# sc15i2gp/daily-ray-trace

Measured on AMD Instinct MI355X. Metric: Mpaths/s (pixels*spp/s) Cornell 1024^2 depth 8; achieved HBM GB/s % of peak, higher is better.
Workload: dtype f64

## Files before the change

daily-ray-trace_amd/csrc/drt_kernels.h:

```cpp
#pragma once

#include "drt_device.h"
#include "drt_build_rule.h"
#include "drt_stash_rule.h"
#include <type_traits>
#include "../../include/drt_hip.h"


enum
{
    SF_PX = 0, SF_PY, SF_PZ, SF_RADIUS,
    SF_NX, SF_NY, SF_NZ,
    SF_UNX, SF_UNY, SF_UNZ,
    SF_VNX, SF_VNY, SF_VNZ,
    SF_ULEN, SF_VLEN,
    SF_COUNT
};
enum
{
    LF_PX = 0, LF_PY, LF_PZ, LF_RADIUS,
    LF_UX, LF_UY, LF_UZ,
    LF_VX, LF_VY, LF_VZ,
    LF_PDF,
    LF_COUNT
// ... 1696 lines not shown
{
    const DevRayTable no_table = {nullptr, nullptr, nullptr, 0u, 0u, 0u, 0u};
    trace_paths_form<SCENE_IN_LDS, TAIL, LIST, false, SCENE_IN_LDS>(k_sc, k_cam, k_tp, records, headers, k_hits, k_counters, k_work_counter, no_table);
}

template <bool SCENE_IN_LDS, bool TAIL = false, bool LIST = false>
__global__ __launch_bounds__(TRACE_BLOCK, DRT_TRACE_WAVES_PER_SIMD) void drt_trace_direct_kernel(DevScene k_sc, DevCamera k_cam, TraceParams k_tp,
                                                                 uint64_t *__restrict__ records, uint64_t *__restrict__ headers,
                                                                 int32_t *__restrict__ k_hits, unsigned long long *__restrict__ k_counters,
                                                                 unsigned long long *__restrict__ k_work_counter)
{
    const DevRayTable no_table = {nullptr, nullptr, nullptr, 0u, 0u, 0u, 0u};
    trace_paths<SCENE_IN_LDS, TAIL, LIST, false>(k_sc, k_cam, k_tp, records, headers, k_hits, k_counters, k_work_counter, no_table);
}

template <bool SCENE_IN_LDS, bool TAIL = false, bool LIST = false>
__global__ __launch_bounds__(TRACE_BLOCK, DRT_TRACE_WAVES_PER_SIMD) void drt_trace_rays_kernel(DevScene k_sc, DevCamera k_cam, TraceParams k_tp,
                                                                 uint64_t *__restrict__ records, uint64_t *__restrict__ headers,
                                                                 int32_t *__restrict__ k_hits, unsigned long long *__restrict__ k_counters,
                                                                 unsigned long long *__restrict__ k_work_counter, DevRayTable k_rt)
{
    trace_paths<SCENE_IN_LDS, TAIL, LIST, true>(k_sc, k_cam, k_tp, records, headers, k_hits, k_counters, k_work_counter, k_rt);
}


#define SHADE_BLOCK 256
#ifndef DRT_SHADE_WAVES_PER_SIMD
#define DRT_SHADE_WAVES_PER_SIMD 4
#endif
#define SHADE_WAVES (SHADE_BLOCK / 64)
#ifndef DRT_SHADE_WAVES_MULTISET
#define DRT_SHADE_WAVES_MULTISET(n) ((n) == 2 ? 3 : 2)
#endif
#define SHADE_WAVES_PER_SIMD_FOR(n) ((n) == 1 ? DRT_SHADE_WAVES_PER_SIMD : DRT_SHADE_WAVES_MULTISET(n))
#ifndef DRT_SHADE_WAVES_SIMPLE
#define DRT_SHADE_WAVES_SIMPLE 5
#endif
#define SHADE_MAX_SETS 4

struct ShadeParams
{
    uint64_t n_pix;
    uint32_t n_samples, first_sample, vertex_words, block_words;
    uint32_t n_lights, batch;
    const uint32_t *overflow;
    uint32_t vertex_shift, mode;
    uint32_t tail_first, tail_count;
    uint32_t chunk, sub_pixels;
    uint32_t light0_em_spd, tail_staged;
    double  *tail_stage;
    const double *tail_resume;
    uint32_t cmf_rw, cmf_x, cmf_y, cmf_z;
    uint32_t tail_period_mains, no_fixed_lists;
    uint32_t items_per_group, n_items;
    const uint32_t *pixel_list;
    const uint32_t *sample_base;
};

struct ShadeConst
{
    DevScene    sc;
    ShadeParams sp;
    const uint64_t     *records, *headers;
    double             *film_pixels, *film_avgs, *film_vars;
    unsigned long long *work_counter;
};
static_assert(sizeof(DevScene) % 8 == 0 && sizeof(ShadeParams) % 8 == 0, "ShadeConst mirrors the kernarg segment only while every argument ends on an 8-byte boundary");
__device__ __forceinline__ const ShadeConst &shade_const()
{
    uint32_t off = 0;
    asm volatile("" : "+s"(off));
    return *(const ShadeConst *)((const char *)__builtin_amdgcn_kernarg_segment_ptr() + off);
}

__device__ __forceinline__ double word_as_double(uint64_t w) { return __longlong_as_double((long long)w); }

__device__ __forceinline__ uint64_t readlane64(uint64_t v, uint32_t l)
{
    uint32_t lo = (uint32_t)__builtin_amdgcn_readlane((int)(uint32_t)v, (int)l);
    uint32_t hi = (uint32_t)__builtin_amdgcn_readlane((int)(uint32_t)(v >> 32), (int)l);
    return (uint64_t)lo | ((uint64_t)hi << 32);
}

__device__ __forceinline__ const uint64_t *path_vertex(const uint64_t *__restrict__ pool, uint32_t block_words, uint32_t vw, uint64_t h2, uint64_t h3, uint32_t v)
{
    const uint32_t b = v >> REC_BLOCK_SHIFT;
    uint32_t id;
    if (b == 0) id = (uint32_t)h2;
    else if (b == 1) id = (uint32_t)(h2 >> 32);
    else if (b == 2) id = (uint32_t)h3;
    else id = ((const uint32_t *)(pool + (uint64_t)(uint32_t)(h3 >> 32) * block_words))[b - REC_HEADER_BLOCKS];
    return pool + (uint64_t)id * block_words + (uint64_t)(v & (REC_BLOCK_VERTICES - 1u)) * vw;
}

template <typename SpdPtr>
__device__ __forceinline__ double spd_at(SpdPtr spds, uint32_t S, uint32_t idx, uint32_t lam)
{
    return spds[idx * S + lam];
}

#define DRT_LIST_MIRROR ((uint64_t)DRT_BDSF_mirror_bdsf)
#define DRT_LIST_GLASS ((uint64_t)DRT_BDSF_fs_dielectric_reflectance_bdsf | ((uint64_t)DRT_BDSF_fs_dielectric_transmittance_bdsf << 4))
#define DRT_LIST_CONDUCTOR ((uint64_t)DRT_BDSF_fs_conductor_bdsf)
#define DRT_LIST_GGX ((uint64_t)DRT_BDSF_ct_conductor_bdsf)
#define DRT_LIST_PLASTIC ((uint64_t)DRT_BDSF_bp_diffuse_bdsf | ((uint64_t)DRT_BDSF_bp_glossy_bdsf << 4))
template <bool SIMPLE = false, uint32_t FIXED_N = 0, uint64_t FIXED_LIST = 0>
__device__ __forceinline__ double bdsf_at_wavelength(uint64_t list_arg, uint32_t num_bdsfs_arg, double diffuse_pi, double glossy, double mirror,
                                                     double ir, double tr, double te, double on_dot, double a_in, double spec,
                                                     double mn_dot, double ct_coef, uint32_t flags, bool paired)
{
    const uint64_t list = FIXED_N != 0u ? FIXED_LIST : list_arg;
    const uint32_t num_bdsfs = FIXED_N != 0u ? FIXED_N : num_bdsfs_arg;
    double bdsf_result = 0.0;
    double reflectance = 0.0;
#define DRT_PIN_HERE(x) asm volatile("" : "+v"(x))
    for (uint32_t i = 0; i < num_bdsfs; i += 1)
    {
        switch ((uint32_t)(list >> (4 * i)) & 15u)
        {
            case DRT_BDSF_bp_diffuse_bdsf:
                bdsf_result = diffuse_pi * a_in;
                break;
            case DRT_BDSF_bp_glossy_bdsf:
                bdsf_result = (glossy * spec) * a_in;
                break;
            case DRT_BDSF_mirror_bdsf:
                bdsf_result = (flags & FLAG_EQR) ? mirror : 0.0;
                break;
            case DRT_BDSF_fs_conductor_bdsf:
                if (SIMPLE) break;
                if (flags & FLAG_EQR)
                {
                    DRT_PIN_HERE(ir);
                    double c2 = on_dot * on_dot;
                    bdsf_result = conductor_reflectance_sel(paired, ir, tr, te, on_dot, c2, 1.0 - c2);
                }
                break;
            case DRT_BDSF_fs_dielectric_reflectance_bdsf:
                if (SIMPLE) break;
                if (flags & FLAG_EQR)
                {
                    DRT_PIN_HERE(ir);
                    bdsf_result = dielectric_reflectance_sel(paired, ir, tr, te, on_dot, 1.0 - on_dot * on_dot);
                }
                break;
            case DRT_BDSF_fs_dielectric_transmittance_bdsf:
                if (SIMPLE) break;
                if (flags & FLAG_EQT)
                {
                    DRT_PIN_HERE(ir);
                    bdsf_result = 1.0 - dielectric_reflectance_sel(paired, ir, tr, te, on_dot, 1.0 - on_dot * on_dot);
                }
                break;
            case DRT_BDSF_ct_conductor_bdsf:
            {
                if (SIMPLE) break;
                DRT_PIN_HERE(ir);
                double c2 = mn_dot * mn_dot;
                bdsf_result = conductor_reflectance_sel(paired, ir, tr, te, mn_dot, c2, 1.0 - c2) * ct_coef;
                break;
            }
            default: break;
        }
        reflectance = bdsf_result + reflectance;
    }
#undef DRT_PIN_HERE
    return reflectance;
}

#ifndef SHADE_PREFETCH_REGS
#define SHADE_PREFETCH_REGS 2
#endif
#define SHADE_PREFETCH_DEPTH 1
#define SHADE_PIXEL_CHUNK 16
#define TAIL_WINDOW_ENTRIES 112u
#define TAIL_WINDOW_WORDS (3u * TAIL_WINDOW_ENTRIES + TAIL_WINDOW_ENTRIES / 4u)
#define SHADE_WAVE_LDS_WORDS ((2u * 64u * SHADE_PREFETCH_REGS) > TAIL_WINDOW_WORDS ? (2u * 64u * SHADE_PREFETCH_REGS) : TAIL_WINDOW_WORDS)

#define XYZ_FILM_WORDS 8

template <bool SPDS_IN_LDS, bool XYZ, bool SIMPLE, bool LIST = false>
__device__ __forceinline__ void shade_tail_group(const DevScene &sc, const ShadeParams &sp, const double *lds, uint64_t *wave_lds, const uint64_t *__restrict__ records,
                                                 const uint64_t *__restrict__ headers, double *__restrict__ film_pixels,
                                                 double *__restrict__ film_avgs, double *__restrict__ film_vars, uint64_t chunk_base,
                                                 uint64_t chunk_end, uint32_t lane, const bool closed)
{
    const uint32_t S = sc.S;
    const uint32_t vw = sp.vertex_words;
    const uint32_t R = sp.tail_count;
    const uint32_t g = lane / R, j = lane - g * R;
    const bool act = g < (uint32_t)(chunk_end - chunk_base) && g < 64u / R;
    const uint32_t lam = sp.tail_first + j;
    const double *table = SPDS_IN_LDS ? (const double *)lds : sc.spds;
    const uint32_t n_groups = 64u / R;
    const uint32_t win = TAIL_WINDOW_ENTRIES / n_groups;
    uint16_t *task_list = (uint16_t *)(wave_lds + 3u * TAIL_WINDOW_ENTRIES);
    const uint32_t leader = g * R;
    const bool in_group = g < n_groups;
    uint32_t v = 0, n_shaded = 0;
    uint64_t ph0 = 0;
    double vignette = 0.0, throughput = 1.0, dst = 0.0;
    uint64_t ph2 = 0;
    uint64_t slot = 0;
    const uint64_t *vcur = records;
    const bool one_light = sp.n_lights == 1u;
    const double em0 = spd_at(table, S, one_light ? sp.light0_em_spd : 0u, lam);
    auto deep_blocks = [&](uint32_t vertex) -> uint64_t { return vertex >= 2u * REC_BLOCK_VERTICES ? headers[slot * REC_HEADER_WORDS + 3] : 0ull; };
    for (uint32_t s0 = sp.tail_staged ? sp.n_samples : 0u; s0 < sp.n_samples; s0 += win)
    {
        const uint32_t s_end = s0 + win < sp.n_samples ? s0 + win : sp.n_samples;
        const uint32_t n_win = s_end - s0, n_px = (uint32_t)(chunk_end - chunk_base);
        uint32_t n_tasks = 0;
        for (uint32_t e0 = 0; e0 < n_px * n_win; e0 += 64u)
        {
            const uint32_t e = e0 + lane;
            const bool valid = e < n_px * n_win;
            const uint32_t ge = valid ? e / n_win : 0u, off = valid ? e - ge * n_win : 0u;
            const uint64_t eslot = (chunk_base + ge) * (uint64_t)sp.batch + s0 + off;
            uint64_t h0 = 0, h1 = 0, h2 = 0;
            if (valid)
            {
                const uint64_t *h = headers + eslot * REC_HEADER_WORDS;
                h0 = h[0];
                h1 = h[1];
                h2 = h[2];
            }
            const bool staged = ((uint32_t)(h0 >> 16) & HDR_TERM_TAIL_STAGED) != 0u;
            const bool has_path = valid && !staged && (h0 & 0xFFFFu) != 0u;
            if (valid && !staged && !has_path)
            {
                const bool emissive = ((uint32_t)(h0 >> 16) & HDR_TERM_MASK) == 1u;
                const uint32_t row = (uint32_t)(h0 >> 32) & 0xFFFFu;
                for (uint32_t t = 0; t < R; t += 1)
                {
                    double d = 0.0;
                    if (emissive) d = d + 1.0 * spd_at(table, S, row, sp.tail_first + t);
                    sp.tail_stage[eslot * R + t] = d * word_as_double(h1);
                }
            }
            const unsigned long long m = __ballot(has_path);
            if (has_path)
            {
                const uint32_t k = n_tasks + (uint32_t)__popcll(m & ((1ull << lane) - 1ull));
                task_list[k] = (uint16_t)e;
                uint64_t *w = wave_lds + e * 3u;
                w[0] = h0;
                w[1] = h1;
                w[2] = h2;
            }
            n_tasks += (uint32_t)__popcll(m);
        }
        __builtin_amdgcn_wave_barrier();
        uint32_t next_task = 0;
        bool busy = false;
        for (;;)
        {
            const unsigned long long want = __ballot(!busy && in_group && lane == leader);
            if (want != 0ull)
            {
                const uint32_t mine = next_task + (uint32_t)__popcll(want & ((1ull << leader) - 1ull));
                if (!busy && in_group && mine < n_tasks)
                {
                    const uint32_t e = task_list[mine];
                    const uint64_t *w = wave_lds + e * 3u;
                    const uint32_t ge = e / n_win, off = e - ge * n_win;
                    slot = (chunk_base + ge) * (uint64_t)sp.batch + s0 + off;
                    ph0 = w[0];
                    vignette = word_as_double(w[1]);
                    ph2 = w[2];
                    n_shaded = (uint32_t)(ph0 & 0xFFFFu);
                    const uint32_t k = ((uint32_t)(ph0 >> 16) >> HDR_TERM_RESUME_SHIFT) & HDR_TERM_RESUME_MASK;
                    v = k;
                    throughput = 1.0;
                    dst = 0.0;
                    if (k != 0u)
                    {
                        const double *at = sp.tail_stage + (slot * R + j);
                        dst = at[0];
                        throughput = at[shade_const().sp.tail_resume - sp.tail_stage];
// ... 121 lines not shown
                        });
                    else if (closed)
                        lane_vertex([&](uint32_t flags, const uint64_t *a) {
                            return bdsf_at_wavelength<SIMPLE, 2, DRT_LIST_PLASTIC>(0, 0, diffuse_pi, glossy, 0.0, 0.0, 0.0, 0.0, 0.0, word_as_double(a[0]), word_as_double(a[1]), 0.0, 0.0, flags, false);
                        });
                    else
                        lane_vertex([&](uint32_t flags, const uint64_t *a) {
                            return bdsf_at_wavelength<SIMPLE>(list, num_bdsfs, diffuse_pi, glossy, mirror, ir, tr, te, on_dot, word_as_double(a[0]), word_as_double(a[1]),
                                                              word_as_double(a[2]), word_as_double(a[3]), flags, paired);
                        });
                    v += 1;
                    if (v < n_shaded) vcur = (v & (REC_BLOCK_VERTICES - 1u)) != 0u ? vcur + vw : path_vertex(records, sp.block_words, vw, ph2, deep_blocks(v), v);
                }
            }
            if (busy && v >= n_shaded)
            {
                if (((uint32_t)(ph0 >> 16) & HDR_TERM_MASK) == 1u) dst = dst + throughput * spd_at(table, S, (uint32_t)(ph0 >> 32) & 0xFFFFu, lam);
                sp.tail_stage[slot * R + j] = dst * vignette;
                busy = false;
            }
        }
        __builtin_amdgcn_wave_barrier();
    }
    uint32_t j_b = j;
    asm volatile("" : "+v"(j_b));
    const uint32_t lam_b = sp.tail_first + j_b;
    uint32_t g_b = g;
    asm volatile("" : "+v"(g_b));
    const uint64_t pix_b = chunk_base + g_b;
    const uint64_t pix_f = LIST ? (act ? (uint64_t)sp.pixel_list[pix_b] : 0u) : pix_b;
    double *px = film_pixels + pix_f * (uint64_t)(XYZ ? XYZ_FILM_WORDS : S + 1);
    double *pa = XYZ ? nullptr : film_avgs + pix_f * (uint64_t)S;
    double *pv = XYZ ? nullptr : film_vars + pix_f * (uint64_t)S;
    const double *stage = sp.tail_stage + (pix_b * (uint64_t)sp.batch) * R + j_b;
    const uint32_t first = LIST ? sp.first_sample + (act ? sp.sample_base[pix_f] : 0u) : sp.first_sample;
    double f_sum = (act && !XYZ) ? px[lam_b] : 0.0, f_avg = (act && !XYZ) ? pa[lam_b] : 0.0, f_var = (act && !XYZ) ? pv[lam_b] : 0.0;
#pragma unroll 4
    for (uint32_t k = 0; k < sp.n_samples; k += 1)
    {
        const double contribution = act ? stage[(uint64_t)k * R] : 0.0;
        const double denom = (double)(first + k + 1);
        f_sum = f_sum + contribution;
        if (!XYZ)
        {
            double t0 = contribution - f_avg;
            double t1 = t0;
            t0 = t0 / denom;
            f_avg = f_avg + t0;
            t0 = contribution - f_avg;
            t0 = t1 * t0;
            f_var = f_var + t0;
        }
    }
    if (XYZ)
    {
        const double rw = spd_at(table, S, sp.cmf_rw, lam_b);
        const double x = act ? (spd_at(table, S, sp.cmf_x, lam_b) * f_sum * rw) : 0.0;
        const double y = act ? (spd_at(table, S, sp.cmf_y, lam_b) * f_sum * rw) : 0.0;
        const double z = act ? (spd_at(table, S, sp.cmf_z, lam_b) * f_sum * rw) : 0.0;
        double X = 0.0, Y = 0.0, Z = 0.0;
        for (uint32_t t = 0; t < R; t += 1)
        {
            const int src = (int)((lane - j_b + t) & 63u);
            X += __shfl(x, src);
            Y += __shfl(y, src);
            Z += __shfl(z, src);
        }
        if (act && j_b == 0)
        {
            px[4] += X;
            px[5] += Y;
            px[6] += Z;
        }
    }
    else if (act)
    {
        px[lam_b] = f_sum;
        pa[lam_b] = f_avg;
        pv[lam_b] = f_var;
    }
}


template <int NSETS, bool SPDS_IN_LDS, bool XYZ, bool DARK, bool SIMPLE, bool LIST, bool CLOSED>
__device__ __forceinline__ void shade_pixels(const DevScene &sc, const ShadeParams &sp, const uint64_t *__restrict__ records,
                                             const uint64_t *__restrict__ headers, double *__restrict__ film_pixels,
                                             double *__restrict__ film_avgs, double *__restrict__ film_vars,
                                             unsigned long long *__restrict__ work_counter)
{
    static_assert(!CLOSED || (NSETS == 1 && SPDS_IN_LDS && !XYZ && !SIMPLE && !LIST), "the closed form exists for one wavelength set, tables in LDS, spectral film, dense launches");
    extern __shared__ double lds[];
    const uint32_t S = sc.S;
    if (*sp.overflow) return;
    if (SPDS_IN_LDS)
    {
        const uint32_t spd_words = sc.n_spd * S;
        for (uint32_t k = threadIdx.x; k < spd_words; k += SHADE_BLOCK) lds[k] = sc.spds[k];
        __syncthreads();
    }
    const uint32_t lane = threadIdx.x & 63u;
    uint64_t *rec_lds = (uint64_t *)(lds + (SPDS_IN_LDS ? (size_t)sc.n_spd * S : 0)) + (size_t)(threadIdx.x >> 6) * SHADE_WAVE_LDS_WORDS;
    const uint32_t vw = sp.vertex_words;
    const uint32_t vpr = vw <= 64 ? 64u / vw : 0u;
    const uint32_t n_fast_regs = vpr * SHADE_PREFETCH_REGS;
    const uint32_t n_fast = n_fast_regs < 2u * REC_BLOCK_VERTICES ? n_fast_regs : 2u * REC_BLOCK_VERTICES;

    uint32_t lam_c[NSETS];
#pragma unroll
    for (int k = 0; k < NSETS; k += 1)
    {
        const uint32_t lam = 64u * k + lane;
        lam_c[k] = lam < S ? lam : 0;
    }

    const uint32_t S_main = sp.tail_count ? sp.tail_first : S;
    for (;;)
    {
        const ShadeParams &qc = shade_const().sp;
        uint32_t item = 0;
        if (lane == 0) item = (uint32_t)atomicAdd(work_counter, 1ull);
        item = (uint32_t)__builtin_amdgcn_readfirstlane((int)item);
        if (item >= qc.n_items) break;
        const bool split = qc.items_per_group > 1;
        const bool inline_tail = qc.tail_count != 0;
        const uint32_t mains_per_group = qc.items_per_group - (inline_tail ? 1u : 0u);
        bool tail_item = inline_tail;
        uint32_t group = item, sub = 0;
        if (split)
        {
            uint32_t m = item;
            if (inline_tail)
            {
                const uint32_t n_groups = qc.n_items / qc.items_per_group;
                const uint32_t q = qc.tail_period_mains, mixed = n_groups * (q + 1u);
                if (item < mixed)
                {
                    const uint32_t period = item / (q + 1u), r = item - period * (q + 1u);
                    tail_item = r == 0u;
                    group = period;
                    m = period * q + (r - 1u);
                }
                else
                {
                    tail_item = false;
                    m = n_groups * q + (item - mixed);
                }
            }
            if (!tail_item)
            {
                group = m / mains_per_group;
                sub = m - group * mains_per_group;
            }
        }
        const uint64_t chunk_base = (uint64_t)group * qc.chunk;
        const uint64_t chunk_end = (chunk_base + qc.chunk < qc.n_pix) ? chunk_base + qc.chunk : qc.n_pix;
        uint64_t main_base = chunk_base, main_end = chunk_end;
        if (split)
        {
            main_base = chunk_base + (uint64_t)sub * qc.sub_pixels;
            main_end = (main_base + qc.sub_pixels < chunk_end) ? main_base + qc.sub_pixels : chunk_end;
            if (tail_item || main_base > chunk_end) main_base = main_end = chunk_end;
        }

      if (qc.mode == 2u) main_base = main_end;
      for (uint64_t pix = main_base; pix < main_end; pix += 1)
      {

        const uint64_t pix_f = LIST ? (uint64_t)sp.pixel_list[pix] : pix;
        double *px = film_pixels + pix_f * (uint64_t)(XYZ ? XYZ_FILM_WORDS : S + 1);
        double *pa = XYZ ? nullptr : film_avgs + pix_f * (uint64_t)S;
        double *pv = XYZ ? nullptr : film_vars + pix_f * (uint64_t)S;
        const uint32_t first = LIST ? sp.first_sample + sp.sample_base[pix_f] : sp.first_sample;
        double f_sum[NSETS], f_avg[NSETS], f_var[NSETS];
#pragma unroll
        for (int k = 0; k < NSETS; k += 1)
        {
            const uint32_t lam = 64u * k + lane;
            const bool active = lam < S_main;
            f_sum[k] = (active && !XYZ) ? px[lam] : 0.0;
            f_avg[k] = (active && !XYZ) ? pa[lam] : 0.0;
            f_var[k] = (active && !XYZ) ? pv[lam] : 0.0;
        }
        bool dark = false;
        if (DARK)
        {
            bool some = false;
#pragma unroll
            for (int k = 0; k < NSETS; k += 1)
                some = some || ((uint64_t)__double_as_longlong(f_sum[k]) | (uint64_t)__double_as_longlong(f_avg[k]) | (uint64_t)__double_as_longlong(f_var[k])) != 0ull;
            dark = !__any(some);
        }
      for (uint32_t s0 = 0; s0 < sp.n_samples; s0 += 64u)
      {
        const uint32_t n_win = (uint32_t)__builtin_amdgcn_readfirstlane((int)((sp.n_samples - s0 < 64u) ? sp.n_samples - s0 : 64u));
        __builtin_assume(n_win >= 1u);
        uint64_t h0 = 0, h1 = 0, h2 = 0, h3 = 0;
        if (lane < n_win)
        {
            const uint64_t *h = headers + (pix * sp.batch + s0 + lane) * REC_HEADER_WORDS;
            h0 = h[0];
            h1 = h[1];
            h2 = h[2];
            h3 = h[3];
        }
        const unsigned long long worthless = !DARK ? 0ull : __ballot(lane < n_win && (h0 & 0xFFFFu) == 0ull && ((uint32_t)(h0 >> 16) & HDR_TERM_MASK) != 1u &&
                                                                      __builtin_isfinite(word_as_double(h1)));
        if (DARK && dark && (uint32_t)__popcll(worthless) == n_win) continue;
        auto prefetch = [&](uint32_t sa, uint32_t nw, uint64_t *dst) {
            if (nw == 0u) return;
            const uint64_t b2 = readlane64(h2, sa);
#pragma unroll
            for (int k = 0; k < SHADE_PREFETCH_REGS; k += 1)
            {
                const uint32_t b = (64u * k) >> (sp.vertex_shift + REC_BLOCK_SHIFT);
                const uint32_t id = b == 0 ? (uint32_t)b2 : (uint32_t)(b2 >> 32);
                const uint64_t *base = records + (uint64_t)id * sp.block_words + (64u * k - (b << (sp.vertex_shift + REC_BLOCK_SHIFT)));
                dst[k] = (64u * k + lane < nw) ? base[lane] : 0;
            }
        };
        uint64_t ring[SHADE_PREFETCH_DEPTH + 1][SHADE_PREFETCH_REGS];
#pragma unroll
        for (int d = 0; d < SHADE_PREFETCH_DEPTH; d += 1)
        {
            const uint32_t nw = ((uint32_t)d < n_win) ? (uint32_t)(readlane64(h0, d) & 0xFFFFu) * vw : 0u;
            prefetch((uint32_t)d < n_win ? (uint32_t)d : 0u, nw, ring[d + 1]);
        }
        for (uint32_t s = 0; s < n_win; s += 1)
        {
            const uint64_t hs = readlane64(h0, s);
            const double vignette = word_as_double(readlane64(h1, s));
            const uint32_t n_shaded = (uint32_t)(hs & 0xFFFFu);
            const uint32_t term = (uint32_t)(hs >> 16) & HDR_TERM_MASK;
            const uint32_t term_spd = (uint32_t)(hs >> 32) & 0xFFFFu;
            const uint32_t plastic_mask = (uint32_t)(hs >> 48);
            const uint32_t vis0_mask = (uint32_t)(hs >> 24) & 0xFFu;
#pragma unroll
            for (int d = 0; d < SHADE_PREFETCH_DEPTH; d += 1)
#pragma unroll
                for (int k = 0; k < SHADE_PREFETCH_REGS; k += 1) ring[d][k] = ring[d + 1][k];
            {
                const uint32_t sa = s + SHADE_PREFETCH_DEPTH;
                const uint32_t nw = (sa < n_win) ? (uint32_t)(readlane64(h0, sa) & 0xFFFFu) * vw : 0u;
                prefetch(sa < n_win ? sa : 0u, nw, ring[SHADE_PREFETCH_DEPTH]);
            }
            const uint64_t *cur = ring[0];
            if (n_shaded != 0u)
            {
                uint64_t *slot_now = rec_lds + (s & 1u) * (64u * SHADE_PREFETCH_REGS);
#pragma unroll
                for (int k = 0; k < SHADE_PREFETCH_REGS; k += 1) slot_now[64u * k + lane] = ring[0][k];
            }
            const uint64_t *rec_words = rec_lds + (s & 1u) * (64u * SHADE_PREFETCH_REGS);
            if (DARK && dark && ((worthless >> s) & 1ull) != 0ull) continue;

            double throughput[NSETS], dst[NSETS];
#pragma unroll
            for (int k = 0; k < NSETS; k += 1)
            {
                throughput[k] = 1.0;
                dst[k] = 0.0;
            }
            uint32_t v_first = 0;
            if (NSETS == 1 && sp.n_lights == 1u && vpr != 0u)
            {
                uint32_t run = (uint32_t)__builtin_ctz(~plastic_mask | 0x10000u);
                run = run < n_shaded ? run : n_shaded;
                run = run < n_fast ? run : n_fast;
                run = run < 8u ? run : 8u;
                if (run != 0u)
                {
                const double *table1 = SPDS_IN_LDS ? (const double *)lds : sc.spds;
                const double em0 = spd_at(table1, S, sp.light0_em_spd, lam_c[0]);
                auto run_vertex = [&](uint64_t w1, const uint64_t *vwords, bool visible) {
                    const double diffuse_pi = spd_at(table1, S, (uint32_t)(w1 >> 16) & 0xFFFFu, lam_c[0]);
                    const double glossy = spd_at(table1, S, (uint32_t)(w1 >> 32) & 0xFFFFu, lam_c[0]);
                    const double dir_pdf = word_as_double(vwords[4]), s_a_in = word_as_double(vwords[5]), s_spec = word_as_double(vwords[6]);
                    const double c = word_as_double(vwords[REC_VERTEX_WORDS + 1]), a_in = word_as_double(vwords[REC_VERTEX_WORDS + 2]);
                    const double spec = word_as_double(vwords[REC_VERTEX_WORDS + 3]);
                    double contribution = 0.0;
                    if (visible)
                    {
                        double reflectance = diffuse_pi * a_in + 0.0;
                        reflectance = (glossy * spec) * a_in + reflectance;
                        contribution = contribution + reflectance;
                        contribution = contribution * em0;
                        contribution = contribution * c;
                    }
                    dst[0] = dst[0] + throughput[0] * contribution;
                    double reflectance = diffuse_pi * s_a_in + 0.0;
                    reflectance = (glossy * s_spec) * s_a_in + reflectance;
                    reflectance = reflectance * dir_pdf;
                    throughput[0] = throughput[0] * reflectance;
                };
                const uint32_t run0 = run < vpr ? run : vpr;
                for (uint32_t v = 0; v < run0; v += 1)
                    run_vertex(readlane64(cur[0], v * vw + 1u), rec_words + v * vw, ((vis0_mask >> v) & 1u) != 0u);
                for (uint32_t v = run0; v < run; v += 1)
                    run_vertex(readlane64(cur[SHADE_PREFETCH_REGS > 1 ? 1 : 0], (v - vpr) * vw + 1u), rec_words + v * vw, ((vis0_mask >> v) & 1u) != 0u);
                v_first = run;
                if (run == n_fast && n_shaded > run && vw * REC_BLOCK_VERTICES == 64u)
                {
                    const uint64_t h3s = readlane64(h3, s);
                    for (uint32_t b = n_fast / REC_BLOCK_VERTICES; b * REC_BLOCK_VERTICES < n_shaded && b < 4u; b += 1)
                    {
                        uint32_t id = (uint32_t)h3s;
                        if (b == 1u) id = (uint32_t)(readlane64(h2, s) >> 32);
                        if (b >= REC_HEADER_BLOCKS) id = ((const uint32_t *)(records + (uint64_t)(uint32_t)(h3s >> 32) * sp.block_words))[b - REC_HEADER_BLOCKS];
                        const uint64_t blockw = records[(uint64_t)id * sp.block_words + lane];
                        uint64_t *slot = rec_lds + (s & 1u) * (64u * SHADE_PREFETCH_REGS);
                        slot[lane] = blockw;
                        const uint32_t v_lo = b * REC_BLOCK_VERTICES;
                        const uint32_t v_hi = n_shaded < v_lo + REC_BLOCK_VERTICES ? n_shaded : v_lo + REC_BLOCK_VERTICES;
                        uint32_t v = v_lo;
                        for (; v < v_hi && ((plastic_mask >> v) & 1u); v += 1)
                        {
                            const uint32_t w0 = (v - v_lo) * vw;
                            const uint64_t lw0 = readlane64(blockw, w0 + REC_VERTEX_WORDS);
                            run_vertex(readlane64(blockw, w0 + 1u), slot + w0, ((uint32_t)(lw0 >> 16) & FLAG_VISIBLE) != 0u);
                        }
                        v_first = v;
                        if (v < v_hi) break;
                    }
                }
                }
            }
            for (uint32_t v = v_first; v < n_shaded; v += 1)
            {
                uint64_t src;
                uint32_t lane0;
                if (v < n_fast)
                {
                    const uint32_t sel = v / vpr;
                    lane0 = (v - sel * vpr) * vw;
                    src = cur[0];
                    if (SHADE_PREFETCH_REGS > 1 && sel != 0) src = cur[SHADE_PREFETCH_REGS > 1 ? 1 : 0];
                }
                else
                {
                    lane0 = 0;
                    src = (lane < vw) ? path_vertex(records, sp.block_words, vw, readlane64(h2, s), readlane64(h3, s), v)[lane] : 0;
                }
                const double *table = SPDS_IN_LDS ? (const double *)lds : sc.spds;
                double contribution[NSETS];
#pragma unroll
                for (int k = 0; k < NSETS; k += 1) contribution[k] = 0.0;
                auto plastic_vertex = [&](uint64_t w1, double dir_pdf, double s_a_in, double s_spec) {
                    const uint32_t i_diffuse = (uint32_t)(w1 >> 16) & 0xFFFFu, i_glossy = (uint32_t)(w1 >> 32) & 0xFFFFu;
                        double diffuse_pi[NSETS], glossy[NSETS];
#pragma unroll
                        for (int k = 0; k < NSETS; k += 1)
                        {
                            diffuse_pi[k] = spd_at(table, S, i_diffuse, lam_c[k]);
                            glossy[k] = spd_at(table, S, i_glossy, lam_c[k]);
                        }
                        if (sp.n_lights == 1u && v < 8u && v < n_fast)
                        {
                            if ((vis0_mask >> v) & 1u)
                            {
                                const uint32_t off = REC_VERTEX_WORDS;
                                const uint64_t *lw = rec_words + v * vw + off;
                                const double c = word_as_double(lw[1]), a_in = word_as_double(lw[2]), spec = word_as_double(lw[3]);
#pragma unroll
                                for (int k = 0; k < NSETS; k += 1)
                                {
                                    double reflectance = diffuse_pi[k] * a_in + 0.0;
                                    reflectance = (glossy[k] * spec) * a_in + reflectance;
                                    contribution[k] = contribution[k] + reflectance;
                                    contribution[k] = contribution[k] * spd_at(table, S, sp.light0_em_spd, lam_c[k]);
                                    contribution[k] = contribution[k] * c;
                                }
                            }
                        }
                        else
                        for (uint32_t l = 0; l < sp.n_lights; l += 1)
                        {
                            if (l == 0 && v < 8u && !((vis0_mask >> v) & 1u)) continue;
                            const uint32_t off = REC_VERTEX_WORDS + l * REC_LIGHT_WORDS;
                            uint64_t lw[4];
                            if (off + REC_LIGHT_WORDS <= 64 || v < n_fast)
                            {
#pragma unroll
                                for (int k = 0; k < 4; k += 1) lw[k] = readlane64(src, lane0 + off + k);
                            }
                            else
                            {
                                const uint64_t *lp = path_vertex(records, sp.block_words, vw, readlane64(h2, s), readlane64(h3, s), v) + off;
#pragma unroll
                                for (int k = 0; k < 4; k += 1) lw[k] = readlane64(lp[k], 0);
                            }
                            if (!((uint32_t)(lw[0] >> 16) & FLAG_VISIBLE)) continue;
                            const uint32_t i_em = (uint32_t)(lw[0] & 0xFFFFu);
                            const double c = word_as_double(lw[1]), a_in = word_as_double(lw[2]), spec = word_as_double(lw[3]);
#pragma unroll
                            for (int k = 0; k < NSETS; k += 1)
                            {
                                double reflectance = diffuse_pi[k] * a_in + 0.0;
                                reflectance = (glossy[k] * spec) * a_in + reflectance;
                                contribution[k] = contribution[k] + reflectance;
                                contribution[k] = contribution[k] * spd_at(table, S, i_em, lam_c[k]);
                                contribution[k] = contribution[k] * c;
                            }
                        }
#pragma unroll
                        for (int k = 0; k < NSETS; k += 1)
                        {
                            dst[k] = dst[k] + throughput[k] * contribution[k];
                            double reflectance = diffuse_pi[k] * s_a_in + 0.0;
                            reflectance = (glossy[k] * s_spec) * s_a_in + reflectance;
                            reflectance = reflectance * dir_pdf;
                            throughput[k] = throughput[k] * reflectance;
                        }
                };
                if (v < 16u && ((plastic_mask >> v) & 1u))
                {
                    const uint64_t w1p = readlane64(src, lane0 + 1);
                    if (v < n_fast)
                    {
                        const uint64_t *vwords = rec_words + v * vw;
                        plastic_vertex(w1p, word_as_double(vwords[4]), word_as_double(vwords[5]), word_as_double(vwords[6]));
                        continue;
                    }
                    const double dir_pdf_p = word_as_double(readlane64(src, lane0 + 4));
                    const double s_a_in_p = word_as_double(readlane64(src, lane0 + 5)), s_spec_p = word_as_double(readlane64(src, lane0 + 6));
                    plastic_vertex(w1p, dir_pdf_p, s_a_in_p, s_spec_p);
                    continue;
                }
                const uint64_t list = readlane64(src, lane0 + 0);
                const uint64_t w1 = readlane64(src, lane0 + 1);
                const uint32_t num_bdsfs = (uint32_t)(w1 & 0xFFu);
                const uint32_t sflags = (uint32_t)(w1 >> 8) & 0xFFu;
                auto fixed_vertex = [&](uint32_t kind) {
                    const bool fresnel = !SIMPLE && kind != 0u;
                    constexpr bool GGX_BODY = CLOSED;
                    const bool rough = GGX_BODY && kind == 3u;
                    const bool in_lds = v < n_fast;
                    const uint64_t *vwords = rec_words + v * vw;
                    uint32_t i_r0 = (uint32_t)(w1 >> 48) & 0xFFFFu, i_r1 = 0, i_r2 = 0;
                    bool paired = false;
                    double on_dot = 0.0;
                    double ct = 0.0;
                    double r0[NSETS], r1[NSETS], r2[NSETS];
#pragma unroll
                    for (int k = 0; k < NSETS; k += 1) r1[k] = r2[k] = 0.0;
                    if (fresnel)
                    {
                        fresnel_rows(readlane64(src, lane0 + 2), i_r0, i_r1, i_r2, paired);
                        if (!rough) on_dot = in_lds ? word_as_double(vwords[3]) : word_as_double(readlane64(src, lane0 + 3));
#pragma unroll
                        for (int k = 0; k < NSETS; k += 1)
                        {
                            r1[k] = spd_at(table, S, i_r1, lam_c[k]);
                            r2[k] = spd_at(table, S, i_r2, lam_c[k]);
                        }
                    }
#pragma unroll
                    for (int k = 0; k < NSETS; k += 1) r0[k] = spd_at(table, S, i_r0, lam_c[k]);
                    auto eval = [&](int k, uint32_t flags) -> double {
                        if (SIMPLE || kind == 0u)
                            return bdsf_at_wavelength<SIMPLE, 1u, DRT_LIST_MIRROR>(0ull, 0u, 0.0, 0.0, r0[k], 0.0, 0.0, 0.0, 0.0, 0.0, 0.0, 0.0, 0.0, flags, false);
                        if (kind == 1u)
                            return bdsf_at_wavelength<SIMPLE, 2u, DRT_LIST_GLASS>(0ull, 0u, 0.0, 0.0, 0.0, r0[k], r1[k], r2[k], on_dot, 0.0, 0.0, 0.0, 0.0, flags, paired);
                        if (kind == 2u || !GGX_BODY)
                            return bdsf_at_wavelength<SIMPLE, 1u, DRT_LIST_CONDUCTOR>(0ull, 0u, 0.0, 0.0, 0.0, r0[k], r1[k], r2[k], on_dot, 0.0, 0.0, 0.0, 0.0, flags, paired);
                        return bdsf_at_wavelength<SIMPLE, 1u, DRT_LIST_GGX>(0ull, 0u, 0.0, 0.0, 0.0, r0[k], r1[k], r2[k], 0.0, 0.0, 0.0, on_dot, ct, flags, paired);
                    };
                    for (uint32_t l = 0; l < sp.n_lights; l += 1)
                    {
                        if (l == 0 && v < 8u && !((vis0_mask >> v) & 1u)) continue;
                        const uint32_t off = REC_VERTEX_WORDS + l * REC_LIGHT_WORDS;
                        uint64_t lw0;
                        double c;
                        if (off + REC_LIGHT_WORDS <= 64 || v < n_fast)
                        {
                            lw0 = readlane64(src, lane0 + off);
                            c = in_lds ? word_as_double(vwords[off + 1u]) : word_as_double(readlane64(src, lane0 + off + 1u));
                            if (rough)
                            {
                                on_dot = in_lds ? word_as_double(vwords[off + 4u]) : word_as_double(readlane64(src, lane0 + off + 4u));
                                ct = in_lds ? word_as_double(vwords[off + 5u]) : word_as_double(readlane64(src, lane0 + off + 5u));
                            }
                        }
                        else
                        {
                            const uint64_t *lp = path_vertex(records, sp.block_words, vw, readlane64(h2, s), readlane64(h3, s), v) + off;
                            lw0 = readlane64(lp[0], 0);
                            c = word_as_double(lp[1]);
                            if (rough)
                            {
                                on_dot = word_as_double(lp[4]);
                                ct = word_as_double(lp[5]);
                            }
                        }
                        const uint32_t lflags = (uint32_t)(lw0 >> 16) & 0xFFu;
                        if (!(lflags & FLAG_VISIBLE)) continue;
                        const uint32_t i_em = (uint32_t)(lw0 & 0xFFFFu);
#pragma unroll
                        for (int k = 0; k < NSETS; k += 1)
                        {
                            double reflectance = eval(k, lflags);
                            contribution[k] = contribution[k] + reflectance;
                            contribution[k] = contribution[k] * spd_at(table, S, i_em, lam_c[k]);
                            contribution[k] = contribution[k] * c;
                        }
                    }
                    if (rough)
                    {
                        on_dot = in_lds ? word_as_double(vwords[7]) : word_as_double(readlane64(src, lane0 + 7));
                        ct = in_lds ? word_as_double(vwords[8]) : word_as_double(readlane64(src, lane0 + 8));
                    }
#pragma unroll
                    for (int k = 0; k < NSETS; k += 1)
                    {
                        dst[k] = dst[k] + throughput[k] * contribution[k];
                        double reflectance = eval(k, sflags);
                        const double dir_pdf = in_lds ? word_as_double(vwords[4]) : word_as_double(readlane64(src, lane0 + 4));
                        reflectance = reflectance * dir_pdf;
                        throughput[k] = throughput[k] * reflectance;
                    }
                };
                if (CLOSED)
                {
                    if (sflags & FLAG_PLASTIC)
                        plastic_vertex(w1, word_as_double(readlane64(src, lane0 + 4)), word_as_double(readlane64(src, lane0 + 5)), word_as_double(readlane64(src, lane0 + 6)));
                    else
                        fixed_vertex(list == DRT_LIST_MIRROR ? 0u : list == DRT_LIST_GLASS ? 1u : list == DRT_LIST_CONDUCTOR ? 2u : 3u);
                    continue;
                }
                if (!shade_const().sp.no_fixed_lists)
                {
                    uint32_t kind = 4u;
                    if (num_bdsfs == 1u && list == DRT_LIST_MIRROR) kind = 0u;
                    if (!SIMPLE && num_bdsfs == 2u && list == DRT_LIST_GLASS) kind = 1u;
                    if (!SIMPLE && num_bdsfs == 1u && list == DRT_LIST_CONDUCTOR) kind = 2u;
                    if (kind != 4u)
                    {
                        fixed_vertex(kind);
                        continue;
                    }
                }
                const uint64_t w2 = readlane64(src, lane0 + 2);
                const double on_dot = word_as_double(readlane64(src, lane0 + 3));
                const double dir_pdf = word_as_double(readlane64(src, lane0 + 4));
                const uint32_t i_diffuse = (uint32_t)(w1 >> 16) & 0xFFFFu, i_glossy = (uint32_t)(w1 >> 32) & 0xFFFFu;
                const uint32_t i_mirror = (uint32_t)(w1 >> 48) & 0xFFFFu;
                uint32_t i_ir, i_tr, i_te;
                bool paired;
                fresnel_rows(w2, i_ir, i_tr, i_te, paired);
                const double s_a_in = word_as_double(readlane64(src, lane0 + 5)), s_spec = word_as_double(readlane64(src, lane0 + 6));

                if (sflags & FLAG_PLASTIC)
                {
                    plastic_vertex(w1, dir_pdf, s_a_in, s_spec);
                    continue;
                }

                double diffuse[NSETS], glossy[NSETS], mirror[NSETS], ir[NSETS], tr[NSETS], te[NSETS];
#pragma unroll
                for (int k = 0; k < NSETS; k += 1)
                {
                    diffuse[k] = spd_at(table, S, i_diffuse, lam_c[k]); glossy[k] = spd_at(table, S, i_glossy, lam_c[k]);
                    mirror[k] = spd_at(table, S, i_mirror, lam_c[k]);   ir[k] = SIMPLE ? 0.0 : spd_at(table, S, i_ir, lam_c[k]);
                    tr[k] = SIMPLE ? 0.0 : spd_at(table, S, i_tr, lam_c[k]); te[k] = SIMPLE ? 0.0 : spd_at(table, S, i_te, lam_c[k]);
                }
                for (uint32_t l = 0; l < sp.n_lights; l += 1)
                {
                    if (l == 0 && v < 8u && !((vis0_mask >> v) & 1u)) continue;
                    const uint32_t off = REC_VERTEX_WORDS + l * REC_LIGHT_WORDS;
                    uint64_t lw[REC_LIGHT_WORDS];
                    if (off + REC_LIGHT_WORDS <= 64 || v < n_fast)
                    {
#pragma unroll
                        for (int k = 0; k < REC_LIGHT_WORDS; k += 1) lw[k] = readlane64(src, lane0 + off + k);
                    }
                    else
                    {
                        const uint64_t *lp = path_vertex(records, sp.block_words, vw, readlane64(h2, s), readlane64(h3, s), v) + off;
#pragma unroll
                        for (int k = 0; k < REC_LIGHT_WORDS; k += 1) lw[k] = readlane64(lp[k], 0);
                    }
                    const uint32_t lflags = (uint32_t)(lw[0] >> 16) & 0xFFu;
                    if (!(lflags & FLAG_VISIBLE)) continue;
                    const uint32_t i_em = (uint32_t)(lw[0] & 0xFFFFu);
                    const double c = word_as_double(lw[1]);
#pragma unroll
                    for (int k = 0; k < NSETS; k += 1)
                    {
                        double reflectance = bdsf_at_wavelength<SIMPLE>(list, num_bdsfs, diffuse[k], glossy[k], mirror[k], ir[k], tr[k], te[k], on_dot,
                                                                word_as_double(lw[2]), word_as_double(lw[3]), word_as_double(lw[4]),
                                                                word_as_double(lw[5]), lflags, paired);
                        contribution[k] = contribution[k] + reflectance;
                        contribution[k] = contribution[k] * spd_at(table, S, i_em, lam_c[k]);
                        contribution[k] = contribution[k] * c;
                    }
                }
                const double s_mn = word_as_double(readlane64(src, lane0 + 7)), s_ct = word_as_double(readlane64(src, lane0 + 8));
#pragma unroll
                for (int k = 0; k < NSETS; k += 1)
                {
                    dst[k] = dst[k] + throughput[k] * contribution[k];
                    double reflectance = bdsf_at_wavelength<SIMPLE>(list, num_bdsfs, diffuse[k], glossy[k], mirror[k], ir[k], tr[k], te[k], on_dot,
                                                            s_a_in, s_spec, s_mn, s_ct, sflags, paired);
                    reflectance = reflectance * dir_pdf;
                    throughput[k] = throughput[k] * reflectance;
                }
            }
            const double denom = (double)(first + s0 + s + 1);
            if (DARK) dark = false;
#pragma unroll
            for (int k = 0; k < NSETS; k += 1)
            {
                if (term == 1)
                {
                    const double em = SPDS_IN_LDS ? spd_at((const double *)lds, S, term_spd, lam_c[k]) : spd_at(sc.spds, S, term_spd, lam_c[k]);
                    dst[k] = dst[k] + throughput[k] * em;
                }
                const double contribution = dst[k] * vignette;
                f_sum[k] = f_sum[k] + contribution;
                if (!XYZ)
                {
                    double t0 = contribution - f_avg[k];
                    double t1 = t0;
                    t0 = t0 / denom;
                    f_avg[k] = f_avg[k] + t0;
                    t0 = contribution - f_avg[k];
                    t0 = t1 * t0;
                    f_var[k] = f_var[k] + t0;
                }
            }
        }
      }
        if (XYZ)
        {
            const double *table = SPDS_IN_LDS ? (const double *)lds : sc.spds;
            double X = 0.0, Y = 0.0, Z = 0.0;
#pragma unroll
            for (int k = 0; k < NSETS; k += 1)
            {
                const uint32_t lam = 64u * k + lane;
                if (lam < S_main)
                {
                    const double rw = spd_at(table, S, sp.cmf_rw, lam);
                    X += (spd_at(table, S, sp.cmf_x, lam) * f_sum[k] * rw);
                    Y += (spd_at(table, S, sp.cmf_y, lam) * f_sum[k] * rw);
                    Z += (spd_at(table, S, sp.cmf_z, lam) * f_sum[k] * rw);
                }
            }
            for (int off = 32; off > 0; off >>= 1)
            {
                X += __shfl_xor(X, off);
                Y += __shfl_xor(Y, off);
                Z += __shfl_xor(Z, off);
            }
            if (lane == 0)
            {
                px[0] += X;
                px[1] += Y;
                px[2] += Z;
                px[3] += (double)sp.n_samples * 1.0;
            }
        }
        else
        {
#pragma unroll
            for (int k = 0; k < NSETS; k += 1)
            {
                const uint32_t lam = 64u * k + lane;
                if (lam < S_main)
                {
                    px[lam] = f_sum[k];
                    pa[lam] = f_avg[k];
                    pv[lam] = f_var[k];
                }
            }
            if (lane == 0) px[S] += (double)sp.n_samples * 1.0;
        }
      }

        if (tail_item && sp.mode != 1u) shade_tail_group<SPDS_IN_LDS, XYZ, SIMPLE, LIST>(sc, sp, (const double *)lds, rec_lds, records, headers, film_pixels, film_avgs, film_vars, chunk_base, chunk_end, lane, CLOSED);
    }
}

template <int NSETS, bool SPDS_IN_LDS, bool XYZ, bool DARK, bool SIMPLE = false, bool LIST = false>
__global__ __launch_bounds__(SHADE_BLOCK, (SIMPLE && NSETS == 1) ? DRT_SHADE_WAVES_SIMPLE : SHADE_WAVES_PER_SIMD_FOR(NSETS)) void drt_shade_kernel(DevScene sc, ShadeParams sp, const uint64_t *__restrict__ records,
                                                                 const uint64_t *__restrict__ headers, double *__restrict__ film_pixels,
                                                                 double *__restrict__ film_avgs, double *__restrict__ film_vars,
                                                                 unsigned long long *__restrict__ work_counter)
{
    shade_pixels<NSETS, SPDS_IN_LDS, XYZ, DARK, SIMPLE, LIST, false>(sc, sp, records, headers, film_pixels, film_avgs, film_vars, work_counter);
}

#ifndef DRT_SHADE_WAVES_CLOSED
#define DRT_SHADE_WAVES_CLOSED 4
#endif
template <bool DARK>
__global__ __launch_bounds__(SHADE_BLOCK, DRT_SHADE_WAVES_CLOSED) void drt_shade_kernel_closed(DevScene sc, ShadeParams sp, const uint64_t *__restrict__ records,
                                                                 const uint64_t *__restrict__ headers, double *__restrict__ film_pixels,
                                                                 double *__restrict__ film_avgs, double *__restrict__ film_vars,
                                                                 unsigned long long *__restrict__ work_counter)
{
    shade_pixels<1, true, false, DARK, false, false, true>(sc, sp, records, headers, film_pixels, film_avgs, film_vars, work_counter);
}

__global__ void drt_film_xyz_kernel(DevScene sc, uint32_t cmf_rw, uint32_t cmf_x, uint32_t cmf_y, uint32_t cmf_z, double interval,
                                    uint64_t n_pix, const double *__restrict__ film_pixels, double *__restrict__ xyz)
{
    uint64_t p = (uint64_t)blockIdx.x * blockDim.x + threadIdx.x;
    if (p >= n_pix) return;
    const uint32_t S = sc.S;
    const double *rw = sc.spds + (size_t)cmf_rw * S, *cx = sc.spds + (size_t)cmf_x * S;
    const double *cy = sc.spds + (size_t)cmf_y * S, *cz = sc.spds + (size_t)cmf_z * S;
    const double *px = film_pixels + p * (uint64_t)(S + 1);
    double f = px[S];
    double n = 0.0;
    for (uint32_t i = 0; i < S; i += 1) n += (cy[i] * rw[i]);
    n *= interval;
    double X = 0.0, Y = 0.0, Z = 0.0;
    for (uint32_t i = 0; i < S; i += 1)
    {
        double v = px[i] / f;
        X += (cx[i] * v * rw[i]);
        Y += (cy[i] * v * rw[i]);
        Z += (cz[i] * v * rw[i]);
    }
    xyz[3 * p + 0] = X * (interval / n);
    xyz[3 * p + 1] = Y * (interval / n);
    xyz[3 * p + 2] = Z * (interval / n);
}

__global__ void drt_film_bgra_kernel(DevScene sc, uint32_t cmf_rw, uint32_t cmf_x, uint32_t cmf_y, uint32_t cmf_z, double interval,
                                     uint64_t n_pix, const double *__restrict__ film, int which, uint8_t *__restrict__ bgra)
{
    uint64_t p = (uint64_t)blockIdx.x * blockDim.x + threadIdx.x;
    if (p >= n_pix) return;
    const uint32_t S = sc.S;
    const double *rw = sc.spds + (size_t)cmf_rw * S, *cx = sc.spds + (size_t)cmf_x * S;
    const double *cy = sc.spds + (size_t)cmf_y * S, *cz = sc.spds + (size_t)cmf_z * S;
    const double *px = film + p * (uint64_t)(which == 0 ? S + 1 : S);
    double div = 1.0;
    bool divide = false;
    if (which == 0) { div = px[S]; divide = true; }
    if (which == 2)
    {
        double highest = 0.0;
        for (uint32_t i = 0; i < S; i += 1) if (px[i] > highest) highest = px[i];
        div = highest;
        divide = true;
    }
    double n = 0.0;
    for (uint32_t i = 0; i < S; i += 1) n += (cy[i] * rw[i]);
    n *= interval;
    double X = 0.0, Y = 0.0, Z = 0.0;
    for (uint32_t i = 0; i < S; i += 1)
    {
        double v = divide ? px[i] / div : px[i];
        X += (cx[i] * v * rw[i]);
        Y += (cy[i] * v * rw[i]);
        Z += (cz[i] * v * rw[i]);
    }
    X *= (interval / n);
    Y *= (interval / n);
    Z *= (interval / n);
    double rgb[3];
    rgb[0] = (2.3706743 * X) - (0.9000405 * Y) - (0.4706338 * Z);
    rgb[1] = (-0.5138850 * X) + (1.4253036 * Y) + (0.0885814 * Z);
    rgb[2] = (0.0052982 * X) - (0.0146949 * Y) + (1.0093968 * Z);
    uint8_t out[3];
    for (int c = 0; c < 3; c += 1)
    {
        double f = rgb[c];
        f = (f < 0.0) ? 0.0 : f;
        f = (f > 1.0) ? 1.0 : f;
        out[c] = (f == f) ? (uint8_t)(f * 255.0) : (uint8_t)0;
    }
    uchar4 o;
    o.x = out[2]; o.y = out[1]; o.z = out[0]; o.w = 255;
    ((uchar4 *)bgra)[p] = o;
}

__global__ void drt_xyz_finish_kernel(DevScene sc, uint32_t cmf_rw, uint32_t cmf_y, double interval, uint64_t n_pix,
                                      const double *__restrict__ film, double *__restrict__ xyz)
{
    uint64_t p = (uint64_t)blockIdx.x * blockDim.x + threadIdx.x;
    if (p >= n_pix) return;
    const uint32_t S = sc.S;
// ... 311 lines not shown
```

daily-ray-trace_amd/csrc/drt_launcher.hip:

```cpp
#include "drt_kernels.h"
#include "drt_bvh_kernels.h"
#include "drt_adaptive_kernels.h"
#include "drt_sample_map_kernels.h"
#include "drt_denoise_kernels.h"
#include "drt_feature_kernels.h"
#include "drt_matte_kernels.h"
#include "drt_ray_kernels.h"
#include "drt_update_kernels.h"
#include "drt_build_kernels.h"
#include "drt_material_kernels.h"
#include "drt_depth_kernels.h"
#include "drt_sensor_kernels.h"
#include "drt_bucket_kernels.h"
#include "drt_lobe_kernels.h"
#include "drt_window_kernels.h"
#include "drt_window_rule.h"
#include "drt_pair_rule.h"
#include "drt_owned.h"

#include <algorithm>
#include <cmath>
#include <cstdarg>
#include <cstdio>
#include <cstdlib>
#include <cstring>
#include <map>
#include <string>
#include <chrono>
#include <vector>

static thread_local std::string g_last_error;

#define RAY_STAGING_RAYS (1u << 20)
#define DRT_DEFAULT_MAX_BATCH 256

#define DRT_PAIR_COUNTERS (DRT_NUM_COUNTERS + 8)
#define DRT_COUNTER_WORDS (DRT_PAIR_COUNTERS + DRT_NUM_COUNTERS)

static int fail(int code, const char *fmt, ...)
{
    char buf[512];
    va_list ap;
    va_start(ap, fmt);
    vsnprintf(buf, sizeof(buf), fmt, ap);
    va_end(ap);
    g_last_error = buf;
    return code;
}

#define HIP_TRY(expr)                                                                                      \
    do                                                                                                     \
    {                                                                                                      \
        hipError_t e_ = (expr);                                                                            \
        if (e_ != hipSuccess) return fail(-100 - (int)e_, "%s: %s", #expr, hipGetErrorString(e_));         \
    } while (0)

struct DeviceMem
{
    static std::atomic<uint64_t> &live() { static std::atomic<uint64_t> n{0}; return n; }
    static hipError_t alloc(void **p, size_t bytes)
    {
        const hipError_t e = hipMalloc(p, bytes);
        if (e == hipSuccess) live() += 1;
        return e;
    }
    static void free(void *p) { (void)hipFree(p); live() -= 1; }
};
struct PinnedMem
{
    static std::atomic<uint64_t> &live() { static std::atomic<uint64_t> n{0}; return n; }
    static hipError_t alloc(void **p, size_t bytes)
    {
        const hipError_t e = hipHostMalloc(p, bytes, hipHostMallocDefault);
        if (e == hipSuccess) live() += 1;
        return e;
    }
    static void free(void *p) { (void)hipHostFree(p); live() -= 1; }
};
template <typename T> using DevBuf = Owned<T, DeviceMem>;
template <typename T> using PinnedBuf = Owned<T, PinnedMem>;

struct drt_context
{
    int         device = 0;
    hipStream_t stream = nullptr;
    Stream      own_stream;
    drt_params  params{};
    DevScene    dsc{};
    DevCamera   dcam{};
    uint32_t    cmf_rw = 0, cmf_x = 0, cmf_y = 0, cmf_z = 0;
    double      interval = 0.0;

    std::vector<DevBuf<unsigned char>> allocations;
    std::vector<DevMaterial> host_mats;
    DevMaterial *d_mat_variants = nullptr;
    double *d_pixels = nullptr, *d_avgs = nullptr, *d_vars = nullptr;
    DevBuf<double> own_pixels, own_avgs, own_vars;
    bool    xyz_mode = false;
    bool    own_film = false;
    DevBuf<uint64_t> d_records, d_headers;
    uint32_t  light0_em_spd = 0;
    DevBuf<double> d_tail_stage;
    DevBuf<double> d_tail_resume;
    uint32_t  batch_spp = 1;
    uint32_t  vertex_words = 0, vertex_shift = 0, block_words = 0;
    uint64_t  pool_blocks = 0;
    uint32_t  worst_blocks_per_path = 0;
    double    est_blocks_per_path = 0.0;
    struct Batch { PairSpan span; uint64_t seq; };
    std::vector<Batch> inflight;
    uint64_t  next_seq = 1;
    uint64_t  redone_batches = 0, pool_peak = 0;
    DevBuf<int32_t> d_hits;
    uint64_t  hits_capacity = 0;
    uint32_t  hits_samples = 0;
    DevBuf<unsigned long long> d_counters;
    DevBuf<PrimaryHit> d_primary;
    DevBuf<uint64_t> d_queue;
    bool        bvh_pipeline = false;
    int         primary_grid_cap = 0, bounce_grid_cap = 0;
    DevBuf<double> d_xyz;
    DevBuf<uint8_t> d_bgra;
    bool      trace_tail = false;
    bool      tail_all_staged = false;
    bool      tail_resume = false;
    bool      dark_skip = true;
    bool      dark_skip_win = true;
    bool      no_fixed_lists = false;
    bool      simple_bdsfs = false;
    bool      no_closed_shade = false;
    bool      closed_lists = false;
    const double *d_spd_tail = nullptr;

    bool   scene_in_lds = true, spds_in_lds = true, use_bvh = false;
    size_t trace_lds = 0, shade_lds = 0;
    bool trace_stash = false;
    int    trace_grid_cap = 0, shade_grid_cap = 0;
    uint32_t trace_chunk_override = 0;
    ShadeOverrides shade_overrides;
    uint32_t debug_shade_mode = 0;
    bool     debug_tail_phase_a_off = false;
    uint32_t shade_sets = 1, tail_first = 0, tail_count = 0;
    uint64_t n_pix = 0;

    std::vector<Event> ev;
    std::vector<double> ev_paths;
    size_t ev_used = 0;
    double trace_ms = 0.0, shade_ms = 0.0;
    uint64_t timed_pairs = 0;
    double min_sample_ms = 0.0, max_sample_ms = 0.0, avg_sample_ms = 0.0;

    bool film_used = false, adaptive_done = false;
    DevBuf<uint32_t> d_counts;
    DevBuf<uint32_t> d_alist[2];
    DevBuf<unsigned long long> d_keep;
    DevBuf<uint32_t> d_bkeep;
    DevBuf<uint32_t> d_ainfo;
    PinnedBuf<uint32_t> h_active;
    uint64_t film_gen = 0;
    uint64_t dn_gen = 0;
    bool     dn_valid = false;
    DevBuf<double> d_dn_mean, d_dn_var, d_dn_guide, d_dn_weights, d_dn_wsum;
    DevBuf<uint32_t> d_dn_unusable;
    uint32_t dn_window_cap = 0;
    std::vector<drt_material> ft_mats;
    std::vector<double> ft_spds;
    uint32_t ft_n_spd = 0, ft_S = 0;
    DevBuf<double> d_ft_mean, d_ft_m2, d_ft_colour;
    DevBuf<int32_t> d_ft_ids;
    DevBuf<uint32_t> d_ft_counts, d_ft_report;
    DevBuf<unsigned long long> d_ft_info;
    Event    ft_ev[2];
    bool     ft_valid = false, ft_from_film = false;
    uint64_t ft_gen = 0;
    DevBuf<int32_t> d_mt_ids, d_mt_list;
    DevBuf<uint32_t> d_mt_counts, d_mt_tail;
    DevBuf<double> d_mt_cover;
    DevBuf<unsigned long long> d_mt_info;
    Event    mt_ev[2];
    bool     mt_valid = false, mt_from_film = false;
    uint64_t mt_gen = 0;
    uint64_t ray_chunk = RAY_STAGING_RAYS;
    int      ray_grid_cap = 1;
    DevBuf<double> d_ray_a, d_ray_b;
    DevBuf<drt_ray_hit> d_ray_hits;
    DevBuf<uint8_t> d_ray_visible;
    DevBuf<uint32_t> d_ray_xy, d_ray_samples;
    bool        rays_bound = false;
    DevRayTable rt{};
    DevBuf<double> d_rt_origins, d_rt_dirs, d_rt_weights;
    std::vector<drt_surface> h_surfaces;
    bool      h_stale = false;
    std::vector<BvhNode>  h_nodes;
    std::vector<uint32_t> h_order;
    double    cam_reach = 0.0, extent = 0.0;
    bool      extent_known = true;
    bool      upd_ready = false;
    DevBuf<drt_surface> d_raw; PinnedBuf<drt_surface> h_stage;
    DevBuf<int32_t> d_light_slot;
    DevBuf<double> d_boxes;
    DevBuf<uint32_t> d_leaf_parent;
    DevBuf<uint2> d_levels;
    std::vector<uint32_t> level_first;
    DevBuf<unsigned long long> d_upd_status;
    Event     upd_ev[3];
    bool      upd_timed = false, stage_busy = false;
    bool      upd_check = false, upd_violation = false;
    uint32_t  updates = 0, refits = 0;
    double    upd_ms = 0.0;
    bool      boxes_valid = false;
    bool      hb_ready = false, hb_timed = false;
    bool      hb_mirror_pending = false;
    DevBuf<uint32_t> d_hb_tree_surf, d_hb_pos[2], d_hb_table, d_hb_order;
    DevBuf<uint64_t> d_hb_keys[2];
    DevBuf<uint4> d_hb_items[2];
    DevBuf<unsigned char> d_hb_status; PinnedBuf<unsigned char> hb_mirror;
    Event     hb_ev[3];
    uint32_t  hb_builds = 0, hb_built_by = 0, hb_depth = 0;
// ... 518 lines not shown
    d.bvh_leaf = nullptr;
    if (ctx->use_bvh)
    {
        BvhBuilder bb;
        bb.build(scene, reach);
        if (bb.max_depth > BVH_STACK) return fail(-2, "BVH of %zu surfaces is %d levels deep, the traversal stack holds %d", bb.prims.size(), bb.max_depth, BVH_STACK);
        if (!(bb.extent < 134217728.0)) return fail(-2, "scene or camera coordinates reach %g: the hierarchy's f32 box test holds up to 2^27", bb.extent);
        std::vector<BvhLeafPrim> leaf(std::max<size_t>(bb.order.size(), 1));
        memset(leaf.data(), 0, leaf.size() * sizeof(BvhLeafPrim));
        for (size_t k = 0; k < bb.order.size(); k += 1)
        {
            const uint32_t i = bb.order[k];
            leaf[k].index = i;
            leaf[k].type = stype[i];
            for (int f = 0; f < 4; f += 1) leaf[k].f[f] = surf[(size_t)f * n_surf + i];
            leaf[k].reach32 = INFINITY;
            if (stype[i] == DRT_GEO_SPHERE)
            {
                for (int f = 0; f < 3; f += 1) leaf[k].c32[f] = (float)leaf[k].f[f];
                leaf[k].reach32 = bvh_sphere_reach32(leaf[k].f[3], bb.extent);
            }
        }
        if ((rc = upload(ctx, bb.nodes, &d.bvh_nodes))) return rc;
        if ((rc = upload(ctx, leaf, &d.bvh_leaf))) return rc;
        ctx->h_nodes = bb.nodes;
        ctx->h_order = bb.order;
        ctx->hb_depth = (uint32_t)bb.max_depth;
        ctx->extent = bb.extent;
    }
    if (!ctx->scene_in_lds) ctx->trace_lds = 0;
    ctx->spds_in_lds = (size_t)d.n_spd * S * 8 <= 64 * 1024;
    {
        uint32_t sets = 0, tf = 0, tc = 0;
        shade_sets(S, &sets, &tf, &tc);
        const size_t extra = (size_t)d.n_spd * tc * 8 + (size_t)(TRACE_BLOCK / 64) * (2 * tc + 1) * 64 * 8;
        ctx->simple_bdsfs = !getenv("DRT_NO_SIMPLE_SHADE");
        ctx->no_fixed_lists = getenv("DRT_NO_FIXED_LISTS") != nullptr;
        for (uint32_t i = 0; i < scene->num_materials; i += 1)
            for (uint32_t j = 0; j < mats[i].num_bdsfs; j += 1)
            {
                const uint32_t b = mats[i].bdsfs[j];
                if (b != DRT_BDSF_bp_diffuse_bdsf && b != DRT_BDSF_bp_glossy_bdsf && b != DRT_BDSF_mirror_bdsf) ctx->simple_bdsfs = false;
            }
        ctx->no_closed_shade = getenv("DRT_NO_CLOSED_SHADE") != nullptr;
        ctx->closed_lists = closed_lists(mats.data(), scene->num_materials, smat.data(), n_surf);
        bool all_simple = true;
        for (uint32_t i = 0; i < n_surf; i += 1)
        {
            const DevMaterial &m = mats[smat[i]];
            const bool mirror_only = m.num_bdsfs == 1u && m.bdsfs[0] == DRT_BDSF_mirror_bdsf;
            if (!(m.is_black_body || (m.vertex_flags & FLAG_PLASTIC) || mirror_only)) all_simple = false;
        }
        const char *e = getenv("DRT_TRACE_TAIL");
        const size_t lane_rows = (size_t)(TRACE_BLOCK / 64) * (TRACE_LANE_ROWS + 1) * 64 * 8;
        ctx->trace_tail = ctx->scene_in_lds && sets == 1 && tc > 0 && tc <= 8 && n_lights == 1 && ctx->trace_lds + extra - lane_rows <= 48 * 1024 && !(e && *e == '0') &&
                          (all_simple || !(e && *e == '2'));
        ctx->tail_all_staged = ctx->trace_tail && all_simple;
        const char *er = getenv("DRT_TAIL_RESUME");
        ctx->tail_resume = ctx->trace_tail && !ctx->tail_all_staged && !(er && *er == '0');
        if (ctx->trace_tail)
        {
            std::vector<double> cols((size_t)d.n_spd * tc);
            for (uint32_t r = 0; r < d.n_spd; r += 1)
                for (uint32_t j = 0; j < tc; j += 1) cols[(size_t)r * tc + j] = spds[(size_t)r * S + tf + j];
            if ((rc = upload(ctx, cols, &ctx->d_spd_tail))) return rc;
            ctx->trace_lds += extra;
        }
    }
    return 0;
}

static bool shade_simple(const drt_context *ctx) { return ctx->simple_bdsfs && ctx->spds_in_lds && ctx->shade_sets == 1; }

static bool shade_dark(const drt_context *ctx, const ShadeParams &sp)
{
    return (ctx->win_open && !sp.pixel_list) ? ctx->dark_skip_win : ctx->dark_skip;
}

static bool shade_closed(const drt_context *ctx)
{
    return ctx->closed_lists && !ctx->no_closed_shade && !ctx->no_fixed_lists && !shade_simple(ctx) && ctx->spds_in_lds && ctx->shade_sets == 1 && !ctx->xyz_mode;
}

template <int NSETS, bool XYZ, bool LIST>
static int launch_shade_mode(drt_context *ctx, uint32_t grid, const ShadeParams &sp, double *const film[3])
{
    if (NSETS == 1 && !XYZ && !LIST && shade_closed(ctx))
    {
#define DRT_LAUNCH_CLOSED(DARK)                                                                                                                    \
    hipLaunchKernelGGL((drt_shade_kernel_closed<DARK>), dim3(grid), dim3(SHADE_BLOCK), ctx->shade_lds, ctx->stream, ctx->dsc, sp, ctx->d_records, \
                       ctx->d_headers, film[0], film[1], film[2], ctx->d_counters + DRT_NUM_COUNTERS + 1)
        if (shade_dark(ctx, sp)) DRT_LAUNCH_CLOSED(true);
        else DRT_LAUNCH_CLOSED(false);
#undef DRT_LAUNCH_CLOSED
        return 0;
    }
#define DRT_LAUNCH_SHADE(LDS, DARK, SIMPLE)                                                                                                       \
    hipLaunchKernelGGL((drt_shade_kernel<NSETS, LDS, XYZ, DARK, SIMPLE, LIST>), dim3(grid), dim3(SHADE_BLOCK), ctx->shade_lds, ctx->stream, ctx->dsc, sp, \
                       ctx->d_records, ctx->d_headers, film[0], film[1], film[2], ctx->d_counters + DRT_NUM_COUNTERS + 1)
    if (NSETS == 1 && shade_simple(ctx))
    {
        if (shade_dark(ctx, sp)) DRT_LAUNCH_SHADE(true, true, (NSETS == 1));
        else DRT_LAUNCH_SHADE(true, false, (NSETS == 1));
    }
    else if (ctx->spds_in_lds && shade_dark(ctx, sp)) DRT_LAUNCH_SHADE(true, true, false);
    else if (ctx->spds_in_lds) DRT_LAUNCH_SHADE(true, false, false);
    else if (shade_dark(ctx, sp)) DRT_LAUNCH_SHADE(false, true, false);
    else DRT_LAUNCH_SHADE(false, false, false);
#undef DRT_LAUNCH_SHADE
    return 0;
}

template <int NSETS>
static int launch_shade_sets(drt_context *ctx, uint32_t grid, const ShadeParams &sp, double *const film[3])
{
    if (sp.pixel_list) return launch_shade_mode<NSETS, false, true>(ctx, grid, sp, film);
    return ctx->xyz_mode ? launch_shade_mode<NSETS, true, false>(ctx, grid, sp, film) : launch_shade_mode<NSETS, false, false>(ctx, grid, sp, film);
}

static void shade_sets(uint32_t S, uint32_t *n_sets, uint32_t *tail_first, uint32_t *tail_count)
{
    uint32_t full = S / 64, rem = S % 64;
    *tail_first = 0;
    *tail_count = 0;
    if (S <= 64 || rem == 0) *n_sets = (S + 63) / 64;
    else if (rem <= 16 && !getenv("DRT_NO_TAIL_PASS"))
    {
        *n_sets = full;
        *tail_first = 64 * full;
        *tail_count = rem;
    }
    else *n_sets = full + 1;
}

static int launch_shade(drt_context *ctx, uint32_t grid, const ShadeParams &sp, double *const film[3])
{
    switch (ctx->shade_sets)
    {
        case 1: return launch_shade_sets<1>(ctx, grid, sp, film);
        case 2: return launch_shade_sets<2>(ctx, grid, sp, film);
        case 3: return launch_shade_sets<3>(ctx, grid, sp, film);
        default: return launch_shade_sets<4>(ctx, grid, sp, film);
    }
}

template <int NCUTS>
static const void *depth_kernel(bool lds) { return lds ? (const void *)drt_depth_cut_kernel<NCUTS, true> : (const void *)drt_depth_cut_kernel<NCUTS, false>; }
static const void *depth_kernel(uint32_t n_cuts, bool lds)
{
    switch (n_cuts)
    {
        case 1: return depth_kernel<1>(lds);
        case 2: return depth_kernel<2>(lds);
        case 3: return depth_kernel<3>(lds);
        case 4: return depth_kernel<4>(lds);
        case 5: return depth_kernel<5>(lds);
        case 6: return depth_kernel<6>(lds);
        case 7: return depth_kernel<7>(lds);
        default: return depth_kernel<8>(lds);
    }
}
static size_t depth_lds_bytes(const drt_context *ctx) { return ctx->spds_in_lds ? (size_t)ctx->dsc.n_spd * ctx->dsc.S * 8 : 0; }

static int launch_depth_cuts(drt_context *ctx, const ShadeParams &sp, uint64_t pix0)
{
    const size_t S = ctx->dsc.S;
    DepthCutParams dp{};
    dp.n_pix = sp.n_pix;
    dp.n_samples = sp.n_samples;
    dp.first_sample = sp.first_sample;
    dp.vertex_words = sp.vertex_words;
    dp.block_words = sp.block_words;
    dp.n_lights = sp.n_lights;
    dp.batch = sp.batch;
    dp.overflow = sp.overflow;
    dp.n_sets = (uint32_t)((S + 63) / 64);
// ... 74 lines not shown
        case 2: return lobe_kernel<2>(lds);
        case 3: return lobe_kernel<3>(lds);
        case 4: return lobe_kernel<4>(lds);
        case 5: return lobe_kernel<5>(lds);
        case 6: return lobe_kernel<6>(lds);
        case 7: return lobe_kernel<7>(lds);
        default: return lobe_kernel<8>(lds);
    }
}

static uint64_t lobe_row(const uint8_t *row)
{
    uint64_t w = 0;
    for (uint32_t f = 0; f < (uint32_t)DRT_NUM_BDSFS; f += 1) w |= (uint64_t)row[f] << (8 * f);
    return w;
}

static int launch_lobes(drt_context *ctx, const ShadeParams &sp, uint64_t pix0)
{
    const size_t S = ctx->dsc.S;
    LobeParams lp{};
    lp.n_pix = sp.n_pix;
    lp.n_samples = sp.n_samples;
    lp.first_sample = sp.first_sample;
    lp.vertex_words = sp.vertex_words;
    lp.block_words = sp.block_words;
    lp.n_lights = sp.n_lights;
    lp.batch = sp.batch;
    lp.overflow = sp.overflow;
    lp.n_sets = (uint32_t)((S + 63) / 64);
    lp.max_depth = ctx->params.max_depth;
    lp.emission = ctx->lobe_map.emission;
    lp.direct = lobe_row(ctx->lobe_map.direct);
    lp.indirect = lobe_row(ctx->lobe_map.indirect);
    if (sp.n_pix * lp.n_sets >= 0xFFFFFFFFull) return fail(-1, "tile too large for the lobe work queue");
    lp.n_items = (uint32_t)(sp.n_pix * lp.n_sets);
    for (uint32_t c = 0; c < ctx->n_lobes; c += 1)
    {
        lp.pixels[c] = ctx->lobes.pixels[c] + pix0 * (S + 1);
        lp.avgs[c] = ctx->lobes.avgs[c] + pix0 * S;
        lp.vars[c] = ctx->lobes.vars[c] + pix0 * S;
    }
    const uint64_t *records = ctx->d_records, *headers = ctx->d_headers;
    unsigned long long *queue = ctx->d_counters + DRT_NUM_COUNTERS + 3;
    const uint32_t grid = (uint32_t)std::min<uint64_t>(((uint64_t)lp.n_items + LOBE_WAVES - 1) / LOBE_WAVES, (uint64_t)ctx->lobes.grid_cap);
    void *args[] = {&ctx->dsc, &lp, &records, &headers, &queue};
    HIP_TRY(hipLaunchKernel(lobe_kernel(ctx->n_lobes, ctx->spds_in_lds), dim3(grid), dim3(LOBE_BLOCK), args, depth_lds_bytes(ctx), ctx->stream));
    return 0;
}

static int launch_sensor(drt_context *ctx, const ShadeParams &sp, uint64_t pix0)
{
    const size_t S = ctx->dsc.S, n = ctx->n_sensor;
    SensorParams np{};
    np.n_pix = sp.n_pix;
    np.n_samples = sp.n_samples;
    np.first_sample = sp.first_sample;
    np.vertex_words = sp.vertex_words;
    np.block_words = sp.block_words;
    np.n_lights = sp.n_lights;
    np.batch = sp.batch;
    np.overflow = sp.overflow;
    np.n_sets = (uint32_t)((S + 63) / 64);
    np.max_depth = ctx->params.max_depth;
    np.n_channels = ctx->n_sensor;
    if (sp.n_pix >= 0xFFFFFFFFull) return fail(-1, "tile too large for the sensor work queue");
    np.n_items = (uint32_t)sp.n_pix;
    np.curves = ctx->sensor.curves;
    np.pixels = ctx->sensor.pixels + pix0 * (n + 1);
    np.avgs = ctx->sensor.avgs + pix0 * n;
    np.vars = ctx->sensor.vars + pix0 * n;
    const uint64_t *records = ctx->d_records, *headers = ctx->d_headers;
    unsigned long long *queue = ctx->d_counters + DRT_NUM_COUNTERS + 3;
    const uint32_t grid = (uint32_t)std::min<uint64_t>((sp.n_pix + SENSOR_WAVES - 1) / SENSOR_WAVES, (uint64_t)ctx->sensor.grid_cap);
    void *args[] = {&ctx->dsc, &np, &records, &headers, &queue};
    HIP_TRY(hipLaunchKernel(sensor_kernel(ctx->sensor.spds_in_lds), dim3(grid), dim3(SENSOR_BLOCK), args,
                            sensor_lds_bytes(ctx, ctx->n_sensor, ctx->sensor.spds_in_lds), ctx->stream));
    return 0;
}

template <int NSETS, bool XYZ>
static int shade_occupancy_mode(drt_context *ctx, int *per_cu)
{
    if (NSETS == 1 && !XYZ && shade_closed(ctx))
        HIP_TRY(hipOccupancyMaxActiveBlocksPerMultiprocessor(per_cu, drt_shade_kernel_closed<true>, SHADE_BLOCK, ctx->shade_lds));
    else if (NSETS == 1 && shade_simple(ctx))
        HIP_TRY(hipOccupancyMaxActiveBlocksPerMultiprocessor(per_cu, drt_shade_kernel<NSETS, true, XYZ, true, (NSETS == 1)>, SHADE_BLOCK, ctx->shade_lds));
    else if (ctx->spds_in_lds)
        HIP_TRY(hipOccupancyMaxActiveBlocksPerMultiprocessor(per_cu, drt_shade_kernel<NSETS, true, XYZ, true>, SHADE_BLOCK, ctx->shade_lds));
    else
        HIP_TRY(hipOccupancyMaxActiveBlocksPerMultiprocessor(per_cu, drt_shade_kernel<NSETS, false, XYZ, true>, SHADE_BLOCK, ctx->shade_lds));
    return 0;
}

template <int NSETS>
static int shade_occupancy(drt_context *ctx, int *per_cu)
{
    return ctx->xyz_mode ? shade_occupancy_mode<NSETS, true>(ctx, per_cu) : shade_occupancy_mode<NSETS, false>(ctx, per_cu);
}

extern "C" const char *drt_last_error(void) { return g_last_error.c_str(); }

extern "C" int drt_bvh_stats(const drt_scene *scene, uint32_t *nodes, uint32_t *leaf_surfaces, uint32_t *depth, uint32_t *stack_entries)
{
    g_last_error.clear();
    if (!scene) return fail(-1, "null argument");
    BvhBuilder bb;
    bb.build(scene, 0.0);
    if (nodes) *nodes = (uint32_t)bb.nodes.size();
    if (leaf_surfaces) *leaf_surfaces = (uint32_t)bb.order.size();
    if (depth) *depth = (uint32_t)bb.max_depth;
    if (stack_entries) *stack_entries = BVH_STACK;
    return 0;
}

extern "C" int drt_device_count(void)
{
    int n = 0;
    hipError_t e = hipGetDeviceCount(&n);
    if (e != hipSuccess) return fail(-1, "hipGetDeviceCount: %s", hipGetErrorString(e));
    return n;
}

static size_t pixels_bytes(const drt_context *ctx)
{
    return (size_t)ctx->n_pix * (ctx->xyz_mode ? (size_t)XYZ_FILM_WORDS : (size_t)ctx->dsc.S + 1) * 8;
}

static int enqueue_trace(drt_context *ctx, const TraceTile &tile, const PairSpan &span);

static uint64_t trace_waves(const drt_context *ctx, uint64_t n_paths)
{
    const uint64_t cap = (uint64_t)(ctx->bvh_pipeline ? ctx->bounce_grid_cap : ctx->trace_grid_cap);
    return std::min<uint64_t>(cap, (n_paths + TRACE_BLOCK - 1) / TRACE_BLOCK) * (TRACE_BLOCK / 64);
}
static uint64_t blocks_worst_case(const drt_context *ctx, uint64_t n_paths)
{
    return (uint64_t)((double)n_paths * ctx->worst_blocks_per_path * (1.0 + 64.0 / POOL_CHUNK)) + trace_waves(ctx, n_paths) * (POOL_CHUNK + 2 * 64) + 1;
}

static double camera_reach(const drt_camera *camera)
{
    double reach = 0.0;
    for (int k = 0; k < 3; k += 1)
    {
        const double a = camera->aperture_position[k], f = camera->film_bottom_left[k];
        reach = std::max(reach, std::fabs(a) + 2.0 * std::fabs(f - a) + std::fabs(camera->aperture_radius));
    }
    return reach;
}

static void set_device_camera(drt_context *ctx, const drt_camera *camera)
{
    DevCamera &c = ctx->dcam;
    c.forward = hv(camera->forward); c.right = hv(camera->right); c.up = hv(camera->up);
    c.aperture_position = hv(camera->aperture_position); c.film_bottom_left = hv(camera->film_bottom_left);
    c.aperture_radius = camera->aperture_radius; c.focal_depth = camera->focal_depth;
    c.pixel_width = camera->pixel_width; c.pixel_height = camera->pixel_height;
    ctx->h_camera = *camera;
    ctx->win_dirty = true;
}

static LiveWindow live_window_of(const drt_surface *surfaces, size_t n_surf, const drt_material &escape, const drt_camera &camera, const drt_params &params)
{
    double lo[3] = {HUGE_VAL, HUGE_VAL, HUGE_VAL}, hi[3] = {-HUGE_VAL, -HUGE_VAL, -HUGE_VAL};
    bool any = false;
// ... 62 lines not shown
    ctx->cam_reach = reach;
    ctx->h_surfaces.assign(scene->surfaces, scene->surfaces + scene->num_surfaces);
    ctx->ft_mats.assign(scene->materials, scene->materials + scene->num_materials);
    ctx->ft_n_spd = scene->num_spds;
    ctx->ft_S = scene->num_wavelengths;
    ctx->ft_spds.assign(scene->spds, scene->spds + (size_t)scene->num_spds * scene->num_wavelengths);
    if (const char *e = getenv("DRT_NO_LIVE_WINDOW")) ctx->win_allowed = atoi(e) == 0;
    if (ctx->xyz_mode)
    {
        const uint32_t rows[4] = {scene->cmf_rw, scene->cmf_x, scene->cmf_y, scene->cmf_z};
        for (int k = 0; k < 4; k += 1)
            for (uint32_t i = 0; i < scene->num_wavelengths; i += 1)
                if (!std::isfinite(scene->spds[(size_t)rows[k] * scene->num_wavelengths + i])) ctx->win_allowed = false;
    }

    set_device_camera(ctx, camera);

    const uint32_t S = scene->num_wavelengths;
    ctx->n_pix = (uint64_t)params->tile_w * params->tile_h;
    ctx->vertex_words = 16;
    while (ctx->vertex_words < REC_VERTEX_WORDS + REC_LIGHT_WORDS * ctx->dsc.n_lights) ctx->vertex_words *= 2;
    ctx->vertex_shift = 0;
    while ((1u << ctx->vertex_shift) < ctx->vertex_words) ctx->vertex_shift += 1;
    ctx->block_words = REC_BLOCK_VERTICES * ctx->vertex_words;
    const uint32_t deepest = (params->max_depth + REC_BLOCK_VERTICES - 1) / REC_BLOCK_VERTICES;
    ctx->worst_blocks_per_path = deepest + (deepest > REC_HEADER_BLOCKS ? 1u : 0u);
    if (deepest > REC_HEADER_BLOCKS + 2 * ctx->block_words)
        return fail(-2, "max_depth %u: a path's table block holds %u blocks beyond the header's %d", params->max_depth, 2 * ctx->block_words, REC_HEADER_BLOCKS);
    if (ctx->dsc.n_spd >= 0xFFFFu) return fail(-2, "too many SPDs for the 16-bit record indices");
    if (S > 64 * SHADE_MAX_SETS) return fail(-2, "more than %d wavelengths", 64 * SHADE_MAX_SETS);
    {
        uint32_t sets = 0, tf = 0, tc = 0;
        shade_sets(S, &sets, &tf, &tc);
        ctx->tail_count = tc;
    }
    ctx->bvh_pipeline = !ctx->scene_in_lds;

    HIP_TRY(ctx->own_pixels.need(pixels_bytes(ctx) / 8));
    if (!ctx->xyz_mode)
    {
        HIP_TRY(ctx->own_avgs.need((size_t)ctx->n_pix * S));
        HIP_TRY(ctx->own_vars.need((size_t)ctx->n_pix * S));
    }
    ctx->d_pixels = ctx->own_pixels;
    ctx->d_avgs = ctx->own_avgs;
    ctx->d_vars = ctx->own_vars;
    ctx->own_film = true;
    HIP_TRY(hipMemsetAsync(ctx->d_pixels, 0, pixels_bytes(ctx), ctx->stream));
    if (ctx->d_avgs) HIP_TRY(hipMemsetAsync(ctx->d_avgs, 0, (size_t)ctx->n_pix * S * 8, ctx->stream));
    if (ctx->d_vars) HIP_TRY(hipMemsetAsync(ctx->d_vars, 0, (size_t)ctx->n_pix * S * 8, ctx->stream));
    HIP_TRY(ctx->d_counters.need(DRT_COUNTER_WORDS));
    HIP_TRY(hipMemsetAsync(ctx->d_counters, 0, DRT_COUNTER_WORDS * sizeof(unsigned long long), ctx->stream));

    hipDeviceProp_t prop;
    HIP_TRY(hipGetDeviceProperties(&prop, ctx->device));
    int per_cu = 0;
    if (ctx->scene_in_lds && ctx->trace_tail)
        HIP_TRY(hipOccupancyMaxActiveBlocksPerMultiprocessor(&per_cu, drt_trace_direct_kernel<true, true>, TRACE_BLOCK, ctx->trace_lds));
    else if (ctx->scene_in_lds)
        HIP_TRY(hipOccupancyMaxActiveBlocksPerMultiprocessor(&per_cu, drt_trace_direct_kernel<true, false>, TRACE_BLOCK, ctx->trace_lds));
    ctx->trace_stash = false;
    if (ctx->scene_in_lds && !(getenv("DRT_NO_RAY_STASH") && atoi(getenv("DRT_NO_RAY_STASH")) != 0) && ctx->trace_lds + TRACE_STASH_BYTES <= 64 * 1024)
    {
        int with = 0;
        if (ctx->trace_tail) HIP_TRY(hipOccupancyMaxActiveBlocksPerMultiprocessor(&with, drt_trace_kernel<true, true>, TRACE_BLOCK, ctx->trace_lds + TRACE_STASH_BYTES));
        else HIP_TRY(hipOccupancyMaxActiveBlocksPerMultiprocessor(&with, drt_trace_kernel<true, false>, TRACE_BLOCK, ctx->trace_lds + TRACE_STASH_BYTES));
        ctx->trace_stash = with >= 1 && with >= per_cu;
    }
    if (per_cu < 1) per_cu = 1;
    if (const char *e = getenv("DRT_TRACE_BLOCKS_PER_CU")) per_cu = std::max(1, atoi(e));
    ctx->trace_grid_cap = prop.multiProcessorCount * per_cu;
    ctx->ray_grid_cap = prop.multiProcessorCount * 4;
    if (const char *e = getenv("DRT_RAY_CHUNK"))
        ctx->ray_chunk = std::max<uint64_t>(1, std::min<uint64_t>(RAY_STAGING_RAYS, strtoull(e, nullptr, 0)));
    if (ctx->bvh_pipeline)
    {
        int p_cu = 0, b_cu = 0;
        HIP_TRY(hipOccupancyMaxActiveBlocksPerMultiprocessor(&p_cu, drt_primary_kernel<false>, PRIMARY_BLOCK, 0));
        HIP_TRY(hipOccupancyMaxActiveBlocksPerMultiprocessor(&b_cu, drt_bounce_kernel<false>, BOUNCE_BLOCK, 0));
        if (const char *e = getenv("DRT_TRACE_BLOCKS_PER_CU")) b_cu = std::max(1, atoi(e));
        ctx->primary_grid_cap = prop.multiProcessorCount * std::max(1, p_cu);
        ctx->bounce_grid_cap = prop.multiProcessorCount * std::max(1, b_cu);
    }
    ctx->shade_lds = ctx->spds_in_lds ? (size_t)ctx->dsc.n_spd * S * 8 : 0;
    ctx->shade_lds += (size_t)SHADE_WAVES * SHADE_WAVE_LDS_WORDS * 8;
    int s_per_cu = 0;
    shade_sets(S, &ctx->shade_sets, &ctx->tail_first, &ctx->tail_count);
    switch (ctx->shade_sets)
    {
        case 1: rc = shade_occupancy<1>(ctx, &s_per_cu); break;
        case 2: rc = shade_occupancy<2>(ctx, &s_per_cu); break;
        case 3: rc = shade_occupancy<3>(ctx, &s_per_cu); break;
        default: rc = shade_occupancy<4>(ctx, &s_per_cu); break;
    }
    if (rc) return rc;
    if (s_per_cu < 1) s_per_cu = 1;
    if (const char *e = getenv("DRT_SHADE_BLOCKS_PER_CU")) s_per_cu = std::max(1, atoi(e));
    ctx->shade_grid_cap = prop.multiProcessorCount * s_per_cu;
    if (const char *e = getenv("DRT_RESERVE_BLOCKS"))
    {
        int n = std::max(0, atoi(e));
        ctx->trace_grid_cap = std::max(1, ctx->trace_grid_cap - n);
        ctx->shade_grid_cap = std::max(1, ctx->shade_grid_cap - n);
    }
    if (const char *e = getenv("DRT_TRACE_CHUNK")) ctx->trace_chunk_override = (uint32_t)std::min(1 << 20, std::max(64, atoi(e) / 64 * 64));
    if (const char *e = getenv("DRT_TAIL_PERIOD")) ctx->shade_overrides.tail_period = (uint32_t)std::max(0, atoi(e));
    if (const char *e = getenv("DRT_SHADE_SUBS")) ctx->shade_overrides.subs = (uint32_t)std::max(0, atoi(e));
    if (const char *e = getenv("DRT_SHADE_CHUNK")) ctx->shade_overrides.chunk = (uint32_t)atoi(e);
    if (const char *e = getenv("DRT_DEBUG_SHADE_MODE")) ctx->debug_shade_mode = (uint32_t)atoi(e);
    if (const char *e = getenv("DRT_DEBUG_TAIL_PHASE_A_OFF")) ctx->debug_tail_phase_a_off = atoi(e) != 0;
    const size_t block_bytes = (size_t)ctx->block_words * 8;
    const uint64_t npx = std::max<uint64_t>(ctx->n_pix, 1);
    const size_t per_path_fixed = REC_HEADER_WORDS * 8 + (size_t)ctx->tail_count * 8 * (ctx->tail_resume ? 2 : 1) +
                                  (ctx->bvh_pipeline ? sizeof(PrimaryHit) + sizeof(uint64_t) : 0);
    size_t free_b = 0, total_b = 0;
    HIP_TRY(hipMemGetInfo(&free_b, &total_b));
    ctx->est_blocks_per_path = (double)ctx->worst_blocks_per_path;
    if (npx * (uint64_t)ctx->worst_blocks_per_path * block_bytes > (256ull << 20) && !getenv("DRT_POOL_WORST_CASE"))
    {
        const bool win = window_in_use(ctx);
        const PairWindow pw = {win, ctx->wx0, ctx->wx1, ctx->wy0, ctx->wy1};
        const uint64_t live_px = win ? (uint64_t)(ctx->wx1 - ctx->wx0) * (ctx->wy1 - ctx->wy0) : npx;
        const TraceTile sample = pool_sample_tile(ctx->params, pw, pool_sample_step(live_px));
        const uint64_t n_sample = sample.n_pix;
        ctx->pool_blocks = blocks_worst_case(ctx, n_sample);
        HIP_TRY(ctx->d_records.need(ctx->pool_blocks * ctx->block_words));
        HIP_TRY(ctx->d_headers.need(n_sample * REC_HEADER_WORDS));
        if (ctx->bvh_pipeline)
        {
            HIP_TRY(ctx->d_primary.need(n_sample));
            HIP_TRY(ctx->d_queue.need(n_sample));
        }
        if ((rc = enqueue_trace(ctx, sample, PairSpan::whole_tile(ctx->params.first_sample, 1, 0)))) return rc;
        unsigned long long used = 0;
        HIP_TRY(hipMemcpyAsync(&used, ctx->d_counters + DRT_PAIR_COUNTERS + 5, sizeof(used), hipMemcpyDeviceToHost, ctx->stream));
        HIP_TRY(hipStreamSynchronize(ctx->stream));
        ctx->est_blocks_per_path = (double)used / (double)n_sample * ((double)live_px / (double)npx);
        {
            unsigned long long cnt[3] = {0, 0, 0};
            HIP_TRY(hipMemcpy(cnt, ctx->d_counters + DRT_PAIR_COUNTERS, sizeof(cnt), hipMemcpyDeviceToHost));
            if (cnt[0] > 0)
            {
                const double per_path = (double)cnt[2] / (double)cnt[0];
                ctx->dark_skip_win = per_path < 3.0;
                ctx->dark_skip = per_path * ((double)live_px / (double)npx) < 3.0;
            }
        }
        ctx->d_records.reset();
        ctx->d_headers.reset();
        ctx->d_primary.reset();
        ctx->d_queue.reset();
        HIP_TRY(hipMemsetAsync(ctx->d_counters, 0, DRT_COUNTER_WORDS * sizeof(unsigned long long), ctx->stream));
        ctx->ev_used = 0;
        ctx->ev_paths.clear();
    }
    auto blocks_for = [&](uint64_t n_paths) -> uint64_t {
        const double want = 1.2 * ctx->est_blocks_per_path * (double)n_paths + 16.0 * std::sqrt((double)n_paths) + 4096.0;
        const uint64_t expect = (uint64_t)(want * (1.0 + 64.0 / POOL_CHUNK)) + trace_waves(ctx, n_paths) * (POOL_CHUNK + 2 * 64) + 1;
        return std::max<uint64_t>(std::min<uint64_t>(expect, blocks_worst_case(ctx, n_paths)), blocks_worst_case(ctx, npx));
    };
    uint32_t batch = params->batch_spp;
    if (batch == DRT_BATCH_RESIDENT)
    {
        const uint64_t resident_paths = getenv("DRT_RESIDENT_PATHS_M") ? (uint64_t)std::max(1, atoi(getenv("DRT_RESIDENT_PATHS_M"))) << 20 : (256ull << 20);
        const uint64_t by_paths = std::max<uint64_t>(1, std::min<uint64_t>(DRT_DEFAULT_MAX_BATCH, resident_paths / npx));
        batch = (uint32_t)std::max<uint64_t>(by_paths, 16);
        if (params->spp) batch = std::min(batch, params->spp);
    }
    else if (batch == 0)
    {
        const double path_bytes = 1.2 * (1.0 + 64.0 / POOL_CHUNK) * ctx->est_blocks_per_path * (double)block_bytes + (double)per_path_fixed;
        uint64_t by_job = (std::max<uint32_t>(params->spp, 1) + 31) / 32;
        uint64_t by_floor = (uint64_t)((double)(16ull << 30) / (path_bytes * (double)npx));
        uint64_t cap = std::max<uint64_t>(1, std::min<uint64_t>(DRT_DEFAULT_MAX_BATCH, (64ull << 20) / npx));
        batch = (uint32_t)std::max<uint64_t>(1, std::min(std::max(by_job, by_floor), cap));
        if (params->spp) batch = std::min(batch, params->spp);
    }
    batch = std::min<uint32_t>(batch, 4096);
    const size_t film_bytes = ctx->xyz_mode ? (size_t)ctx->n_pix * XYZ_FILM_WORDS * 8 : (size_t)ctx->n_pix * (3 * (size_t)S + 1) * 8;
    (void)film_bytes;
    auto bytes_for = [&](uint32_t b) -> size_t { return blocks_for(npx * b) * block_bytes + (size_t)npx * b * per_path_fixed; };
    while (batch > 1 && bytes_for(batch) > free_b / 2) batch /= 2;
    if (bytes_for(batch) > free_b) return fail(-3, "not enough device memory: need %zu bytes", bytes_for(batch));
    ctx->batch_spp = batch;
    ctx->pool_blocks = blocks_for(npx * batch);
    if (const char *e = getenv("DRT_POOL_BLOCKS"))
    {
        const bool win = window_in_use(ctx);
        const uint64_t live = (uint64_t)(ctx->wx1 - ctx->wx0) * (ctx->wy1 - ctx->wy0);
        const uint64_t floor_px = win ? std::min<uint64_t>(npx, std::max<uint64_t>(live, params->tile_w)) : npx;
        ctx->pool_blocks = std::max<uint64_t>(blocks_worst_case(ctx, floor_px), std::min<uint64_t>(ctx->pool_blocks, strtoull(e, nullptr, 0)));
    }
    if (ctx->pool_blocks >= 0xFFFFFFF0ull) return fail(-3, "record pool of %llu blocks: block numbers are 32 bits", (unsigned long long)ctx->pool_blocks);
    HIP_TRY(ctx->d_records.need(ctx->pool_blocks * ctx->block_words));
    HIP_TRY(ctx->d_headers.need((size_t)npx * batch * REC_HEADER_WORDS));
    if (ctx->bvh_pipeline)
    {
        HIP_TRY(ctx->d_primary.need((size_t)npx * batch));
        HIP_TRY(ctx->d_queue.need((size_t)npx * batch));
    }
    if (ctx->tail_count) HIP_TRY(ctx->d_tail_stage.need((size_t)npx * batch * ctx->tail_count));
    if (ctx->tail_count && ctx->tail_resume) HIP_TRY(ctx->d_tail_resume.need((size_t)npx * batch * ctx->tail_count));
    if (const char *e = getenv("DRT_DARK_SKIP")) ctx->dark_skip = ctx->dark_skip_win = atoi(e) != 0;
    if (getenv("DRT_VERBOSE"))
        fprintf(stderr, "drt: %d CUs, trace %d blocks/CU (lds %zu), shade %d blocks/CU (lds %zu), batch %u, %.3f blocks/path measured (worst %u), pool %.2f GB\n",
                prop.multiProcessorCount, per_cu, ctx->trace_lds, s_per_cu, ctx->shade_lds, ctx->batch_spp, ctx->est_blocks_per_path,
                ctx->worst_blocks_per_path, (double)(ctx->pool_blocks * block_bytes) / 1e9);
    HIP_TRY(hipStreamSynchronize(ctx->stream));
    return 0;
}

extern "C" drt_context *drt_create(const drt_scene *scene, const drt_camera *camera, const drt_params *params)
{
    g_last_error.clear();
    drt_context *ctx = new drt_context();
    int rc = create_impl(ctx, scene, camera, params);
    if (rc != 0)
    {
        std::string keep = g_last_error;
        drt_destroy(ctx);
        (void)hipGetLastError();
        g_last_error = keep;
        return nullptr;
    }
    return ctx;
}

extern "C" void drt_destroy(drt_context *ctx)
{
    if (!ctx) return;
    (void)hipSetDevice(ctx->device);
    if (ctx->stream) (void)hipStreamSynchronize(ctx->stream);
    delete ctx;
}

extern "C" int drt_bind_film(drt_context *ctx, void *d_pixels, void *d_avgs, void *d_vars)
{
    if (!ctx || !d_pixels || (!ctx->xyz_mode && (!d_avgs || !d_vars))) return fail(-1, "null argument");
    HIP_TRY(hipSetDevice(ctx->device));
    HIP_TRY(hipStreamSynchronize(ctx->stream));
    ctx->own_pixels.reset();
    ctx->own_avgs.reset();
    ctx->own_vars.reset();
    ctx->own_film = false;
    ctx->film_gen += 1;
    ctx->d_pixels = (double *)d_pixels;
    ctx->d_avgs = (double *)d_avgs;
    ctx->d_vars = (double *)d_vars;
    return 0;
}

extern "C" int drt_set_stream(drt_context *ctx, void *hip_stream)
{
    if (!ctx) return fail(-1, "null context");
    HIP_TRY(hipSetDevice(ctx->device));
    HIP_TRY(hipStreamSynchronize(ctx->stream));
    ctx->stream = hip_stream ? (hipStream_t)hip_stream : ctx->own_stream;
    return 0;
}

extern "C" int drt_synchronize(drt_context *ctx);

static int next_events(drt_context *ctx, hipEvent_t out[3])
{
    if (ctx->ev.size() < ctx->ev_used + 3) ctx->ev.resize(ctx->ev_used + 3);
    for (int k = 0; k < 3; k += 1) HIP_TRY(ctx->ev[ctx->ev_used + k].need());
    for (int k = 0; k < 3; k += 1) out[k] = ctx->ev[ctx->ev_used + k];
    ctx->ev_used += 3;
    return 0;
}

static int collect_timings(drt_context *ctx)
{
    for (size_t k = 0; k + 3 <= ctx->ev_used; k += 3)
    {
        float a = 0.f, b = 0.f;
        HIP_TRY(hipEventElapsedTime(&a, ctx->ev[k], ctx->ev[k + 1]));
        HIP_TRY(hipEventElapsedTime(&b, ctx->ev[k + 1], ctx->ev[k + 2]));
        ctx->trace_ms += a;
        ctx->shade_ms += b;
        const double paths = k / 3 < ctx->ev_paths.size() ? ctx->ev_paths[k / 3] : 0.0;
        if (paths > 0.0)
        {
            const double t = ((double)a + (double)b) * (double)ctx->n_pix / paths;
            if (ctx->timed_pairs == 0 || t < ctx->min_sample_ms) ctx->min_sample_ms = t;
            if (ctx->timed_pairs == 0 || t > ctx->max_sample_ms) ctx->max_sample_ms = t;
            ctx->timed_pairs += 1;
            ctx->avg_sample_ms += (t - ctx->avg_sample_ms) / (double)ctx->timed_pairs;
        }
// ... 527 lines not shown
    return 0;
}

extern "C" int drt_read_bgra(drt_context *ctx, int which, uint8_t *bgra)
{
    if (!ctx || !bgra) return fail(-1, "null argument");
    int rc = film_to_bgra(ctx, which);
    if (rc) return rc;
    HIP_TRY(hipMemcpy(bgra, ctx->d_bgra, (size_t)ctx->n_pix * 4, hipMemcpyDeviceToHost));
    return 0;
}

extern "C" int drt_read_hit_indices(drt_context *ctx, int32_t *dst, uint64_t capacity_paths)
{
    if (!ctx || !dst) return fail(-1, "null argument");
    if (!(ctx->params.flags & DRT_FLAG_RECORD_HITS) || !ctx->d_hits) return fail(-4, "hit recording is off (DRT_FLAG_RECORD_HITS)");
    int rc = drt_synchronize(ctx);
    if (rc) return rc;
    uint64_t n = std::min<uint64_t>(capacity_paths, ctx->n_pix * (uint64_t)ctx->hits_samples);
    HIP_TRY(hipMemcpy(dst, ctx->d_hits, n * ctx->params.max_depth * sizeof(int32_t), hipMemcpyDeviceToHost));
    return 0;
}

extern "C" int drt_get_stats(drt_context *ctx, drt_stats *out)
{
    if (!ctx || !out) return fail(-1, "null argument");
    int rc = drt_synchronize(ctx);
    if (rc) return rc;
    unsigned long long c[DRT_NUM_COUNTERS];
    HIP_TRY(hipMemcpy(c, ctx->d_counters, sizeof(c), hipMemcpyDeviceToHost));
    memset(out, 0, sizeof(*out));
    out->paths = c[0];
    out->closest_hit_scans = c[1];
    out->shaded_vertices = c[2];
    out->shadow_scans = c[3];
    out->rng_draws = c[4];
    out->trace_ms = ctx->trace_ms;
    out->shade_ms = ctx->shade_ms;
    out->total_ms = ctx->trace_ms + ctx->shade_ms;
    out->record_pool_blocks = ctx->pool_blocks;
    out->record_pool_peak = ctx->pool_peak;
    out->record_block_bytes = ctx->block_words * 8;
    out->redone_launches = (uint32_t)ctx->redone_batches;
    out->launches = (uint32_t)std::min<uint64_t>(ctx->timed_pairs, 0xFFFFFFFFull);
    out->path_flags = (ctx->bvh_pipeline ? DRT_PATH_BVH : 0u) | ((ctx->trace_tail && ctx->d_tail_stage) ? DRT_PATH_TRACE_TAIL : 0u) |
                      (ctx->rays_bound ? DRT_PATH_RAYS : 0u) | ((ctx->trace_stash && !ctx->bvh_pipeline) ? DRT_PATH_RAY_STASH : 0u);
    out->min_sample_ms = ctx->min_sample_ms;
    out->max_sample_ms = ctx->max_sample_ms;
    out->avg_sample_ms = ctx->avg_sample_ms;
    return 0;
}

extern "C" uint32_t drt_batch_spp(drt_context *ctx) { return ctx ? ctx->batch_spp : 0; }

static void window_out(const LiveWindow &w, uint32_t out[4]) { out[0] = w.x_lo; out[1] = w.x_hi; out[2] = w.y_lo; out[3] = w.y_hi; }

extern "C" int drt_live_window_of(const drt_scene *scene, const drt_camera *camera, const drt_params *params, uint32_t out[4])
{
    g_last_error.clear();
    if (!scene || !camera || !params || !out) return fail(-1, "drt_live_window_of: null argument");
    if (scene->escape_material >= scene->num_materials) return fail(-2, "base/escape material index out of range");
    if ((uint64_t)params->x0 + params->tile_w > params->width ||
        (params->tile_h && (uint64_t)params->y0 + (uint64_t)(params->tile_h - 1) * (params->row_stride ? params->row_stride : 1) >= params->height))
        return fail(-1, "tile does not fit the %ux%u image", params->width, params->height);
    drt_params p = *params;
    if (p.row_stride == 0) p.row_stride = 1;
    window_out(live_window_of(scene->surfaces, scene->num_surfaces, scene->materials[scene->escape_material], *camera, p), out);
    return 0;
}

extern "C" int drt_live_window(drt_context *ctx, uint32_t out[4])
{
    if (!ctx || !out) return fail(-1, "drt_live_window: null argument");
    window_refresh(ctx);
    window_out(ctx->win, out);
    return 0;
}

extern "C" int drt_shade_instantiation(const drt_context *ctx)
{
    if (!ctx) return -1;
    if (shade_closed(ctx)) return DRT_SHADE_CLOSED;
    return shade_simple(ctx) ? DRT_SHADE_SIMPLE : DRT_SHADE_GENERAL;
}

static int adaptive_check(drt_context *ctx, const drt_adaptive *a, bool held = false)
{
    if (!ctx || !a) return fail(-1, "null argument");
    if (ctx->n_cuts) return fail(-4, "adaptive sampling with depth cuts bound is not supported: drt_bind_depth_cuts(ctx, NULL, 0) first");
    if (ctx->n_sensor) return fail(-4, "adaptive sampling with a sensor bound is not supported: drt_bind_sensor(ctx, NULL, 0) first");
    if (ctx->n_buckets) return fail(-4, "adaptive sampling with buckets bound is not supported: drt_bind_buckets(ctx, 0) first");
    if (ctx->n_lobes) return fail(-4, "adaptive sampling with lobes bound is not supported: drt_bind_lobes(ctx, 0, NULL) first");
    if (ctx->xyz_mode) return fail(-4, "adaptive sampling needs the spectral film (DRT_MODE_XYZ keeps no variance)");
    if (ctx->params.flags & DRT_FLAG_RECORD_HITS) return fail(-4, "adaptive sampling does not record hit indices (DRT_FLAG_RECORD_HITS)");
    if (!held && ctx->adaptive_done) return fail(-7, "the film holds an adaptive render: drt_reset_film first");
    if (!held && ctx->film_used) return fail(-7, "adaptive sampling needs a film without samples: drt_reset_film first");
    if (held && !ctx->adaptive_done && !ctx->film_used) return fail(-7, "the film holds no samples to continue from: drt_render_adaptive renders from the start");
    if (a->min_spp < 2) return fail(-1, "min_spp %u: at least 2 (the variance needs two samples)", a->min_spp);
    if (a->max_spp < a->min_spp) return fail(-1, "max_spp %u is below min_spp %u", a->max_spp, a->min_spp);
    if (a->step < 1) return fail(-1, "step must be at least 1");
    if (a->flags != 0) return fail(-1, "flags %u: none are defined", a->flags);
    if (!std::isfinite(a->rel_error) || !(a->rel_error > 0.0)) return fail(-1, "rel_error %g: a finite number above 0", a->rel_error);
    if (!std::isfinite(a->floor) || !(a->floor >= 0.0)) return fail(-1, "floor %g: a finite number, 0 or more", a->floor);
    if (ctx->n_pix > 0xFFFFFFFFull) return fail(-1, "adaptive sampling lists pixels in 32 bits: the tile has %llu", (unsigned long long)ctx->n_pix);
    return 0;
}

static int enqueue_converge(drt_context *ctx)
{
    drt_context::Adaptive &ad = ctx->ad;
    const uint32_t n_blocks = (uint32_t)(((uint64_t)ad.n_in + CONVERGE_BLOCK - 1) / CONVERGE_BLOCK);
    ConvergeParams cp{};
    cp.list_in = ad.first ? nullptr : ctx->d_alist[ad.cur];
    cp.n_in = ad.n_in;
    cp.max_spp = ad.a.max_spp;
    cp.cmf_rw = ctx->cmf_rw;
    cp.cmf_y = ctx->cmf_y;
    cp.interval = ctx->interval;
    cp.rel_error = ad.a.rel_error;
    cp.floor = ad.a.floor;
    cp.counts = ctx->d_counts;
    cp.keep_mask = ctx->d_keep;
    cp.block_keep = ctx->d_bkeep;
    cp.active = ctx->d_bkeep + n_blocks;
    cp.list_out = ctx->d_alist[ad.cur ^ 1];
    cp.overflow = (const uint32_t *)(ctx->d_counters + DRT_NUM_COUNTERS + 5);
    cp.pixels = ctx->d_pixels;
    cp.at_max = ctx->d_ainfo;
    hipLaunchKernelGGL(drt_converge_kernel, dim3(n_blocks), dim3(CONVERGE_BLOCK), 0, ctx->stream, ctx->dsc, cp, ctx->d_avgs, ctx->d_vars);
    HIP_TRY(hipGetLastError());
    hipLaunchKernelGGL(drt_converge_scan, dim3(1), dim3(CONVERGE_SCAN_BLOCK), 0, ctx->stream, cp, n_blocks);
    HIP_TRY(hipGetLastError());
    hipLaunchKernelGGL(drt_converge_scatter, dim3(n_blocks), dim3(CONVERGE_BLOCK), 0, ctx->stream, cp);
    HIP_TRY(hipGetLastError());
    HIP_TRY(hipMemcpyAsync(ctx->h_active, cp.active, sizeof(uint32_t), hipMemcpyDeviceToHost, ctx->stream));
    HIP_TRY(hipMemcpyAsync(ctx->h_active + 1, ctx->d_ainfo, sizeof(uint32_t), hipMemcpyDeviceToHost, ctx->stream));
    return 0;
}

static int adaptive_alloc(drt_context *ctx)
{
    const uint64_t n_pix = ctx->n_pix;
    HIP_TRY(ctx->d_counts.need(n_pix));
    HIP_TRY(ctx->d_alist[0].need(n_pix));
    HIP_TRY(ctx->d_alist[1].need(n_pix));
    HIP_TRY(ctx->d_keep.need((n_pix + 63) / 64));
    HIP_TRY(ctx->d_bkeep.need((n_pix + CONVERGE_BLOCK - 1) / CONVERGE_BLOCK + 1));
    HIP_TRY(ctx->d_ainfo.need(1 + ADOPT_WORDS));
    HIP_TRY(ctx->h_active.need(2 + ADOPT_WORDS));
    return 0;
}

static int adaptive_buffers(drt_context *ctx)
{
    if (!ctx->h_active)
    {
        const int rc = adaptive_alloc(ctx);
        if (rc)
        {
            for (DevBuf<uint32_t> *b : {&ctx->d_counts, &ctx->d_alist[0], &ctx->d_alist[1], &ctx->d_bkeep, &ctx->d_ainfo}) b->reset();
            ctx->d_keep.reset();
            return rc;
        }
    }
    HIP_TRY(hipMemsetAsync(ctx->d_ainfo, 0, sizeof(uint32_t), ctx->stream));
    HIP_TRY(hipMemsetAsync(ctx->d_ainfo + 1 + ADOPT_BAD, 0xFF, sizeof(uint32_t), ctx->stream));
// ... 4042 lines not shown
```

daily-ray-trace_amd/pydrt.py:

```python
import ctypes as C
import os
import sys

import numpy as np

HERE = os.path.dirname(os.path.abspath(__file__))
REPO = os.path.dirname(HERE)

DRT_MAX_BDSFS = 16
GEO_POINT, GEO_SPHERE, GEO_PLANE = 1, 2, 3
FILM_SAMPLE_CENTER, FILM_SAMPLE_RANDOM = 1, 2
MODE_SPECTRAL, MODE_XYZ = 0, 1
FLAG_RECORD_HITS = 1
BATCH_RESIDENT = 0xFFFFFFFF
FLAG_FILM_ZERO = 2
PATH_BVH, PATH_TRACE_TAIL, PATH_RAYS, PATH_RAY_STASH = 1, 2, 4, 8

BDSF_NAMES = ["bp_diffuse_bdsf", "bp_glossy_bdsf", "mirror_bdsf", "fs_conductor_bdsf",
              "fs_dielectric_reflectance_bdsf", "fs_dielectric_transmittance_bdsf", "ct_conductor_bdsf"]
DIRF_NAMES = ["cos_weighted_sample_hemisphere", "uniform_sample_hemisphere", "sample_specular_direction",
              "sample_transmit_direction", "sample_reflect_or_transmit_direction", "sample_ct_direction"]
BDSF = {n: i for i, n in enumerate(BDSF_NAMES)}
DIRF = {n: i for i, n in enumerate(DIRF_NAMES)}

# ... 560 lines not shown
    global _hip
    if _hip is None:
        path = os.environ.get("DRT_HIP_LIB") or os.path.join(HERE, "libdrt_hip.so")
        if not os.path.exists(path):
            raise RuntimeError("libdrt_hip.so is not built (no fallback exists): run __graft_entry__.build()")
        _share_torch_hip_runtime()
        L = C.CDLL(path)
        L.drt_last_error.restype = C.c_char_p
        L.drt_device_count.restype = C.c_int
        L.drt_create.restype = C.c_void_p
        L.drt_create.argtypes = [C.POINTER(Scene), C.POINTER(Camera), C.POINTER(Params)]
        L.drt_destroy.argtypes = [C.c_void_p]
        L.drt_bind_film.argtypes = [C.c_void_p, C.c_void_p, C.c_void_p, C.c_void_p]
        L.drt_set_stream.argtypes = [C.c_void_p, C.c_void_p]
        L.drt_render.argtypes = [C.c_void_p, C.c_uint32, C.c_uint32]
        L.drt_synchronize.argtypes = [C.c_void_p]
        L.drt_reset_film.argtypes = [C.c_void_p]
        L.drt_film_device_ptrs.argtypes = [C.c_void_p, C.POINTER(C.c_void_p), C.POINTER(C.c_void_p), C.POINTER(C.c_void_p)]
        L.drt_read_film.argtypes = [C.c_void_p, C.POINTER(C.c_double), C.POINTER(C.c_double), C.POINTER(C.c_double)]
        L.drt_read_xyz.argtypes = [C.c_void_p, C.POINTER(C.c_double)]
        L.drt_read_bgra.argtypes = [C.c_void_p, C.c_int, C.POINTER(C.c_uint8)]
        L.drt_group_read_bgra.argtypes = [C.c_void_p, C.c_int, C.POINTER(C.c_uint8)]
        f64p, i32p = C.POINTER(C.c_double), C.POINTER(C.c_int32)
        L.drt_group_create.restype = C.c_void_p
        L.drt_group_create.argtypes = [C.POINTER(Scene), C.POINTER(Camera), C.POINTER(Params), i32p, C.c_uint32]
        L.drt_group_destroy.argtypes = [C.c_void_p]
        L.drt_group_destroy.restype = None
        L.drt_group_size.argtypes = [C.c_void_p]
        L.drt_group_size.restype = C.c_uint32
        L.drt_group_render.argtypes = [C.c_void_p, C.c_uint32, C.c_uint32]
        L.drt_group_synchronize.argtypes = [C.c_void_p]
        L.drt_group_read_film.argtypes = [C.c_void_p, f64p, f64p, f64p]
        L.drt_group_write_film.argtypes = [C.c_void_p, f64p, f64p, f64p]
        L.drt_group_get_stats.argtypes = [C.c_void_p, C.POINTER(Stats)]
        L.drt_render_tile_multi.argtypes = [C.POINTER(Scene), C.POINTER(Camera), C.POINTER(Params), i32p, C.c_uint32, f64p, f64p, f64p,
                                            C.POINTER(Stats)]
        L.drt_write_film.argtypes = [C.c_void_p, C.POINTER(C.c_double), C.POINTER(C.c_double), C.POINTER(C.c_double)]
        L.drt_read_hit_indices.argtypes = [C.c_void_p, C.POINTER(C.c_int32), C.c_uint64]
        L.drt_get_stats.argtypes = [C.c_void_p, C.POINTER(Stats)]
        L.drt_render_adaptive.argtypes = [C.c_void_p, C.POINTER(Adaptive)]
        L.drt_read_sample_counts.argtypes = [C.c_void_p, C.POINTER(C.c_uint32)]
        L.drt_read_active_list.argtypes = [C.c_void_p, C.POINTER(C.c_uint32), C.c_uint32, C.POINTER(C.c_uint32)]
        L.drt_group_render_adaptive.argtypes = [C.c_void_p, C.POINTER(Adaptive)]
        L.drt_group_read_sample_counts.argtypes = [C.c_void_p, C.POINTER(C.c_uint32)]
        L.drt_render_adaptive_continue.argtypes = [C.c_void_p, C.POINTER(Adaptive), C.c_uint32, C.POINTER(C.c_uint32)]
        L.drt_group_render_adaptive_continue.argtypes = [C.c_void_p, C.POINTER(Adaptive), C.c_uint32, C.POINTER(C.c_uint32)]
        if hasattr(L, "drt_render_sample_map"):
            L.drt_render_sample_map.argtypes = [C.c_void_p, C.POINTER(SampleMap)]
            L.drt_group_render_sample_map.argtypes = [C.c_void_p, C.POINTER(SampleMap)]
        if hasattr(L, "drt_denoise_film"):
            L.drt_denoise_film.argtypes = [C.c_void_p, C.POINTER(Denoise)]
            L.drt_read_denoised.argtypes = [C.c_void_p, f64p, f64p]
            L.drt_read_denoised_bgra.argtypes = [C.c_void_p, C.POINTER(C.c_uint8)]
            L.drt_denoise_buffers.argtypes = [C.POINTER(Scene), C.POINTER(Params), C.POINTER(Denoise), f64p, f64p, f64p, f64p, f64p]
            L.drt_group_denoise.argtypes = [C.c_void_p, C.POINTER(Denoise), f64p, f64p]
        if hasattr(L, "drt_render_features"):
            L.drt_render_features.argtypes = [C.c_void_p, C.POINTER(Features)]
            L.drt_read_features.argtypes = [C.c_void_p, f64p, f64p, i32p]
            L.drt_read_feature_bgra.argtypes = [C.c_void_p, C.c_int, C.c_double, C.c_double, C.POINTER(C.c_uint8)]
            L.drt_group_render_features.argtypes = [C.c_void_p, C.POINTER(Features), f64p, f64p, i32p]
        if hasattr(L, "drt_cast_rays"):
            vp = C.c_void_p
            L.drt_cast_rays.argtypes = [C.c_void_p, vp, vp, C.c_uint64, vp, C.c_uint32]
            L.drt_test_visibility.argtypes = [C.c_void_p, vp, vp, C.c_uint64, vp, C.c_uint32]
            L.drt_cast_pixels.argtypes = [C.c_void_p, vp, vp, C.c_uint64, vp, vp, vp, C.c_uint32]
            L.drt_group_cast_rays.argtypes = [C.c_void_p, vp, vp, C.c_uint64, vp]
            L.drt_group_test_visibility.argtypes = [C.c_void_p, vp, vp, C.c_uint64, vp]
            L.drt_group_cast_pixels.argtypes = [C.c_void_p, vp, vp, C.c_uint64, vp, vp, vp]
        if hasattr(L, "drt_render_mattes"):
            u32p = C.POINTER(C.c_uint32)
            L.drt_render_mattes.argtypes = [C.c_void_p, C.POINTER(Mattes)]
            L.drt_read_mattes.argtypes = [C.c_void_p, i32p, u32p, u32p]
            L.drt_read_matte.argtypes = [C.c_void_p, C.c_int, i32p, C.c_uint32, f64p]
            L.drt_read_matte_bgra.argtypes = [C.c_void_p, C.c_int, C.POINTER(C.c_uint8)]
            L.drt_group_render_mattes.argtypes = [C.c_void_p, C.POINTER(Mattes), i32p, u32p, u32p]
        L.drt_batch_spp.restype = C.c_uint32
        if hasattr(L, "drt_bind_rays"):
            L.drt_bind_rays.argtypes = [C.c_void_p, C.POINTER(RayTable)]
            L.drt_group_bind_rays.argtypes = [C.c_void_p, C.POINTER(RayTable)]
        L.drt_batch_spp.argtypes = [C.c_void_p]
        if hasattr(L, "drt_shade_instantiation"):
            L.drt_shade_instantiation.argtypes = [C.c_void_p]
            L.drt_shade_instantiation.restype = C.c_int
        if hasattr(L, "drt_update_surfaces"):
            L.drt_set_camera.argtypes = [C.c_void_p, C.POINTER(Camera)]
            L.drt_update_surfaces.argtypes = [C.c_void_p, C.c_void_p, C.c_uint32, C.c_uint32, C.c_uint32]
            L.drt_get_update_report.argtypes = [C.c_void_p, C.POINTER(UpdateReport)]
            L.drt_group_set_camera.argtypes = [C.c_void_p, C.POINTER(Camera)]
            L.drt_group_update_surfaces.argtypes = [C.c_void_p, C.c_void_p, C.c_uint32, C.c_uint32, C.c_uint32]
            L.drt_group_reset_film.argtypes = [C.c_void_p]
        if hasattr(L, "drt_update_spectra"):
            L.drt_update_spectra.argtypes = [C.c_void_p, C.c_void_p, C.c_uint32, C.c_uint32, C.c_uint32]
            L.drt_update_materials.argtypes = [C.c_void_p, C.c_void_p, C.c_uint32, C.c_uint32, C.c_uint32]
            L.drt_group_update_spectra.argtypes = [C.c_void_p, C.c_void_p, C.c_uint32, C.c_uint32, C.c_uint32]
            L.drt_group_update_materials.argtypes = [C.c_void_p, C.c_void_p, C.c_uint32, C.c_uint32, C.c_uint32]
        if hasattr(L, "drt_bind_depth_cuts"):
            u32p, vpp = C.POINTER(C.c_uint32), C.POINTER(C.c_void_p)
            L.drt_bind_depth_cuts.argtypes = [C.c_void_p, u32p, C.c_uint32]
            L.drt_read_depth_film.argtypes = [C.c_void_p, C.c_uint32, f64p, f64p, f64p]
            L.drt_depth_film_device_ptrs.argtypes = [C.c_void_p, C.c_uint32, vpp, vpp, vpp]
            L.drt_read_depth_xyz.argtypes = [C.c_void_p, C.c_uint32, f64p]
            L.drt_read_depth_bgra.argtypes = [C.c_void_p, C.c_uint32, C.c_int, C.POINTER(C.c_uint8)]
            L.drt_group_bind_depth_cuts.argtypes = [C.c_void_p, u32p, C.c_uint32]
            L.drt_group_read_depth_film.argtypes = [C.c_void_p, C.c_uint32, f64p, f64p, f64p]
        if hasattr(L, "drt_bind_sensor"):
            vpp = C.POINTER(C.c_void_p)
            L.drt_bind_sensor.argtypes = [C.c_void_p, f64p, C.c_uint32]
            L.drt_read_sensor_film.argtypes = [C.c_void_p, f64p, f64p, f64p]
            L.drt_sensor_film_device_ptrs.argtypes = [C.c_void_p, vpp, vpp, vpp]
            L.drt_read_sensor_bgra.argtypes = [C.c_void_p, C.c_int, f64p, C.POINTER(C.c_uint8)]
            L.drt_group_bind_sensor.argtypes = [C.c_void_p, f64p, C.c_uint32]
            L.drt_group_read_sensor_film.argtypes = [C.c_void_p, f64p, f64p, f64p]
        if hasattr(L, "drt_bind_buckets"):
            vpp, u8p = C.POINTER(C.c_void_p), C.POINTER(C.c_uint8)
            L.drt_bind_buckets.argtypes = [C.c_void_p, C.c_uint32]
            L.drt_read_bucket_film.argtypes = [C.c_void_p, C.c_uint32, f64p, f64p, f64p]
            L.drt_bucket_film_device_ptrs.argtypes = [C.c_void_p, C.c_uint32, vpp, vpp, vpp]
            L.drt_resolve_buckets.argtypes = [C.c_void_p, C.c_uint32]
            L.drt_read_bucket_resolve.argtypes = [C.c_void_p, f64p, f64p]
            L.drt_bucket_resolve_device_ptrs.argtypes = [C.c_void_p, vpp, vpp]
            L.drt_read_bucket_resolve_xyz.argtypes = [C.c_void_p, f64p]
            L.drt_read_bucket_resolve_bgra.argtypes = [C.c_void_p, u8p]
            L.drt_group_bind_buckets.argtypes = [C.c_void_p, C.c_uint32]
            L.drt_group_read_bucket_film.argtypes = [C.c_void_p, C.c_uint32, f64p, f64p, f64p]
            L.drt_group_resolve_buckets.argtypes = [C.c_void_p, C.c_uint32]
            L.drt_group_read_bucket_resolve.argtypes = [C.c_void_p, f64p, f64p]
        if hasattr(L, "drt_bind_lobes"):
            vpp, u8p, mapp = C.POINTER(C.c_void_p), C.POINTER(C.c_uint8), C.POINTER(LobeMap)
            L.drt_bind_lobes.argtypes = [C.c_void_p, C.c_uint32, mapp]
            L.drt_read_lobe_film.argtypes = [C.c_void_p, C.c_uint32, f64p, f64p, f64p]
            L.drt_lobe_film_device_ptrs.argtypes = [C.c_void_p, C.c_uint32, vpp, vpp, vpp]
            L.drt_read_lobe_xyz.argtypes = [C.c_void_p, C.c_uint32, f64p]
            L.drt_read_lobe_bgra.argtypes = [C.c_void_p, C.c_uint32, C.c_int, u8p]
            L.drt_group_bind_lobes.argtypes = [C.c_void_p, C.c_uint32, mapp]
            L.drt_group_read_lobe_film.argtypes = [C.c_void_p, C.c_uint32, f64p, f64p, f64p]
        if hasattr(L, "drt_rebuild_hierarchy"):
            L.drt_rebuild_hierarchy.argtypes = [C.c_void_p, C.c_uint32]
            L.drt_group_rebuild_hierarchy.argtypes = [C.c_void_p, C.c_uint32]
            L.drt_get_hierarchy_report.argtypes = [C.c_void_p, C.POINTER(HierarchyReport)]
            L.drt_read_hierarchy.argtypes = [C.c_void_p, C.c_void_p, C.c_uint32, C.POINTER(C.c_uint32), C.c_uint32]
        if hasattr(L, "drt_live_window_of"):
            L.drt_live_window_of.argtypes = [C.POINTER(Scene), C.POINTER(Camera), C.POINTER(Params), C.POINTER(C.c_uint32)]
            L.drt_live_window.argtypes = [C.c_void_p, C.POINTER(C.c_uint32)]
        L.drt_render_tile.argtypes = [C.POINTER(Scene), C.POINTER(Camera), C.POINTER(Params), C.POINTER(C.c_double),
                                      C.POINTER(C.c_double), C.POINTER(C.c_double), C.POINTER(Stats)]
        L.drt_selftest_arith.argtypes = [C.c_int, C.c_int, C.POINTER(C.c_double), C.POINTER(C.c_double),
                                         C.POINTER(C.c_double), C.c_uint64]
        if hasattr(L, "drt_selftest_path_ids"):
            L.drt_selftest_path_ids.argtypes = [C.c_int, C.POINTER(C.c_uint64), C.c_uint32, C.POINTER(C.c_uint32), C.c_uint32, C.c_uint32,
                                                C.c_uint32, C.POINTER(C.c_uint64)]
        L.drt_bvh_stats.argtypes = [C.POINTER(Scene)] + [C.POINTER(C.c_uint32)] * 4
        L.drt_selftest_unit.argtypes = [C.c_int, C.c_int, C.POINTER(C.c_double), C.c_uint32, C.POINTER(C.c_double), C.c_uint32,
                                        C.c_uint64]
        L.drt_selftest_material.argtypes = [C.c_void_p, C.c_int, C.POINTER(C.c_double), C.c_uint32, C.POINTER(C.c_double), C.c_uint32,
                                            C.c_uint64]
        if hasattr(L, "drt_selftest_build_sort"):
            u32p, u64p = C.POINTER(C.c_uint32), C.POINTER(C.c_uint64)
            L.drt_selftest_build_sort.argtypes = [C.c_int, u64p, C.c_uint32, u64p, u32p]
            L.drt_selftest_build_topology.argtypes = [C.c_int, u64p, C.c_uint32, C.POINTER(C.c_int32), C.POINTER(C.c_int32), u32p, u32p]
        if hasattr(L, "drt_selftest_live_resources"):
            L.drt_selftest_live_resources.argtypes = [C.POINTER(C.c_uint64)]
        if hasattr(L, "drt_selftest_division"):
            L.drt_selftest_division.argtypes = [C.c_int, C.c_int, C.POINTER(C.c_double), C.c_uint32, C.POINTER(C.c_double), C.c_uint32,
                                                C.c_uint64]
        _hip = L
    return _hip


SHADE_INSTANTIATIONS = ("general", "simple", "closed")

HIP_SYMBOLS = ["drt_shade_instantiation",
               "drt_last_error", "drt_device_count", "drt_create", "drt_destroy", "drt_bind_film", "drt_set_stream",
               "drt_render", "drt_synchronize", "drt_reset_film", "drt_film_device_ptrs", "drt_read_film", "drt_write_film",
               "drt_read_xyz", "drt_read_bgra", "drt_read_hit_indices", "drt_get_stats", "drt_batch_spp", "drt_render_tile", "drt_selftest_arith",
               "drt_selftest_unit", "drt_selftest_material", "drt_selftest_path_ids", "drt_bvh_stats",
               "drt_selftest_build_sort", "drt_selftest_build_topology", "drt_selftest_live_resources",
               "drt_group_create", "drt_group_destroy", "drt_group_size", "drt_group_render", "drt_group_synchronize",
               "drt_group_read_film", "drt_group_write_film", "drt_group_read_bgra", "drt_group_get_stats", "drt_render_tile_multi",
               "drt_render_adaptive", "drt_read_sample_counts", "drt_group_render_adaptive", "drt_group_read_sample_counts",
               "drt_read_active_list", "drt_render_adaptive_continue", "drt_group_render_adaptive_continue",
               "drt_denoise_film", "drt_read_denoised", "drt_read_denoised_bgra", "drt_denoise_buffers", "drt_group_denoise",
               "drt_render_features", "drt_read_features", "drt_read_feature_bgra", "drt_group_render_features",
               "drt_render_mattes", "drt_read_mattes", "drt_read_matte", "drt_read_matte_bgra", "drt_group_render_mattes",
               "drt_cast_rays", "drt_test_visibility", "drt_cast_pixels", "drt_group_cast_rays", "drt_group_test_visibility",
               "drt_group_cast_pixels", "drt_bind_rays", "drt_group_bind_rays",
               "drt_set_camera", "drt_update_surfaces", "drt_get_update_report", "drt_group_set_camera", "drt_group_update_surfaces",
               "drt_group_reset_film",
               "drt_rebuild_hierarchy", "drt_group_rebuild_hierarchy", "drt_get_hierarchy_report", "drt_read_hierarchy",
               "drt_update_spectra", "drt_update_materials", "drt_group_update_spectra", "drt_group_update_materials",
               "drt_bind_depth_cuts", "drt_read_depth_film", "drt_depth_film_device_ptrs", "drt_read_depth_xyz", "drt_read_depth_bgra",
               "drt_group_bind_depth_cuts", "drt_group_read_depth_film",
               "drt_bind_sensor", "drt_read_sensor_film", "drt_sensor_film_device_ptrs", "drt_read_sensor_bgra",
               "drt_group_bind_sensor", "drt_group_read_sensor_film",
               "drt_bind_buckets", "drt_read_bucket_film", "drt_bucket_film_device_ptrs", "drt_resolve_buckets", "drt_read_bucket_resolve",
               "drt_bucket_resolve_device_ptrs", "drt_read_bucket_resolve_xyz", "drt_read_bucket_resolve_bgra",
               "drt_group_bind_buckets", "drt_group_read_bucket_film", "drt_group_resolve_buckets", "drt_group_read_bucket_resolve",
               "drt_bind_lobes", "drt_read_lobe_film", "drt_lobe_film_device_ptrs", "drt_read_lobe_xyz", "drt_read_lobe_bgra",
               "drt_group_bind_lobes", "drt_group_read_lobe_film",
               "drt_render_sample_map", "drt_group_render_sample_map",
               "drt_live_window_of", "drt_live_window", "drt_selftest_division"]

MAX_DEPTH_CUTS = 8


def _depth_array(depths):
    depths = [] if depths is None else [int(d) for d in depths]
    if any(d < 0 or d > 0xFFFFFFFF for d in depths):
        raise ValueError("bind_depth_cuts: depths are unsigned 32-bit numbers")
    return ((C.c_uint32 * len(depths))(*depths) if depths else None), len(depths)


MAX_SENSOR_CHANNELS = 8


def _sensor_curves(curves, S):
    if curves is None:
        return None, 0
    a = np.ascontiguousarray(curves, dtype=np.float64)
    if a.ndim == 1 and a.size == 0:
        return None, 0
    if a.ndim != 2 or a.shape[1] != S:
        raise ValueError("bind_sensor: curves of shape %s, need [n][%d] (one value per wavelength of the render's grid)" % (a.shape, S))
    if a.shape[0] == 0:
        return None, 0
    return a, int(a.shape[0])


def _sensor_matrix(matrix, n):
    m = np.ascontiguousarray(matrix, dtype=np.float64)
    if m.shape != (3, n):
        raise ValueError("read_sensor_bgra: a matrix of shape %s, need (3, %d): the bound channels to R, G, B" % (m.shape, n))
    return m


MAX_BUCKETS = 8


def _u32(value, what):
    v = int(value)
    if v < 0 or v > 0xFFFFFFFF:
        raise ValueError("%s = %d: an unsigned 32-bit number" % (what, v))
    return v


def bucket_pair(means):
    m = np.asarray(means, dtype=np.float64)
    if m.ndim < 1 or m.shape[0] < 2:
        raise ValueError("bucket_pair: means of shape %s, need [n][...] with n >= 2 buckets" % (m.shape,))
    out = []
    for half in (m[0::2], m[1::2]):
        acc = half[0].copy()
        for k in range(1, half.shape[0]):
            acc = acc + half[k]
        out.append(acc / float(half.shape[0]))
# ... 243 lines not shown
        a, b = C.c_void_p(), C.c_void_p()
        _check(self.L.drt_bucket_resolve_device_ptrs(self.ctx, C.byref(a), C.byref(b)), "drt_bucket_resolve_device_ptrs")
        return a.value, b.value

    def read_bucket_resolve_xyz(self):
        out = np.empty((self.n_pixels, 3))
        _check(self.L.drt_read_bucket_resolve_xyz(self.ctx, _ptr(out, C.c_double)), "drt_read_bucket_resolve_xyz")
        return out

    def read_bucket_resolve_bgra(self):
        out = np.empty((self.n_pixels, 4), dtype=np.uint8)
        _check(self.L.drt_read_bucket_resolve_bgra(self.ctx, _ptr(out, C.c_uint8)), "drt_read_bucket_resolve_bgra")
        return out

    def bind_lobes(self, map_or_preset, n=None):
        n, m = _lobe_bind_args(map_or_preset, n)
        _check(self.L.drt_bind_lobes(self.ctx, n, C.byref(m) if m is not None else None), "drt_bind_lobes")
        self.n_lobes = n

    def read_lobe_film(self, c):
        c = _u32(c, "read_lobe_film: c")
        if not getattr(self, "n_lobes", 0) or c >= self.n_lobes:
            _check(self.L.drt_read_lobe_film(self.ctx, c, None, None, None), "drt_read_lobe_film")
        S, n = self.S, self.n_pixels
        px, av, va = np.empty((n, S + 1)), np.empty((n, S)), np.empty((n, S))
        _check(self.L.drt_read_lobe_film(self.ctx, c, _ptr(px, C.c_double), _ptr(av, C.c_double), _ptr(va, C.c_double)), "drt_read_lobe_film")
        return px, av, va

    def lobe_film_device_ptrs(self, c):
        a, b, d = C.c_void_p(), C.c_void_p(), C.c_void_p()
        _check(self.L.drt_lobe_film_device_ptrs(self.ctx, _u32(c, "lobe_film_device_ptrs: c"), C.byref(a), C.byref(b), C.byref(d)),
               "drt_lobe_film_device_ptrs")
        return a.value, b.value, d.value

    def read_lobe_xyz(self, c):
        out = np.empty((self.n_pixels, 3))
        _check(self.L.drt_read_lobe_xyz(self.ctx, _u32(c, "read_lobe_xyz: c"), _ptr(out, C.c_double)), "drt_read_lobe_xyz")
        return out

    def read_lobe_bgra(self, c, which=1):
        out = np.empty((self.n_pixels, 4), dtype=np.uint8)
        _check(self.L.drt_read_lobe_bgra(self.ctx, _u32(c, "read_lobe_bgra: c"), int(which), _ptr(out, C.c_uint8)), "drt_read_lobe_bgra")
        return out

    def bind_sensor(self, curves):
        arr, n = _sensor_curves(curves, self.S)
        _check(self.L.drt_bind_sensor(self.ctx, None if arr is None else _ptr(arr, C.c_double), n), "drt_bind_sensor")
        self.n_sensor = n

    def read_sensor_film(self):
        n = getattr(self, "n_sensor", 0)
        px = np.empty((self.n_pixels, n + 1), dtype=np.float64)
        av = np.empty((self.n_pixels, n), dtype=np.float64)
        va = np.empty((self.n_pixels, n), dtype=np.float64)
        _check(self.L.drt_read_sensor_film(self.ctx, _ptr(px, C.c_double), _ptr(av, C.c_double), _ptr(va, C.c_double)), "drt_read_sensor_film")
        return px, av, va

    def sensor_film_device_ptrs(self):
        a, b, c = C.c_void_p(), C.c_void_p(), C.c_void_p()
        _check(self.L.drt_sensor_film_device_ptrs(self.ctx, C.byref(a), C.byref(b), C.byref(c)), "drt_sensor_film_device_ptrs")
        return a.value, b.value, c.value

    def read_sensor_bgra(self, which, matrix):
        n = getattr(self, "n_sensor", 0)
        if n == 0:
            _check(self.L.drt_read_sensor_bgra(self.ctx, int(which), None, None), "drt_read_sensor_bgra")
        m = _sensor_matrix(matrix, n)
        out = np.empty((self.n_pixels, 4), dtype=np.uint8)
        _check(self.L.drt_read_sensor_bgra(self.ctx, int(which), _ptr(m, C.c_double), _ptr(out, C.c_uint8)), "drt_read_sensor_bgra")
        return out

    def read_hit_indices(self, num_samples):
        n = self.n_pixels * num_samples
        out = np.empty((n, int(self.params.max_depth)), dtype=np.int32)
        _check(self.L.drt_read_hit_indices(self.ctx, _ptr(out, C.c_int32), n), "drt_read_hit_indices")
        return out

    def batch_spp(self):
        return int(self.L.drt_batch_spp(self.ctx))

    def shade_instantiation(self):
        return SHADE_INSTANTIATIONS[int(self.L.drt_shade_instantiation(self.ctx))]

    def stats(self):
        st = Stats()
        _check(self.L.drt_get_stats(self.ctx, C.byref(st)), "drt_get_stats")
        return st

    def render_adaptive(self, min_spp, max_spp, step, rel_error, floor=0.0):
        a = make_adaptive(min_spp, max_spp, step, rel_error, floor)
        _check(self.L.drt_render_adaptive(self.ctx, C.byref(a)), "drt_render_adaptive")
        return {"rounds": a.rounds, "pixels_at_max": a.pixels_at_max, "paths": a.paths}

    def render_adaptive_continue(self, max_spp, step, rel_error, floor=0.0, max_rounds=0):
        a = make_adaptive(2, max_spp, step, rel_error, floor)
        left = C.c_uint32()
        _check(self.L.drt_render_adaptive_continue(self.ctx, C.byref(a), max_rounds, C.byref(left)), "drt_render_adaptive_continue")
        return {"rounds": a.rounds, "pixels_at_max": a.pixels_at_max, "paths": a.paths, "still_active": left.value}

    def denoise(self, radius=5, patch=1, k=1.0, alpha=1.0):
        d = make_denoise(radius, patch, k, alpha)
        _check(self.L.drt_denoise_film(self.ctx, C.byref(d)), "drt_denoise_film")
        return {"unusable": d.unusable, "kernel_ms": d.kernel_ms}

    def read_denoised(self):
        mean = np.empty((self.n_pixels, self.S), dtype=np.float64)
        var = np.empty((self.n_pixels, self.S), dtype=np.float64)
        _check(self.L.drt_read_denoised(self.ctx, _ptr(mean, C.c_double), _ptr(var, C.c_double)), "drt_read_denoised")
        return mean, var

    def read_denoised_bgra(self):
        out = np.empty((self.n_pixels, 4), dtype=np.uint8)
        _check(self.L.drt_read_denoised_bgra(self.ctx, _ptr(out, C.c_uint8)), "drt_read_denoised_bgra")
        return out

    def render_features(self, n_samples=0, first_sample=0, flags=0):
        f = make_features(n_samples, first_sample)
        f.flags = flags
        _check(self.L.drt_render_features(self.ctx, C.byref(f)), "drt_render_features")
        return {"empty_pixels": f.empty_pixels, "rays": f.rays, "kernel_ms": f.kernel_ms}

    def read_features(self):
        mean = np.empty((self.n_pixels, FEATURE_CHANNELS), dtype=np.float64)
        m2 = np.empty((self.n_pixels, FEATURE_CHANNELS), dtype=np.float64)
        ids = np.empty(self.n_pixels, dtype=np.int32)
        _check(self.L.drt_read_features(self.ctx, _ptr(mean, C.c_double), _ptr(m2, C.c_double), _ptr(ids, C.c_int32)), "drt_read_features")
        return mean, m2, ids

    def read_feature_bgra(self, which, lo, hi):
        out = np.empty((self.n_pixels, 4), dtype=np.uint8)
        _check(self.L.drt_read_feature_bgra(self.ctx, int(which), float(lo), float(hi), _ptr(out, C.c_uint8)), "drt_read_feature_bgra")
        return out

    def render_mattes(self, n_samples=0, first_sample=0, flags=0):
        m = make_mattes(n_samples, first_sample)
        m.flags = flags
        _check(self.L.drt_render_mattes(self.ctx, C.byref(m)), "drt_render_mattes")
        return _mattes_report(m)

    def read_mattes(self):
        ids = np.empty((self.n_pixels, MATTE_LAYERS, MATTE_SLOTS), dtype=np.int32)
        counts = np.empty((self.n_pixels, MATTE_LAYERS, MATTE_SLOTS), dtype=np.uint32)
        tail = np.empty((self.n_pixels, 4), dtype=np.uint32)
        _check(self.L.drt_read_mattes(self.ctx, _ptr(ids, C.c_int32), _ptr(counts, C.c_uint32), _ptr(tail, C.c_uint32)), "drt_read_mattes")
        return ids, counts, tail

    def read_matte(self, layer, id_list):
        lst = np.ascontiguousarray(id_list, dtype=np.int32).reshape(-1)
        out = np.empty(self.n_pixels, dtype=np.float64)
        _check(self.L.drt_read_matte(self.ctx, int(layer), _ptr(lst, C.c_int32), len(lst), _ptr(out, C.c_double)), "drt_read_matte")
        return out

    def read_matte_bgra(self, layer):
        out = np.empty((self.n_pixels, 4), dtype=np.uint8)
        _check(self.L.drt_read_matte_bgra(self.ctx, int(layer), _ptr(out, C.c_uint8)), "drt_read_matte_bgra")
        return out

    def cast_rays(self, origins, dirs):
        if _is_tensor(origins) or _is_tensor(dirs):
            torch = sys.modules["torch"]
            dev = int(self.params.device)
            o, d = _rays_tensor(origins, "origins", dev), _rays_tensor(dirs, "dirs", dev)
            if o.shape != d.shape:
                raise ValueError("origins and dirs: the same shape")
            hits = torch.empty((o.shape[0], 104), dtype=torch.uint8, device=o.device)
            _check(self.L.drt_cast_rays(self.ctx, o.data_ptr(), d.data_ptr(), o.shape[0], hits.data_ptr(), RAYS_DEVICE), "drt_cast_rays")
# ... 526 lines not shown
```

include/drt_hip.h:

```cpp
#ifndef DRT_HIP_H
#define DRT_HIP_H

#include <stdint.h>

#ifdef __cplusplus
extern "C" {
#endif

#define DRT_MAX_BDSFS 16

enum
{
    DRT_GEO_NONE   = 0,
    DRT_GEO_POINT  = 1,
    DRT_GEO_SPHERE = 2,
    DRT_GEO_PLANE  = 3
};

enum
{
    DRT_FILM_SAMPLE_CENTER = 1,
    DRT_FILM_SAMPLE_RANDOM = 2
};

// ... 76 lines not shown
} drt_camera;

enum
{
    DRT_MODE_SPECTRAL = 0,
    DRT_MODE_XYZ      = 1
};

typedef struct drt_params
{
    uint32_t width, height;
    uint32_t x0, y0, tile_w, tile_h, row_stride;
    uint32_t spp;
    uint32_t first_sample;
    uint32_t max_depth;
    uint32_t pixel_scheme;
    uint64_t seed;
    uint32_t mode;
    int32_t  device;
    uint32_t batch_spp;
    uint32_t flags;
} drt_params;

#define DRT_BATCH_RESIDENT 0xFFFFFFFFu

enum
{
    DRT_FLAG_RECORD_HITS = 1u,
    DRT_FLAG_FILM_ZERO   = 2u
};

typedef struct drt_stats
{
    uint64_t paths;
    uint64_t closest_hit_scans;
    uint64_t shaded_vertices;
    uint64_t shadow_scans;
    uint64_t rng_draws;
    double   trace_ms;
    double   shade_ms;
    double   total_ms;
    uint64_t record_pool_blocks;
    uint64_t record_pool_peak;
    uint32_t record_block_bytes;
    uint32_t redone_launches;
    uint32_t launches;
    uint32_t path_flags;
    double   min_sample_ms, max_sample_ms, avg_sample_ms;
} drt_stats;

enum
{
    DRT_PATH_BVH        = 1u,
    DRT_PATH_TRACE_TAIL = 2u,
    DRT_PATH_RAYS       = 4u,
    DRT_PATH_RAY_STASH  = 8u
};

typedef struct drt_context drt_context;

const char *drt_last_error(void);
int drt_device_count(void);

drt_context *drt_create(const drt_scene *scene, const drt_camera *camera, const drt_params *params);
void         drt_destroy(drt_context *ctx);
int drt_bind_film(drt_context *ctx, void *d_pixels, void *d_avgs, void *d_vars);
int drt_set_stream(drt_context *ctx, void *hip_stream);
int drt_render(drt_context *ctx, uint32_t first_sample, uint32_t num_samples);
int drt_synchronize(drt_context *ctx);
int drt_reset_film(drt_context *ctx);
int drt_film_device_ptrs(drt_context *ctx, void **d_pixels, void **d_avgs, void **d_vars);
int drt_read_film(drt_context *ctx, double *pixels, double *avgs, double *vars);
int drt_write_film(drt_context *ctx, const double *pixels, const double *avgs, const double *vars);
int drt_read_xyz(drt_context *ctx, double *xyz);
int drt_read_bgra(drt_context *ctx, int which, uint8_t *bgra);
int drt_read_hit_indices(drt_context *ctx, int32_t *dst, uint64_t capacity_paths);
int drt_get_stats(drt_context *ctx, drt_stats *out);
uint32_t drt_batch_spp(drt_context *ctx);

#define DRT_SHADE_GENERAL 0
#define DRT_SHADE_SIMPLE 1
#define DRT_SHADE_CLOSED 2
int drt_shade_instantiation(const drt_context *ctx);

int drt_render_tile(const drt_scene *scene, const drt_camera *camera, const drt_params *params,
                    double *dst_pixels, double *dst_avgs, double *dst_vars, drt_stats *stats);

typedef struct drt_group drt_group;
drt_group *drt_group_create(const drt_scene *scene, const drt_camera *camera, const drt_params *params,
                            const int32_t *devices, uint32_t n_devices);
void     drt_group_destroy(drt_group *g);
uint32_t drt_group_size(drt_group *g);
int drt_group_render(drt_group *g, uint32_t first_sample, uint32_t num_samples);
int drt_group_synchronize(drt_group *g);
int drt_group_read_film(drt_group *g, double *pixels, double *avgs, double *vars);
int drt_group_write_film(drt_group *g, const double *pixels, const double *avgs, const double *vars);
int drt_group_read_bgra(drt_group *g, int which, uint8_t *bgra);
int drt_group_get_stats(drt_group *g, drt_stats *out);
int drt_render_tile_multi(const drt_scene *scene, const drt_camera *camera, const drt_params *params,
                          const int32_t *devices, uint32_t n_devices,
                          double *dst_pixels, double *dst_avgs, double *dst_vars, drt_stats *stats);

typedef struct drt_adaptive
{
    uint32_t min_spp, max_spp, step, flags;
    double   rel_error, floor;
    uint32_t rounds, pixels_at_max;
    uint64_t paths;
} drt_adaptive;
int drt_render_adaptive(drt_context *ctx, drt_adaptive *a);
int drt_read_sample_counts(drt_context *ctx, uint32_t *counts);
int drt_read_active_list(drt_context *ctx, uint32_t *list, uint32_t capacity, uint32_t *count);
int drt_group_render_adaptive(drt_group *g, drt_adaptive *a);
int drt_group_read_sample_counts(drt_group *g, uint32_t *counts);

int drt_render_adaptive_continue(drt_context *ctx, drt_adaptive *a, uint32_t max_rounds, uint32_t *still_active);
int drt_group_render_adaptive_continue(drt_group *g, drt_adaptive *a, uint32_t max_rounds, uint32_t *still_active);

#define DRT_MAP_DEVICE 1u
#define DRT_MAP_ADD    2u
typedef struct drt_sample_map
{
    const uint32_t *targets;
    uint32_t flags;
    uint32_t rounds, pixels_rendered, pixels_above, max_count;
    uint64_t paths;
} drt_sample_map;
int drt_render_sample_map(drt_context *ctx, drt_sample_map *map);
int drt_group_render_sample_map(drt_group *g, drt_sample_map *map);

typedef struct drt_denoise
{
    uint32_t radius, patch, flags;
    uint32_t unusable;
    double   k, alpha;
    double   kernel_ms;
} drt_denoise;
int drt_denoise_film(drt_context *ctx, drt_denoise *d);
int drt_read_denoised(drt_context *ctx, double *mean, double *var);
int drt_read_denoised_bgra(drt_context *ctx, uint8_t *bgra);
int drt_denoise_buffers(const drt_scene *scene, const drt_params *params, drt_denoise *d, const double *pixels, const double *avgs,
                        const double *vars, double *mean, double *var);
int drt_group_denoise(drt_group *g, drt_denoise *d, double *mean, double *var);

#define DRT_FEATURE_CHANNELS 8
typedef struct drt_features
{
    uint32_t n_samples;
    uint32_t first_sample;
    uint32_t flags;
    uint32_t empty_pixels;
    uint64_t rays;
    double   kernel_ms;
} drt_features;
int drt_render_features(drt_context *ctx, drt_features *f);
int drt_read_features(drt_context *ctx, double *mean, double *m2, int32_t *ids);
int drt_read_feature_bgra(drt_context *ctx, int which, double lo, double hi, uint8_t *bgra);
int drt_group_render_features(drt_group *g, drt_features *f, double *mean, double *m2, int32_t *ids);

#define DRT_MATTE_SLOTS   6
#define DRT_MATTE_ID_MISS (-1)
enum { DRT_MATTE_SURFACE = 0, DRT_MATTE_MATERIAL = 1, DRT_MATTE_LAYERS = 2 };
typedef struct drt_mattes
{
    uint32_t n_samples;
    uint32_t first_sample;
// ... 148 lines not shown
```

Before: 2301.

## Stage shade headers in LDS for the closed-form kernel to cut register pressure

Adds a closed-form shade kernel variant that writes per-sample header words into a per-wave LDS region and reads them back with broadcast loads, replacing repeated cross-lane readlane extraction. It uses a single prefetch slot instead of a double buffer and shrinks the tail window so the per-wave LDS footprint stays bounded. The variant is picked on the host when an LDS budgeting rule says enough groups fit per CU, and the grid cap is clamped to that rule. The goal is fewer live VGPRs and higher waves per SIMD, at the cost of extra LDS traffic, wave barriers, and a smaller tail window.

Measured after the change: 2552, median of 6. +10.9%, better.

```diff
diff --git a/daily-ray-trace_amd/csrc/drt_kernels.h b/daily-ray-trace_amd/csrc/drt_kernels.h
--- a/daily-ray-trace_amd/csrc/drt_kernels.h
+++ b/daily-ray-trace_amd/csrc/drt_kernels.h
@@ -1802,6 +1802,33 @@
     return (uint64_t)lo | ((uint64_t)hi << 32);
 }
 
+__device__ __forceinline__ uint64_t first64(uint64_t v)
+{
+    uint32_t lo = (uint32_t)__builtin_amdgcn_readfirstlane((int)(uint32_t)v);
+    uint32_t hi = (uint32_t)__builtin_amdgcn_readfirstlane((int)(uint32_t)(v >> 32));
+    return (uint64_t)lo | ((uint64_t)hi << 32);
+}
+
+template <bool AGAIN>
+__device__ __forceinline__ uint32_t made_again(uint32_t v)
+{
+    if constexpr (AGAIN) asm volatile("" : "+v"(v));
+    return v;
+}
+
+template <bool FROM_LDS>
+__device__ __forceinline__ uint64_t lifted_word(const uint64_t *at, uint64_t v, uint32_t l)
+{
+    if constexpr (FROM_LDS) return first64(*at);
+    else return readlane64(v, l);
+}
+template <bool FROM_LDS>
+__device__ __forceinline__ double lifted_double(const uint64_t *at, uint64_t v, uint32_t l)
+{
+    if constexpr (FROM_LDS) return word_as_double(*at);
+    else return word_as_double(readlane64(v, l));
+}
+
 __device__ __forceinline__ const uint64_t *path_vertex(const uint64_t *__restrict__ pool, uint32_t block_words, uint32_t vw, uint64_t h2, uint64_t h3, uint32_t v)
 {
     const uint32_t b = v >> REC_BLOCK_SHIFT;
@@ -1896,6 +1923,16 @@
 #define TAIL_WINDOW_ENTRIES 112u
 #define TAIL_WINDOW_WORDS (3u * TAIL_WINDOW_ENTRIES + TAIL_WINDOW_ENTRIES / 4u)
 #define SHADE_WAVE_LDS_WORDS ((2u * 64u * SHADE_PREFETCH_REGS) > TAIL_WINDOW_WORDS ? (2u * 64u * SHADE_PREFETCH_REGS) : TAIL_WINDOW_WORDS)
+#ifndef DRT_SHADE_CLOSED_LDS_HEADERS
+#define DRT_SHADE_CLOSED_LDS_HEADERS 1
+#endif
+#define SHADE_CLOSED_SLOT_WORDS (64u * SHADE_PREFETCH_REGS)
+#define SHADE_CLOSED_HDR01_AT SHADE_CLOSED_SLOT_WORDS
+#define SHADE_CLOSED_HDR2_AT (SHADE_CLOSED_HDR01_AT + 128u)
+#define SHADE_CLOSED_TAIL_ENTRIES 96u
+#define SHADE_CLOSED_WAVE_LDS_WORDS (SHADE_CLOSED_HDR2_AT + 64u)
+static_assert(3u * SHADE_CLOSED_TAIL_ENTRIES + SHADE_CLOSED_TAIL_ENTRIES / 4u <= SHADE_CLOSED_WAVE_LDS_WORDS, "the tail pass's window fits the closed form's region");
+#define SHADE_WAVE_LDS_WORDS_FOR(closed_lds) ((closed_lds) ? SHADE_CLOSED_WAVE_LDS_WORDS : SHADE_WAVE_LDS_WORDS)
 
 #define XYZ_FILM_WORDS 8
 
@@ -1903,7 +1940,7 @@
 __device__ __forceinline__ void shade_tail_group(const DevScene &sc, const ShadeParams &sp, const double *lds, uint64_t *wave_lds, const uint64_t *__restrict__ records,
                                                  const uint64_t *__restrict__ headers, double *__restrict__ film_pixels,
                                                  double *__restrict__ film_avgs, double *__restrict__ film_vars, uint64_t chunk_base,
-                                                 uint64_t chunk_end, uint32_t lane, const bool closed)
+                                                 uint64_t chunk_end, uint32_t lane, const bool closed, const bool closed_lds = false)
 {
     const uint32_t S = sc.S;
     const uint32_t vw = sp.vertex_words;
@@ -1913,8 +1950,9 @@
     const uint32_t lam = sp.tail_first + j;
     const double *table = SPDS_IN_LDS ? (const double *)lds : sc.spds;
     const uint32_t n_groups = 64u / R;
-    const uint32_t win = TAIL_WINDOW_ENTRIES / n_groups;
-    uint16_t *task_list = (uint16_t *)(wave_lds + 3u * TAIL_WINDOW_ENTRIES);
+    const uint32_t entries = closed_lds ? SHADE_CLOSED_TAIL_ENTRIES : TAIL_WINDOW_ENTRIES;
+    const uint32_t win = entries / n_groups;
+    uint16_t *task_list = (uint16_t *)(wave_lds + 3u * entries);
     const uint32_t leader = g * R;
     const bool in_group = g < n_groups;
     uint32_t v = 0, n_shaded = 0;
@@ -2202,7 +2240,7 @@
 }
 
 
-template <int NSETS, bool SPDS_IN_LDS, bool XYZ, bool DARK, bool SIMPLE, bool LIST, bool CLOSED>
+template <int NSETS, bool SPDS_IN_LDS, bool XYZ, bool DARK, bool SIMPLE, bool LIST, bool CLOSED, bool CLOSED_LDS = false>
 __device__ __forceinline__ void shade_pixels(const DevScene &sc, const ShadeParams &sp, const uint64_t *__restrict__ records,
                                              const uint64_t *__restrict__ headers, double *__restrict__ film_pixels,
                                              double *__restrict__ film_avgs, double *__restrict__ film_vars,
@@ -2218,8 +2256,10 @@
         for (uint32_t k = threadIdx.x; k < spd_words; k += SHADE_BLOCK) lds[k] = sc.spds[k];
         __syncthreads();
     }
-    const uint32_t lane = threadIdx.x & 63u;
-    uint64_t *rec_lds = (uint64_t *)(lds + (SPDS_IN_LDS ? (size_t)sc.n_spd * S : 0)) + (size_t)(threadIdx.x >> 6) * SHADE_WAVE_LDS_WORDS;
+    const uint32_t lane_k = threadIdx.x & 63u;
+    static_assert(!CLOSED_LDS || CLOSED, "the form with headers in LDS is a closed form");
+    constexpr bool LDS_HDR = CLOSED_LDS;
+    uint64_t *rec_lds = (uint64_t *)(lds + (SPDS_IN_LDS ? (size_t)sc.n_spd * S : 0)) + (size_t)(threadIdx.x >> 6) * SHADE_WAVE_LDS_WORDS_FOR(LDS_HDR);
     const uint32_t vw = sp.vertex_words;
     const uint32_t vpr = vw <= 64 ? 64u / vw : 0u;
     const uint32_t n_fast_regs = vpr * SHADE_PREFETCH_REGS;
@@ -2229,7 +2269,7 @@
 #pragma unroll
     for (int k = 0; k < NSETS; k += 1)
     {
-        const uint32_t lam = 64u * k + lane;
+        const uint32_t lam = 64u * k + lane_k;
         lam_c[k] = lam < S ? lam : 0;
     }
 
@@ -2238,9 +2278,11 @@
     {
         const ShadeParams &qc = shade_const().sp;
         uint32_t item = 0;
-        if (lane == 0) item = (uint32_t)atomicAdd(work_counter, 1ull);
+        if (lane_k == 0) item = (uint32_t)atomicAdd(work_counter, 1ull);
         item = (uint32_t)__builtin_amdgcn_readfirstlane((int)item);
         if (item >= qc.n_items) break;
+        const uint32_t lane = made_again<LDS_HDR>(lane_k);
+        if constexpr (LDS_HDR) lam_c[0] = lane < S ? lane : 0;
         const bool split = qc.items_per_group > 1;
         const bool inline_tail = qc.tail_count != 0;
         const uint32_t mains_per_group = qc.items_per_group - (inline_tail ? 1u : 0u);
@@ -2321,14 +2363,12 @@
             h0 = h[0];
             h1 = h[1];
             h2 = h[2];
-            h3 = h[3];
+            if (!LDS_HDR) h3 = h[3];
         }
         const unsigned long long worthless = !DARK ? 0ull : __ballot(lane < n_win && (h0 & 0xFFFFu) == 0ull && ((uint32_t)(h0 >> 16) & HDR_TERM_MASK) != 1u &&
                                                                       __builtin_isfinite(word_as_double(h1)));
         if (DARK && dark && (uint32_t)__popcll(worthless) == n_win) continue;
-        auto prefetch = [&](uint32_t sa, uint32_t nw, uint64_t *dst) {
-            if (nw == 0u) return;
-            const uint64_t b2 = readlane64(h2, sa);
+        auto prefetch_blocks = [&](uint64_t b2, uint32_t nw, uint64_t *dst) __attribute__((always_inline)) {
 #pragma unroll
             for (int k = 0; k < SHADE_PREFETCH_REGS; k += 1)
             {
@@ -2338,22 +2378,69 @@
                 dst[k] = (64u * k + lane < nw) ? base[lane] : 0;
             }
         };
+        auto prefetch = [&](uint32_t sa, uint32_t nw, uint64_t *dst) {
+            if (nw == 0u) return;
+            prefetch_blocks(readlane64(h2, sa), nw, dst);
+        };
         uint64_t ring[SHADE_PREFETCH_DEPTH + 1][SHADE_PREFETCH_REGS];
+        const uint64_t *hdr01 = rec_lds + SHADE_CLOSED_HDR01_AT, *hdr2 = rec_lds + SHADE_CLOSED_HDR2_AT;
+        uint64_t hs_v = 0, vig_v = 0, nx0_v = 0, nx2_v = 0;
+        auto fetch_headers = [&](uint32_t t) {
+            const uint32_t a = t & 63u, b = (t + 1u) & 63u;
+            hs_v = hdr01[a];
+            vig_v = hdr01[64u + a];
+            nx0_v = hdr01[b];
+            nx2_v = hdr2[b];
+        };
+        if constexpr (LDS_HDR)
+        {
+            static_assert(SHADE_PREFETCH_DEPTH == 1, "one sample ahead");
+            __builtin_amdgcn_wave_barrier();
+            uint64_t *hw = rec_lds + SHADE_CLOSED_HDR01_AT;
+            hw[lane] = h0;
+            hw[64u + lane] = h1;
+            hw[128u + lane] = h2;
+            __builtin_amdgcn_wave_barrier();
+            fetch_headers(0u);
+            const uint64_t head0 = first64(hs_v);
+            const uint32_t nw = (uint32_t)(head0 & 0xFFFFu) * vw;
+            if (nw != 0u) prefetch_blocks(first64(hdr2[0]), nw, ring[1]);
+        }
+        else
+        {
 #pragma unroll
         for (int d = 0; d < SHADE_PREFETCH_DEPTH; d += 1)
         {
             const uint32_t nw = ((uint32_t)d < n_win) ? (uint32_t)(readlane64(h0, d) & 0xFFFFu) * vw : 0u;
             prefetch((uint32_t)d < n_win ? (uint32_t)d : 0u, nw, ring[d + 1]);
         }
+        }
         for (uint32_t s = 0; s < n_win; s += 1)
         {
-            const uint64_t hs = readlane64(h0, s);
-            const double vignette = word_as_double(readlane64(h1, s));
+            const uint64_t hs = LDS_HDR ? first64(hs_v) : readlane64(h0, s);
+            const uint64_t vig_w = LDS_HDR ? vig_v : readlane64(h1, s);
+            const double vignette = word_as_double(vig_w);
             const uint32_t n_shaded = (uint32_t)(hs & 0xFFFFu);
             const uint32_t term = (uint32_t)(hs >> 16) & HDR_TERM_MASK;
             const uint32_t term_spd = (uint32_t)(hs >> 32) & 0xFFFFu;
             const uint32_t plastic_mask = (uint32_t)(hs >> 48);
             const uint32_t vis0_mask = (uint32_t)(hs >> 24) & 0xFFu;
+            uint64_t w1_first = 0;
+            if constexpr (LDS_HDR)
+            {
+                if (n_shaded != 0u)
+                {
+                    w1_first = readlane64(ring[1][0], 1u);
+                    uint64_t *slot_now = rec_lds;
+#pragma unroll
+                    for (int k = 0; k < SHADE_PREFETCH_REGS; k += 1) slot_now[64u * k + lane] = ring[1][k];
+                }
+                const uint64_t next0 = first64(nx0_v);
+                const uint32_t nw = (s + 1u < n_win) ? (uint32_t)(next0 & 0xFFFFu) * vw : 0u;
+                if (nw != 0u) prefetch_blocks(first64(nx2_v), nw, ring[1]);
+            }
+            else
+            {
 #pragma unroll
             for (int d = 0; d < SHADE_PREFETCH_DEPTH; d += 1)
 #pragma unroll
@@ -2363,15 +2450,24 @@
                 const uint32_t nw = (sa < n_win) ? (uint32_t)(readlane64(h0, sa) & 0xFFFFu) * vw : 0u;
                 prefetch(sa < n_win ? sa : 0u, nw, ring[SHADE_PREFETCH_DEPTH]);
             }
+            }
             const uint64_t *cur = ring[0];
+            if constexpr (!LDS_HDR)
+            {
             if (n_shaded != 0u)
             {
                 uint64_t *slot_now = rec_lds + (s & 1u) * (64u * SHADE_PREFETCH_REGS);
 #pragma unroll
                 for (int k = 0; k < SHADE_PREFETCH_REGS; k += 1) slot_now[64u * k + lane] = ring[0][k];
             }
-            const uint64_t *rec_words = rec_lds + (s & 1u) * (64u * SHADE_PREFETCH_REGS);
-            if (DARK && dark && ((worthless >> s) & 1ull) != 0ull) continue;
+            }
+            const uint64_t *rec_words = rec_lds + (LDS_HDR ? 0u : (s & 1u) * (64u * SHADE_PREFETCH_REGS));
+            if (DARK && dark && ((worthless >> s) & 1ull) != 0ull)
+            {
+                if constexpr (LDS_HDR) fetch_headers(s + 1u);
+                continue;
+            }
+            const uint64_t *head3_at = headers + ((pix * sp.batch + s0 + s) * REC_HEADER_WORDS + 3);
 
             double throughput[NSETS], dst[NSETS];
 #pragma unroll
@@ -2413,21 +2509,34 @@
                     throughput[0] = throughput[0] * reflectance;
                 };
                 const uint32_t run0 = run < vpr ? run : vpr;
+                if constexpr (LDS_HDR)
+                {
+                    uint64_t w1 = w1_first;
+                    for (uint32_t v = 0; v < run; v += 1)
+                    {
+                        const uint64_t w1_next = rec_words[((v + 1u) * vw + 1u) & (SHADE_CLOSED_SLOT_WORDS - 1u)];
+                        run_vertex(w1, rec_words + v * vw, ((vis0_mask >> v) & 1u) != 0u);
+                        w1 = first64(w1_next);
+                    }
+                }
+                else
+                {
                 for (uint32_t v = 0; v < run0; v += 1)
                     run_vertex(readlane64(cur[0], v * vw + 1u), rec_words + v * vw, ((vis0_mask >> v) & 1u) != 0u);
                 for (uint32_t v = run0; v < run; v += 1)
                     run_vertex(readlane64(cur[SHADE_PREFETCH_REGS > 1 ? 1 : 0], (v - vpr) * vw + 1u), rec_words + v * vw, ((vis0_mask >> v) & 1u) != 0u);
+                }
                 v_first = run;
                 if (run == n_fast && n_shaded > run && vw * REC_BLOCK_VERTICES == 64u)
                 {
-                    const uint64_t h3s = readlane64(h3, s);
+                    const uint64_t h3s = lifted_word<LDS_HDR>(head3_at, h3, s);
                     for (uint32_t b = n_fast / REC_BLOCK_VERTICES; b * REC_BLOCK_VERTICES < n_shaded && b < 4u; b += 1)
                     {
                         uint32_t id = (uint32_t)h3s;
-                        if (b == 1u) id = (uint32_t)(readlane64(h2, s) >> 32);
+                        if (b == 1u) id = (uint32_t)(lifted_word<LDS_HDR>(hdr2 + s, h2, s) >> 32);
                         if (b >= REC_HEADER_BLOCKS) id = ((const uint32_t *)(records + (uint64_t)(uint32_t)(h3s >> 32) * sp.block_words))[b - REC_HEADER_BLOCKS];
                         const uint64_t blockw = records[(uint64_t)id * sp.block_words + lane];
-                        uint64_t *slot = rec_lds + (s & 1u) * (64u * SHADE_PREFETCH_REGS);
+                        uint64_t *slot = rec_lds + (LDS_HDR ? 0u : (s & 1u) * (64u * SHADE_PREFETCH_REGS));
                         slot[lane] = blockw;
                         const uint32_t v_lo = b * REC_BLOCK_VERTICES;
                         const uint32_t v_hi = n_shaded < v_lo + REC_BLOCK_VERTICES ? n_shaded : v_lo + REC_BLOCK_VERTICES;
@@ -2448,7 +2557,15 @@
             {
                 uint64_t src;
                 uint32_t lane0;
-                if (v < n_fast)
+                uint32_t vbase = 0;
+                if constexpr (LDS_HDR)
+                {
+                    lane0 = 0;
+                    src = 0;
+                    if (v < n_fast) vbase = v * vw;
+                    else rec_lds[lane] = (lane < vw) ? path_vertex(records, sp.block_words, vw, lifted_word<LDS_HDR>(hdr2 + s, h2, s), lifted_word<LDS_HDR>(head3_at, h3, s), v)[lane] : 0;
+                }
+                else if (v < n_fast)
                 {
                     const uint32_t sel = v / vpr;
                     lane0 = (v - sel * vpr) * vw;
@@ -2458,8 +2575,9 @@
                 else
                 {
                     lane0 = 0;
-                    src = (lane < vw) ? path_vertex(records, sp.block_words, vw, readlane64(h2, s), readlane64(h3, s), v)[lane] : 0;
-                }
+                    src = (lane < vw) ? path_vertex(records, sp.block_words, vw, lifted_word<LDS_HDR>(hdr2 + s, h2, s), lifted_word<LDS_HDR>(head3_at, h3, s), v)[lane] : 0;
+                }
+                const uint64_t *vslot = rec_words + vbase;
                 const double *table = SPDS_IN_LDS ? (const double *)lds : sc.spds;
                 double contribution[NSETS];
 #pragma unroll
@@ -2500,11 +2618,11 @@
                             if (off + REC_LIGHT_WORDS <= 64 || v < n_fast)
                             {
 #pragma unroll
-                                for (int k = 0; k < 4; k += 1) lw[k] = readlane64(src, lane0 + off + k);
+                                for (int k = 0; k < 4; k += 1) lw[k] = lifted_word<LDS_HDR>(vslot + off + k, src, lane0 + off + k);
                             }
                             else
                             {
-                                const uint64_t *lp = path_vertex(records, sp.block_words, vw, readlane64(h2, s), readlane64(h3, s), v) + off;
+                                const uint64_t *lp = path_vertex(records, sp.block_words, vw, lifted_word<LDS_HDR>(hdr2 + s, h2, s), lifted_word<LDS_HDR>(head3_at, h3, s), v) + off;
 #pragma unroll
                                 for (int k = 0; k < 4; k += 1) lw[k] = readlane64(lp[k], 0);
                             }
@@ -2533,28 +2651,28 @@
                 };
                 if (v < 16u && ((plastic_mask >> v) & 1u))
                 {
-                    const uint64_t w1p = readlane64(src, lane0 + 1);
+                    const uint64_t w1p = lifted_word<LDS_HDR>(vslot + 1, src, lane0 + 1);
                     if (v < n_fast)
                     {
                         const uint64_t *vwords = rec_words + v * vw;
                         plastic_vertex(w1p, word_as_double(vwords[4]), word_as_double(vwords[5]), word_as_double(vwords[6]));
                         continue;
                     }
-                    const double dir_pdf_p = word_as_double(readlane64(src, lane0 + 4));
-                    const double s_a_in_p = word_as_double(readlane64(src, lane0 + 5)), s_spec_p = word_as_double(readlane64(src, lane0 + 6));
+                    const double dir_pdf_p = lifted_double<LDS_HDR>(vslot + 4, src, lane0 + 4);
+                    const double s_a_in_p = lifted_double<LDS_HDR>(vslot + 5, src, lane0 + 5), s_spec_p = lifted_double<LDS_HDR>(vslot + 6, src, lane0 + 6);
                     plastic_vertex(w1p, dir_pdf_p, s_a_in_p, s_spec_p);
                     continue;
                 }
-                const uint64_t list = readlane64(src, lane0 + 0);
-                const uint64_t w1 = readlane64(src, lane0 + 1);
+                const uint64_t list = lifted_word<LDS_HDR>(vslot + 0, src, lane0 + 0);
+                const uint64_t w1 = lifted_word<LDS_HDR>(vslot + 1, src, lane0 + 1);
                 const uint32_t num_bdsfs = (uint32_t)(w1 & 0xFFu);
                 const uint32_t sflags = (uint32_t)(w1 >> 8) & 0xFFu;
                 auto fixed_vertex = [&](uint32_t kind) {
                     const bool fresnel = !SIMPLE && kind != 0u;
                     constexpr bool GGX_BODY = CLOSED;
                     const bool rough = GGX_BODY && kind == 3u;
-                    const bool in_lds = v < n_fast;
-                    const uint64_t *vwords = rec_words + v * vw;
+                    const bool in_lds = LDS_HDR || v < n_fast;
+                    const uint64_t *vwords = rec_words + (LDS_HDR ? vbase : v * vw);
                     uint32_t i_r0 = (uint32_t)(w1 >> 48) & 0xFFFFu, i_r1 = 0, i_r2 = 0;
                     bool paired = false;
                     double on_dot = 0.0;
@@ -2564,8 +2682,8 @@
                     for (int k = 0; k < NSETS; k += 1) r1[k] = r2[k] = 0.0;
                     if (fresnel)
                     {
-                        fresnel_rows(readlane64(src, lane0 + 2), i_r0, i_r1, i_r2, paired);
-                        if (!rough) on_dot = in_lds ? word_as_double(vwords[3]) : word_as_double(readlane64(src, lane0 + 3));
+                        fresnel_rows(lifted_word<LDS_HDR>(vslot + 2, src, lane0 + 2), i_r0, i_r1, i_r2, paired);
+                        if (!rough) on_dot = in_lds ? word_as_double(vwords[3]) : lifted_double<LDS_HDR>(vslot + 3, src, lane0 + 3);
 #pragma unroll
                         for (int k = 0; k < NSETS; k += 1)
                         {
@@ -2592,17 +2710,17 @@
                         double c;
                         if (off + REC_LIGHT_WORDS <= 64 || v < n_fast)
                         {
-                            lw0 = readlane64(src, lane0 + off);
-                            c = in_lds ? word_as_double(vwords[off + 1u]) : word_as_double(readlane64(src, lane0 + off + 1u));
+                            lw0 = lifted_word<LDS_HDR>(vslot + off, src, lane0 + off);
+                            c = in_lds ? word_as_double(vwords[off + 1u]) : lifted_double<LDS_HDR>(vslot + off + 1u, src, lane0 + off + 1u);
                             if (rough)
                             {
-                                on_dot = in_lds ? word_as_double(vwords[off + 4u]) : word_as_double(readlane64(src, lane0 + off + 4u));
-                                ct = in_lds ? word_as_double(vwords[off + 5u]) : word_as_double(readlane64(src, lane0 + off + 5u));
+                                on_dot = in_lds ? word_as_double(vwords[off + 4u]) : lifted_double<LDS_HDR>(vslot + off + 4u, src, lane0 + off + 4u);
+                                ct = in_lds ? word_as_double(vwords[off + 5u]) : lifted_double<LDS_HDR>(vslot + off + 5u, src, lane0 + off + 5u);
                             }
                         }
                         else
                         {
-                            const uint64_t *lp = path_vertex(records, sp.block_words, vw, readlane64(h2, s), readlane64(h3, s), v) + off;
+                            const uint64_t *lp = path_vertex(records, sp.block_words, vw, lifted_word<LDS_HDR>(hdr2 + s, h2, s), lifted_word<LDS_HDR>(head3_at, h3, s), v) + off;
                             lw0 = readlane64(lp[0], 0);
                             c = word_as_double(lp[1]);
                             if (rough)
@@ -2625,15 +2743,15 @@
                     }
                     if (rough)
                     {
-                        on_dot = in_lds ? word_as_double(vwords[7]) : word_as_double(readlane64(src, lane0 + 7));
-                        ct = in_lds ? word_as_double(vwords[8]) : word_as_double(readlane64(src, lane0 + 8));
+                        on_dot = in_lds ? word_as_double(vwords[7]) : lifted_double<LDS_HDR>(vslot + 7, src, lane0 + 7);
+                        ct = in_lds ? word_as_double(vwords[8]) : lifted_double<LDS_HDR>(vslot + 8, src, lane0 + 8);
                     }
 #pragma unroll
                     for (int k = 0; k < NSETS; k += 1)
                     {
                         dst[k] = dst[k] + throughput[k] * contribution[k];
                         double reflectance = eval(k, sflags);
-                        const double dir_pdf = in_lds ? word_as_double(vwords[4]) : word_as_double(readlane64(src, lane0 + 4));
+                        const double dir_pdf = in_lds ? word_as_double(vwords[4]) : lifted_double<LDS_HDR>(vslot + 4, src, lane0 + 4);
                         reflectance = reflectance * dir_pdf;
                         throughput[k] = throughput[k] * reflectance;
                     }
@@ -2641,7 +2759,7 @@
                 if (CLOSED)
                 {
                     if (sflags & FLAG_PLASTIC)
-                        plastic_vertex(w1, word_as_double(readlane64(src, lane0 + 4)), word_as_double(readlane64(src, lane0 + 5)), word_as_double(readlane64(src, lane0 + 6)));
+                        plastic_vertex(w1, lifted_double<LDS_HDR>(vslot + 4, src, lane0 + 4), lifted_double<LDS_HDR>(vslot + 5, src, lane0 + 5), lifted_double<LDS_HDR>(vslot + 6, src, lane0 + 6));
                     else
                         fixed_vertex(list == DRT_LIST_MIRROR ? 0u : list == DRT_LIST_GLASS ? 1u : list == DRT_LIST_CONDUCTOR ? 2u : 3u);
                     continue;
@@ -2658,15 +2776,15 @@
                         continue;
                     }
                 }
-                const uint64_t w2 = readlane64(src, lane0 + 2);
-                const double on_dot = word_as_double(readlane64(src, lane0 + 3));
-                const double dir_pdf = word_as_double(readlane64(src, lane0 + 4));
+                const uint64_t w2 = lifted_word<LDS_HDR>(vslot + 2, src, lane0 + 2);
+                const double on_dot = lifted_double<LDS_HDR>(vslot + 3, src, lane0 + 3);
+                const double dir_pdf = lifted_double<LDS_HDR>(vslot + 4, src, lane0 + 4);
                 const uint32_t i_diffuse = (uint32_t)(w1 >> 16) & 0xFFFFu, i_glossy = (uint32_t)(w1 >> 32) & 0xFFFFu;
                 const uint32_t i_mirror = (uint32_t)(w1 >> 48) & 0xFFFFu;
                 uint32_t i_ir, i_tr, i_te;
                 bool paired;
                 fresnel_rows(w2, i_ir, i_tr, i_te, paired);
-                const double s_a_in = word_as_double(readlane64(src, lane0 + 5)), s_spec = word_as_double(readlane64(src, lane0 + 6));
+                const double s_a_in = lifted_double<LDS_HDR>(vslot + 5, src, lane0 + 5), s_spec = lifted_double<LDS_HDR>(vslot + 6, src, lane0 + 6);
 
                 if (sflags & FLAG_PLASTIC)
                 {
@@ -2690,11 +2808,11 @@
                     if (off + REC_LIGHT_WORDS <= 64 || v < n_fast)
                     {
 #pragma unroll
-                        for (int k = 0; k < REC_LIGHT_WORDS; k += 1) lw[k] = readlane64(src, lane0 + off + k);
+                        for (int k = 0; k < REC_LIGHT_WORDS; k += 1) lw[k] = lifted_word<LDS_HDR>(vslot + off + k, src, lane0 + off + k);
                     }
                     else
                     {
-                        const uint64_t *lp = path_vertex(records, sp.block_words, vw, readlane64(h2, s), readlane64(h3, s), v) + off;
+                        const uint64_t *lp = path_vertex(records, sp.block_words, vw, lifted_word<LDS_HDR>(hdr2 + s, h2, s), lifted_word<LDS_HDR>(head3_at, h3, s), v) + off;
 #pragma unroll
                         for (int k = 0; k < REC_LIGHT_WORDS; k += 1) lw[k] = readlane64(lp[k], 0);
                     }
@@ -2713,7 +2831,7 @@
                         contribution[k] = contribution[k] * c;
                     }
                 }
-                const double s_mn = word_as_double(readlane64(src, lane0 + 7)), s_ct = word_as_double(readlane64(src, lane0 + 8));
+                const double s_mn = lifted_double<LDS_HDR>(vslot + 7, src, lane0 + 7), s_ct = lifted_double<LDS_HDR>(vslot + 8, src, lane0 + 8);
 #pragma unroll
                 for (int k = 0; k < NSETS; k += 1)
                 {
@@ -2724,6 +2842,7 @@
                     throughput[k] = throughput[k] * reflectance;
                 }
             }
+            if constexpr (LDS_HDR) fetch_headers(s + 1u);
             const double denom = (double)(first + s0 + s + 1);
             if (DARK) dark = false;
 #pragma unroll
@@ -2796,7 +2915,11 @@
         }
       }
 
-        if (tail_item && sp.mode != 1u) shade_tail_group<SPDS_IN_LDS, XYZ, SIMPLE, LIST>(sc, sp, (const double *)lds, rec_lds, records, headers, film_pixels, film_avgs, film_vars, chunk_base, chunk_end, lane, CLOSED);
+        if constexpr (LDS_HDR)
+        {
+            __builtin_amdgcn_wave_barrier();
+        }
+        if (tail_item && sp.mode != 1u) shade_tail_group<SPDS_IN_LDS, XYZ, SIMPLE, LIST>(sc, sp, (const double *)lds, rec_lds, records, headers, film_pixels, film_avgs, film_vars, chunk_base, chunk_end, made_again<LDS_HDR>(lane), CLOSED, LDS_HDR);
     }
 }
 
@@ -2820,6 +2943,20 @@
 {
     shade_pixels<1, true, false, DARK, false, false, true>(sc, sp, records, headers, film_pixels, film_avgs, film_vars, work_counter);
 }
+
+#ifndef DRT_SHADE_WAVES_CLOSED_LDS
+#define DRT_SHADE_WAVES_CLOSED_LDS 5
+#endif
+#if DRT_SHADE_CLOSED_LDS_HEADERS
+template <bool DARK>
+__global__ __launch_bounds__(SHADE_BLOCK, DRT_SHADE_WAVES_CLOSED_LDS) void drt_shade_kernel_closed_lds(DevScene sc, ShadeParams sp, const uint64_t *__restrict__ records,
+                                                                 const uint64_t *__restrict__ headers, double *__restrict__ film_pixels,
+                                                                 double *__restrict__ film_avgs, double *__restrict__ film_vars,
+                                                                 unsigned long long *__restrict__ work_counter)
+{
+    shade_pixels<1, true, false, DARK, false, false, true, true>(sc, sp, records, headers, film_pixels, film_avgs, film_vars, work_counter);
+}
+#endif
 
 __global__ void drt_film_xyz_kernel(DevScene sc, uint32_t cmf_rw, uint32_t cmf_x, uint32_t cmf_y, uint32_t cmf_z, double interval,
                                     uint64_t n_pix, const double *__restrict__ film_pixels, double *__restrict__ xyz)
diff --git a/daily-ray-trace_amd/csrc/drt_launcher.hip b/daily-ray-trace_amd/csrc/drt_launcher.hip
--- a/daily-ray-trace_amd/csrc/drt_launcher.hip
+++ b/daily-ray-trace_amd/csrc/drt_launcher.hip
@@ -16,6 +16,7 @@
 #include "drt_window_kernels.h"
 #include "drt_window_rule.h"
 #include "drt_pair_rule.h"
+#include "drt_shade_lds_rule.h"
 #include "drt_owned.h"
 
 #include <algorithm>
@@ -134,6 +135,8 @@
 
     bool   scene_in_lds = true, spds_in_lds = true, use_bvh = false;
     size_t trace_lds = 0, shade_lds = 0;
+    size_t shade_lds_closed = 0;
+    bool   closed_lds = false;
     bool trace_stash = false;
     int    trace_grid_cap = 0, shade_grid_cap = 0;
     uint32_t trace_chunk_override = 0;
@@ -818,16 +821,26 @@
     return ctx->closed_lists && !ctx->no_closed_shade && !ctx->no_fixed_lists && !shade_simple(ctx) && ctx->spds_in_lds && ctx->shade_sets == 1 && !ctx->xyz_mode;
 }
 
+static bool shade_closed_lds(const drt_context *ctx) { return DRT_SHADE_CLOSED_LDS_HEADERS != 0 && ctx->closed_lds && shade_closed(ctx); }
+
 template <int NSETS, bool XYZ, bool LIST>
 static int launch_shade_mode(drt_context *ctx, uint32_t grid, const ShadeParams &sp, double *const film[3])
 {
     if (NSETS == 1 && !XYZ && !LIST && shade_closed(ctx))
     {
-#define DRT_LAUNCH_CLOSED(DARK)                                                                                                                    \
-    hipLaunchKernelGGL((drt_shade_kernel_closed<DARK>), dim3(grid), dim3(SHADE_BLOCK), ctx->shade_lds, ctx->stream, ctx->dsc, sp, ctx->d_records, \
+#define DRT_LAUNCH_CLOSED(KERNEL, DARK, LDS_BYTES)                                                                                                 \
+    hipLaunchKernelGGL((KERNEL<DARK>), dim3(grid), dim3(SHADE_BLOCK), LDS_BYTES, ctx->stream, ctx->dsc, sp, ctx->d_records, \
                        ctx->d_headers, film[0], film[1], film[2], ctx->d_counters + DRT_NUM_COUNTERS + 1)
-        if (shade_dark(ctx, sp)) DRT_LAUNCH_CLOSED(true);
-        else DRT_LAUNCH_CLOSED(false);
+#if DRT_SHADE_CLOSED_LDS_HEADERS
+        if (shade_closed_lds(ctx))
+        {
+            if (shade_dark(ctx, sp)) DRT_LAUNCH_CLOSED(drt_shade_kernel_closed_lds, true, ctx->shade_lds_closed);
+            else DRT_LAUNCH_CLOSED(drt_shade_kernel_closed_lds, false, ctx->shade_lds_closed);
+            return 0;
+        }
+#endif
+        if (shade_dark(ctx, sp)) DRT_LAUNCH_CLOSED(drt_shade_kernel_closed, true, ctx->shade_lds);
+        else DRT_LAUNCH_CLOSED(drt_shade_kernel_closed, false, ctx->shade_lds);
 #undef DRT_LAUNCH_CLOSED
         return 0;
     }
@@ -1068,6 +1081,11 @@
 template <int NSETS, bool XYZ>
 static int shade_occupancy_mode(drt_context *ctx, int *per_cu)
 {
+#if DRT_SHADE_CLOSED_LDS_HEADERS
+    if (NSETS == 1 && !XYZ && shade_closed_lds(ctx))
+        HIP_TRY(hipOccupancyMaxActiveBlocksPerMultiprocessor(per_cu, drt_shade_kernel_closed_lds<true>, SHADE_BLOCK, ctx->shade_lds_closed));
+    else
+#endif
     if (NSETS == 1 && !XYZ && shade_closed(ctx))
         HIP_TRY(hipOccupancyMaxActiveBlocksPerMultiprocessor(per_cu, drt_shade_kernel_closed<true>, SHADE_BLOCK, ctx->shade_lds));
     else if (NSETS == 1 && shade_simple(ctx))
@@ -1296,8 +1314,11 @@
         ctx->primary_grid_cap = prop.multiProcessorCount * std::max(1, p_cu);
         ctx->bounce_grid_cap = prop.multiProcessorCount * std::max(1, b_cu);
     }
-    ctx->shade_lds = ctx->spds_in_lds ? (size_t)ctx->dsc.n_spd * S * 8 : 0;
-    ctx->shade_lds += (size_t)SHADE_WAVES * SHADE_WAVE_LDS_WORDS * 8;
+    const ShadeLdsPlan lds_general = shade_lds_plan(ctx->dsc.n_spd, S, ctx->spds_in_lds, SHADE_WAVES, SHADE_WAVE_LDS_WORDS_FOR(false), DRT_SHADE_WAVES_PER_SIMD);
+    const ShadeLdsPlan lds_closed = shade_lds_plan(ctx->dsc.n_spd, S, ctx->spds_in_lds, SHADE_WAVES, SHADE_WAVE_LDS_WORDS_FOR(true), DRT_SHADE_WAVES_CLOSED_LDS);
+    ctx->shade_lds = lds_general.group_bytes;
+    ctx->shade_lds_closed = lds_closed.group_bytes;
+    ctx->closed_lds = lds_closed.groups >= DRT_SHADE_WAVES_CLOSED_LDS * SHADE_SIMDS_PER_CU / SHADE_WAVES && getenv("DRT_NO_CLOSED_LDS") == nullptr;
     int s_per_cu = 0;
     shade_sets(S, &ctx->shade_sets, &ctx->tail_first, &ctx->tail_count);
     switch (ctx->shade_sets)
@@ -1308,6 +1329,8 @@
         default: rc = shade_occupancy<4>(ctx, &s_per_cu); break;
     }
     if (rc) return rc;
+    const int s_query = s_per_cu;
+    if (shade_closed_lds(ctx)) s_per_cu = std::min(s_per_cu, (int)lds_closed.groups);
     if (s_per_cu < 1) s_per_cu = 1;
     if (const char *e = getenv("DRT_SHADE_BLOCKS_PER_CU")) s_per_cu = std::max(1, atoi(e));
     ctx->shade_grid_cap = prop.multiProcessorCount * s_per_cu;
@@ -1417,8 +1440,10 @@
     if (ctx->tail_count && ctx->tail_resume) HIP_TRY(ctx->d_tail_resume.need((size_t)npx * batch * ctx->tail_count));
     if (const char *e = getenv("DRT_DARK_SKIP")) ctx->dark_skip = ctx->dark_skip_win = atoi(e) != 0;
     if (getenv("DRT_VERBOSE"))
-        fprintf(stderr, "drt: %d CUs, trace %d blocks/CU (lds %zu), shade %d blocks/CU (lds %zu), batch %u, %.3f blocks/path measured (worst %u), pool %.2f GB\n",
-                prop.multiProcessorCount, per_cu, ctx->trace_lds, s_per_cu, ctx->shade_lds, ctx->batch_spp, ctx->est_blocks_per_path,
+        fprintf(stderr, "drt: %d CUs, trace %d blocks/CU (lds %zu), shade %d blocks/CU (%s, occupancy query %d, lds %zu; LDS rule: general %u, closed %u of %zu bytes), batch %u, %.3f blocks/path measured (worst %u), pool %.2f GB\n",
+                prop.multiProcessorCount, per_cu, ctx->trace_lds, s_per_cu, shade_closed_lds(ctx) ? "closed, headers in LDS" : shade_closed(ctx) ? "closed" : "general", s_query,
+                shade_closed_lds(ctx) ? ctx->shade_lds_closed : ctx->shade_lds, lds_general.groups_by_lds, lds_closed.groups_by_lds, lds_closed.group_bytes,
+                ctx->batch_spp, ctx->est_blocks_per_path,
                 ctx->worst_blocks_per_path, (double)(ctx->pool_blocks * block_bytes) / 1e9);
     HIP_TRY(hipStreamSynchronize(ctx->stream));
     return 0;
@@ -2112,6 +2137,12 @@
     if (!ctx) return -1;
     if (shade_closed(ctx)) return DRT_SHADE_CLOSED;
     return shade_simple(ctx) ? DRT_SHADE_SIMPLE : DRT_SHADE_GENERAL;
+}
+
+extern "C" int drt_shade_closed_lds(const drt_context *ctx)
+{
+    if (!ctx) return -1;
+    return shade_closed_lds(ctx) ? 1 : 0;
 }
 
 static int adaptive_check(drt_context *ctx, const drt_adaptive *a, bool held = false)
diff --git a/daily-ray-trace_amd/csrc/drt_shade_lds_rule.h b/daily-ray-trace_amd/csrc/drt_shade_lds_rule.h
--- /dev/null
+++ b/daily-ray-trace_amd/csrc/drt_shade_lds_rule.h
@@ -0,0 +1,37 @@
+#ifndef DRT_SHADE_LDS_RULE_H
+#define DRT_SHADE_LDS_RULE_H
+
+#include <algorithm>
+#include <cstddef>
+#include <cstdint>
+
+#define SHADE_LDS_PER_CU (160u * 1024u)
+#define SHADE_LDS_GRANULE 1280u
+#define SHADE_SIMDS_PER_CU 4u
+
+struct ShadeLdsPlan
+{
+    size_t   table_bytes;
+    size_t   wave_bytes;
+    size_t   group_bytes;
+    size_t   granted_bytes;
+    uint32_t groups_by_lds;
+    uint32_t groups;
+    uint32_t waves_per_simd;
+};
+
+static inline ShadeLdsPlan shade_lds_plan(uint32_t n_spd, uint32_t S, bool spds_in_lds, uint32_t block_waves, uint32_t wave_words, uint32_t register_waves)
+{
+    ShadeLdsPlan p{};
+    p.table_bytes = spds_in_lds ? (size_t)n_spd * S * 8 : 0;
+    p.wave_bytes = (size_t)wave_words * 8;
+    p.group_bytes = p.table_bytes + (size_t)block_waves * p.wave_bytes;
+    p.granted_bytes = (p.group_bytes + SHADE_LDS_GRANULE - 1) / SHADE_LDS_GRANULE * SHADE_LDS_GRANULE;
+    p.groups_by_lds = p.granted_bytes ? (uint32_t)(SHADE_LDS_PER_CU / p.granted_bytes) : ~0u;
+    const uint32_t groups_by_registers = register_waves * SHADE_SIMDS_PER_CU / std::max(1u, block_waves);
+    p.groups = std::min(p.groups_by_lds, groups_by_registers);
+    p.waves_per_simd = p.groups * block_waves / SHADE_SIMDS_PER_CU;
+    return p;
+}
+
+#endif
diff --git a/daily-ray-trace_amd/pydrt.py b/daily-ray-trace_amd/pydrt.py
--- a/daily-ray-trace_amd/pydrt.py
+++ b/daily-ray-trace_amd/pydrt.py
@@ -666,6 +666,9 @@
         if hasattr(L, "drt_shade_instantiation"):
             L.drt_shade_instantiation.argtypes = [C.c_void_p]
             L.drt_shade_instantiation.restype = C.c_int
+        if hasattr(L, "drt_shade_closed_lds"):
+            L.drt_shade_closed_lds.argtypes = [C.c_void_p]
+            L.drt_shade_closed_lds.restype = C.c_int
         if hasattr(L, "drt_update_surfaces"):
             L.drt_set_camera.argtypes = [C.c_void_p, C.POINTER(Camera)]
             L.drt_update_surfaces.argtypes = [C.c_void_p, C.c_void_p, C.c_uint32, C.c_uint32, C.c_uint32]
@@ -753,7 +756,7 @@
 
 SHADE_INSTANTIATIONS = ("general", "simple", "closed")
 
-HIP_SYMBOLS = ["drt_shade_instantiation",
+HIP_SYMBOLS = ["drt_shade_instantiation", "drt_shade_closed_lds",
                "drt_last_error", "drt_device_count", "drt_create", "drt_destroy", "drt_bind_film", "drt_set_stream",
                "drt_render", "drt_synchronize", "drt_reset_film", "drt_film_device_ptrs", "drt_read_film", "drt_write_film",
                "drt_read_xyz", "drt_read_bgra", "drt_read_hit_indices", "drt_get_stats", "drt_batch_spp", "drt_render_tile", "drt_selftest_arith",
@@ -1163,6 +1166,9 @@
     def shade_instantiation(self):
         return SHADE_INSTANTIATIONS[int(self.L.drt_shade_instantiation(self.ctx))]
 
+    def shade_closed_lds(self):
+        return int(self.L.drt_shade_closed_lds(self.ctx)) == 1
+
     def stats(self):
         st = Stats()
         _check(self.L.drt_get_stats(self.ctx, C.byref(st)), "drt_get_stats")
diff --git a/include/drt_hip.h b/include/drt_hip.h
--- a/include/drt_hip.h
+++ b/include/drt_hip.h
@@ -182,6 +182,7 @@
 #define DRT_SHADE_SIMPLE 1
 #define DRT_SHADE_CLOSED 2
 int drt_shade_instantiation(const drt_context *ctx);
+int drt_shade_closed_lds(const drt_context *ctx);
 
 int drt_render_tile(const drt_scene *scene, const drt_camera *camera, const drt_params *params,
                     double *dst_pixels, double *dst_avgs, double *dst_vars, drt_stats *stats);
```
